# titus-leistner/mmlf

Measured on AMD Instinct MI355X. Metric: 96x96 EPI patches/sec fwd+bwd, bs=512, higher is better.
Workload: dtype f32 via 2 x f16 operand split (22 significant bits per operand, locally scaled; 3 MFMA passes, f32 accumulate)

## Files before the change

### include/mmlf_hip.h

```cpp
#ifndef MMLF_HIP_H
#define MMLF_HIP_H

#include <stddef.h>
#include <stdint.h>

#ifdef __cplusplus
extern "C" {
#endif

#define MMLF_TILE_POSITIONS 256

const char *mmlf_last_error(void);
#define MMLF_ABI_VERSION 10
int mmlf_abi_version(void);

const char *mmlf_build_info(void);
int mmlf_build_is_ablation(void);
int mmlf_conv_cus(void);

enum { MMLF_AUDIT_IN = 0, MMLF_AUDIT_PACKED = 1, MMLF_AUDIT_BIAS = 2, MMLF_AUDIT_OUT = 3, MMLF_AUDIT_REF = 4,
       MMLF_AUDIT_IN_AMAX = 5, MMLF_AUDIT_OUT_AMAX = 6, MMLF_AUDIT_BN_PARTIAL = 7, MMLF_AUDIT_MASK = 8, MMLF_AUDIT_CONV_N = 9 };
int mmlf_audit_conv_h2(int cs_in, int K, int N, int cs_out, int N_store, int out_shift, int cs_ref, int B, int H, int W,
                       int64_t *ends);
enum { MMLF_AUDIT_WG_IN = 0, MMLF_AUDIT_WG_G = 1, MMLF_AUDIT_WG_GW = 2, MMLF_AUDIT_WG_GB = 3, MMLF_AUDIT_WG_WORKSPACE = 4,
       MMLF_AUDIT_WG_IN_AMAX = 5, MMLF_AUDIT_WG_G_AMAX = 6, MMLF_AUDIT_WGRAD_N = 7 };
int mmlf_audit_wgrad_h2(int cs_in, int Cin, int cs_g, int Cout, int g_shift, int B, int H, int W, int64_t *ends);

int64_t mmlf_grid_alloc_positions(int B, int H, int W);
int64_t mmlf_packed_filter_floats(int K, int N);
int64_t mmlf_wgrad_workspace_floats(int Cin, int Cout, int B, int H, int W);

enum { MMLF_VAR_IDENTITY = 0, MMLF_VAR_TRANSPOSE = 1, MMLF_VAR_TRANSPOSE_FLIPH = 2 };

int mmlf_pack_filter(const float *w_oihw, float *packed, int Cout, int Cin, int variant, int dgrad,
                     void *stream);

int mmlf_conv2x2(const float *in, int cs_in, int K, const float *packed, const float *bias, int N,
                 float *out, int cs_out, int N_store, int out_shift, int vh, int vw,
                 int B, int H, int W, int relu, const float *relu_ref, int cs_ref, void *stream);

int64_t mmlf_packed_filter_split_bytes(int K, int N);
int mmlf_pack_filter_split(const float *w_oihw, void *packed, int Cout, int Cin, int variant, int dgrad,
                           void *stream);
int mmlf_conv2x2_split(const float *in, int cs_in, int K, const void *packed, const float *bias, int N,
                       float *out, int cs_out, int N_store, int out_shift, int vh, int vw,
                       int B, int H, int W, int relu, const float *relu_ref, int cs_ref, void *stream);

int64_t mmlf_amax_entries(int B, int H, int W);
int mmlf_grid_pad_w(void);
int mmlf_grid_pad_h(void);
int mmlf_amax_head(void);
int mmlf_amax_shard_stride(void);
int64_t mmlf_packed_filter_h2_bytes(int K, int N);
int mmlf_pack_filter_h2(const float *w_oihw, void *packed, int Cout, int Cin, int variant, int dgrad, void *stream);
typedef struct mmlf_pack_desc {
    const float *w_oihw;
    void *packed;
    int32_t Cout, Cin, variant, dgrad;
    int32_t col0;
    int32_t np;
} mmlf_pack_desc;
int mmlf_packed_filter_h2_columns(int N);
int mmlf_pack_filters_h2(const mmlf_pack_desc *table, int n, int total_columns, void *stream);
int mmlf_conv2x2_h2(const float *in, int cs_in, int K, const void *packed, const float *bias, int N,
                    float *out, int cs_out, int N_store, int out_shift, int vh, int vw,
                    int B, int H, int W, int relu, const float *relu_ref, int cs_ref,
                    const float *in_amax , float *out_amax ,
                    double *bn_partial ,
                    uint32_t *relu_mask_out , const uint32_t *relu_mask_in , void *stream);
int64_t mmlf_relu_mask_words(int B, int H, int W);
int mmlf_conv2x2_blocks(int K, int N, int B, int H, int W);

int64_t mmlf_conv2x2_thin_workspace_floats(int B, int H, int W);
int mmlf_conv2x2_thin(const float *in, int cs_in, int K, const float *w_oihw, const float *bias, int N,
                      float *out, int cs_out, int out_shift, int vh, int vw, int B, int H, int W, int relu,
                      int variant, float *workspace, float *out_amax, void *stream);
int64_t mmlf_conv2x2_wgrad_thin_workspace_floats(int Cin);
int mmlf_conv2x2_wgrad_thin(const float *in, int cs_in, int Cin, const float *g, int cs_g, int Cout, int g_shift,
                            float *gw_oihw, float *gb, int variant, int accumulate, float *workspace,
                            int B, int H, int W, void *stream);

int mmlf_conv2x2_wgrad(const float *in, int cs_in, int Cin, const float *g, int cs_g, int Cout,
                       int g_shift, float *gw_oihw, float *gb, int variant, int accumulate,
                       float *workspace, int B, int H, int W, void *stream);

int mmlf_conv2x2_wgrad_split(const float *in, int cs_in, int Cin, const float *g, int cs_g, int Cout,
                             int g_shift, float *gw_oihw, float *gb, int variant, int accumulate,
                             float *workspace, int B, int H, int W, void *stream);

int mmlf_conv2x2_wgrad_h2(const float *in, int cs_in, int Cin, const float *g, int cs_g, int Cout,
                          int g_shift, float *gw_oihw, float *gb, int variant, int accumulate,
                          float *workspace, int B, int H, int W, const float *in_amax, const float *g_amax,
                          void *stream);

int mmlf_bn_stats_train(const float *z, int cs, int C, const float *gamma, const float *beta,
                        float *running_mean, float *running_var, double momentum, double eps,
                        float *save_mean, float *save_invstd, float *scale, float *shift,
                        double *partial, int nblocks, int B, int H, int W, void *stream);
int mmlf_bn_coeffs_eval(const float *gamma, const float *beta, const float *running_mean,
                        const float *running_var, double eps, float *scale, float *shift, int C,
                        void *stream);
int mmlf_fold_bn_eval(const float *w_oihw, const float *bias, const float *scale, const float *shift,
                      float *w_out, float *bias_out, int Cout, int Cin, void *stream);
int mmlf_bn_stats_finalize(const double *partial, int nblocks, int C, const float *gamma, const float *beta,
                           float *running_mean, float *running_var, double momentum, double eps,
                           float *save_mean, float *save_invstd, float *scale, float *shift,
                           int B, int H, int W, void *stream);
int mmlf_bn_apply_relu(const float *z, int cs_z, int C, const float *scale, const float *shift,
                       float *y, int cs_y, int c_off, int C_store, int B, int H, int W,
                       float *amax_out , void *stream);
int mmlf_bn_apply_relu4(const float *const z[4], int cs_z, int C, const float *const scale[4],
                        const float *const shift[4], float *y, int cs_y, int B, int H, int W,
                        float *amax_out , void *stream);
int mmlf_bn_bwd_reduce(const float *gy, int cs_gy, int c_off, const float *z, int cs_z, int C,
                       const float *scale, const float *shift, const float *gamma,
                       const float *save_mean, const float *save_invstd,
                       float *dgamma, float *dbeta, int accumulate, float *coef,
                       double *partial, int nblocks, int B, int H, int W, void *stream);
int mmlf_bn_bwd_apply(const float *gy, int cs_gy, int c_off, const float *z, int cs_z, int C,
                      const float *scale, const float *shift, const float *save_mean,
                      const float *coef, float *dz, int cs_dz, int B, int H, int W,
                      float *amax_out , void *stream);
int mmlf_relu_bwd_slice(const float *src, int cs_src, int c_off, const float *ref, int cs_ref, int ref_off, int C,
                        float *dst, int cs_dst, int B, int H, int W,
                        float *amax_out , void *stream);
enum { MMLF_AUDIT_SLICE_SRC = 0, MMLF_AUDIT_SLICE_REF = 1, MMLF_AUDIT_SLICE_DST = 2, MMLF_AUDIT_SLICE_AMAX = 3,
       MMLF_AUDIT_SLICE_N = 4 };
int mmlf_audit_relu_bwd_slice(int cs_src, int c_off, int cs_ref, int ref_off, int C, int cs_dst, int B, int H, int W,
                              int64_t *ends);

int mmlf_pack_nchw(const float *nchw, int C, float *grid, int cs, int B, int H, int W,
                   float *amax_out , void *stream);
int mmlf_unpack_nchw(const float *grid, int cs, float *nchw, int C, int B, int H, int W, void *stream);
int mmlf_zero_slack(float *grid, int cs, int B, int H, int W, float *amax, void *stream);
int mmlf_zero_slack4(float *const grid[4], const int cs[4], float *const amax[4], int B, int H, int W, void *stream);

int64_t mmlf_grid_alloc_positions_k3(int B, int H, int W);
int mmlf_zero_slack_k3(float *grid, int cs, int B, int H, int W, float *amax, void *stream);
int mmlf_zero_slack4_k3(float *const grid[4], const int cs[4], float *const amax[4], int B, int H, int W, void *stream);
int64_t mmlf_packed_filter3x3_floats(int K, int N);
int mmlf_pack_filter3x3(const float *w_oihw, float *packed, int Cout, int Cin, int variant, int dgrad, void *stream);
int mmlf_conv3x3(const float *in, int cs_in, int K, const float *packed, const float *bias, int N,
                 float *out, int cs_out, int N_store, int B, int H, int W, int relu, const float *relu_ref, int cs_ref,
                 void *stream);
int64_t mmlf_wgrad3x3_workspace_floats(int Cin, int Cout, int B, int H, int W);
int mmlf_conv3x3_wgrad(const float *in, int cs_in, int Cin, const float *g, int cs_g, int Cout, float *gw_oihw, float *gb,
                       int variant, int accumulate, float *workspace, int B, int H, int W, void *stream);
int mmlf_fold_bn_eval3x3(const float *w_oihw, const float *bias, const float *scale, const float *shift,
                         float *w_out, float *bias_out, int Cout, int Cin, void *stream);
int mmlf_audit_conv3x3(int cs_in, int K, int N, int cs_out, int N_store, int cs_ref, int B, int H, int W, int64_t *ends);
int mmlf_audit_wgrad3x3(int cs_in, int Cin, int cs_g, int Cout, int B, int H, int W, int64_t *ends);

int mmlf_head_upr(const float *output_nchw, const float *grid108, float *posterior, int steps,
                  int B, int H, int W, void *stream);
int mmlf_head_dpp(const float *scores_nchw, const float *grid_torch, const float *grid_np,
                  float *one_hot, float *posterior, float *mean, float *logvar, int steps,
                  int B, int H, int W, void *stream);
int mmlf_head_upr_bwd(const float *output_nchw, const float *grid108, const float *grad_posterior, float *grad_output,
                      int steps, int B, int H, int W, void *stream);
int mmlf_head_dpp_bwd(const float *scores_nchw, const float *grid_np, const float *mean, const float *grad_posterior,
                      const float *grad_logvar, float *grad_scores, int steps, int B, int H, int W, void *stream);

int mmlf_loss_fwd_bwd(int kind, const float *output_nchw, int oc, const float *gt, const int32_t *mask,
                      const float *grid_torch, double half_step, float *loss_out, float *grad_nchw,
                      double *scratch, int nblocks, const double *den_override, int B, int H, int W,
                      void *stream);

int64_t mmlf_loss_multi_scratch_doubles(int nblocks);
int mmlf_loss_multi_fwd_bwd(int kind, const float *output_nchw, int oc, const float *target, int P,
                            const int32_t *mask, const int32_t *mask_padding, const float *grid_torch,
                            double half_step, float *loss_out, float *grad_nchw, double *scratch, int nblocks,
                            const double *den_override, const double *aux_override, int B, int H, int W,
                            void *stream);

int mmlf_adam_step(float *p, const float *g, float *m, float *v, int64_t n, double lr, double beta1,
                   double beta2, double eps, int64_t step, double grad_scale, void *stream);

int mmlf_shift_views(const float *h, const float *v, const float *i, const float *d,
                     float *oh, float *ov, float *oi, float *od, const int32_t *tab_s, const float *tab_w,
                     int S, int views, int H, int W, void *stream);
int mmlf_shift_pack(const float *in, int kind, float *grid, int cs, const int32_t *tab_s, const float *tab_w,
                    int S, int views, int H, int W, float *amax_out, void *stream);
int mmlf_ensamble_reduce(const float *means, const float *logvars, const float *grid, float *mean,
                         float *logvar, float *posterior, int S, int B, int H, int W, void *stream);

int mmlf_lmm_to_discrete(const float *means, const float *logvars, const double *edges, double *out,
                         int S, int B, int n_bins, long long HW, void *stream);

int mmlf_patch_gather(const float *stacks, const float *center, const float *gt, const float *mpi,
                      const int32_t *mask, int S, int V, int P, int Hf, int Wf, const int32_t *iparam,
                      const float *fparam, const int32_t *tab_s, const float *tab_w, const double *mat,
                      const int32_t *rot_src, float *o_stacks, float *o_center, float *o_gt, float *o_mpi,
                      int32_t *o_mask, double *mean_sum, int B, int ps, void *stream);
int mmlf_patch_contrast(float *o_stacks, float *o_center, const double *mean_sum, const float *alpha,
                        int B, int V, int ps, void *stream);

#ifdef __cplusplus
}
#endif
#endif
```

### mmlf_amd/csrc/conv.hip

```cpp
#include "conv_device.h"


#ifdef MMLF_BOUNDS_DEBUG
extern "C" int mmlf_debug_oob_counts(unsigned long long *host8, int reset)
{
    unsigned long long other[8];
    if (hipMemcpyFromSymbol(host8, HIP_SYMBOL(g_mmlf_oob), sizeof(unsigned long long) * 8) != hipSuccess) return 1;
    if (reset) {
        const unsigned long long z[8] = {};
        if (hipMemcpyToSymbol(HIP_SYMBOL(g_mmlf_oob), z, sizeof(z)) != hipSuccess) return 1;
    }
    if (mmlf_oob_counts_wgrad(other, reset)) return 1;
    for (int k = 0; k < 8; ++k) host8[k] += other[k];
    return 0;
}
#endif

template <int KS>
__global__ void pack_filter_f32_kernel(const float *__restrict__ w, float *__restrict__ out, int Cout, int Cin,
                                       int variant, int dgrad, int nchunk, int NP)
{
    constexpr int TAPS = KS * KS;
    const long long total = (long long)nchunk * TAPS * 2 * NP * 4;
    for (long long idx = blockIdx.x * (long long)blockDim.x + threadIdx.x; idx < total;
         idx += (long long)gridDim.x * blockDim.x) {
        int s = idx & 3;
        long long r = idx >> 2;
        int n = r % NP; r /= NP;
        int kh = r & 1; r >>= 1;
        int t = r % TAPS; r /= TAPS;
        int c = (int)r;
        int k = 8 * c + 4 * kh + s;
        int ci, co, tsrc;
        if (!dgrad) { ci = k; co = n; tsrc = t; }
        else { co = k; ci = n; tsrc = TAPS - 1 - t; }
        float v = 0.f;
        if (ci < Cin && co < Cout) v = w[((size_t)co * Cin + ci) * TAPS + master_tap<KS>(tsrc, variant)];
        out[idx] = v;
    }
}

struct ConvArgs {
    const float *in;
    const float *wp;
    const float *bias;
    float *out;
    const float *ref;
    long long NQ;
    int cs_in, nchunk, cs_out, n_store, n_true, out_shift, vh, vw, P, G, relu, cs_ref;
    int a_pieces, seg_slot, seg_delta;
    int a_per_seg, a_tail;
    int nw;
    const float *in_amax;
    const float *w_unscale;
    float *out_amax;
    Magic divP, divR;
    int R;
    double *bn_partial;
    unsigned *relu_mask_out;
    const unsigned *relu_mask_in;
    long long out_bytes, ref_bytes;
    long long in_bytes, amax_n, mask_words;
};


__device__ __forceinline__ unsigned wave_row_mask(const ConvArgs &a, long long Q0, int w, int lane)
{
    const unsigned qrow = (unsigned)Q0 + 32 * w + (lane & 31);
    const unsigned row = fastdiv(qrow, a.divP);
    const int x = (int)(qrow - row * a.P), y = (int)(row - fastdiv(row, a.divR) * a.R);
    return (unsigned)__ballot((long long)qrow < a.NQ && y < a.vh && x < a.vw);
}

template <int NT>
__device__ __forceinline__ void conv_epilogue(const ConvArgs &a, const f32x16 (&acc)[NT], long long Q0, int w, int i,
                                              int kh)
{
    const unsigned m = wave_row_mask(a, Q0, w, i) >> (4 * kh);
    const long long qb = Q0 + 32 * w + a.out_shift;
    const __amdgpu_buffer_rsrc_t ob = __builtin_amdgcn_make_buffer_rsrc(
        a.out + (size_t)qb * a.cs_out, 0, mmlf_records_left(a.out_bytes, qb * a.cs_out * 4ll), MMLF_BUF_FLAGS);
    const bool has_ref = a.ref != nullptr;
    const __amdgpu_buffer_rsrc_t rb = __builtin_amdgcn_make_buffer_rsrc(
        const_cast<float *>(has_ref ? a.ref + (size_t)qb * a.cs_ref : a.out), 0,
        has_ref ? mmlf_records_left(a.ref_bytes, qb * a.cs_ref * 4ll) : 0, MMLF_BUF_FLAGS);
    unsigned lo = ((unsigned)(4 * kh) * a.cs_out + i) * 4u;
    unsigned lr = ((unsigned)(4 * kh) * a.cs_ref + i) * 4u;
    asm volatile("" : "+v"(lo), "+v"(lr));
    float bv[NT];
#pragma unroll
    for (int nt = 0; nt < NT; ++nt) {
        const int ch = 32 * nt + i;
        bv[nt] = (a.bias && ch < a.n_true) ? a.bias[ch] : 0.f;
    }
#pragma unroll
    for (int nt = 0; nt < NT; ++nt) {
        if (32 * nt + i >= a.n_store) continue;
        unsigned keep = m;
        if (has_ref) {
            float rv[16];
#pragma unroll
            for (int r = 0; r < 16; ++r)
                rv[r] = __uint_as_float(__builtin_amdgcn_raw_buffer_load_b32(
                    rb, lr + (unsigned)((r & 3) + 8 * (r >> 2)) * a.cs_ref * 4u + 128 * nt, 0, 0));
#pragma unroll
            for (int r = 0; r < 16; ++r)
                if (!(rv[r] > 0.f)) keep &= ~(1u << ((r & 3) + 8 * (r >> 2)));
        }
#pragma unroll
        for (int r = 0; r < 16; ++r) {
            const int rc = (r & 3) + 8 * (r >> 2);
            float v = acc[nt][r] + bv[nt];
            if (a.relu) v = fmaxf(v, 0.f);
            __builtin_amdgcn_raw_buffer_store_b32(__float_as_uint((keep >> rc & 1) ? v : 0.f), ob,
                                                  lo + (unsigned)rc * a.cs_out * 4u + 128 * nt, 0, 0);
        }
    }
}

__device__ __forceinline__ void pack_filter_h2_column(const float *__restrict__ w, unsigned short *__restrict__ out,
                                                      int Cout, int Cin, int variant, int dgrad, int nchunk, int NP,
                                                      float *__restrict__ unscale, int n, float *red)
{
    const int tid = threadIdx.x;
    const int K = dgrad ? Cout : Cin, N = dgrad ? Cin : Cout;
    auto at = [&](int k, int tap) -> size_t {
        return dgrad ? ((size_t)k * Cin + n) * 4 + tap : ((size_t)n * Cin + k) * 4 + tap;
    };
    float m = 0.f;
    if (n < N)
        for (int e = tid; e < 4 * K; e += 256) m = fmaxf(m, fabsf(w[at(e >> 2, e & 3)]));
    m = mmlf_wave_max(m);
    if ((tid & 63) == 0) red[tid >> 6] = m;
    __syncthreads();
    const float sc = pow2_scale_for(fmaxf(fmaxf(red[0], red[1]), fmaxf(red[2], red[3])));
    if (tid == 0) unscale[n] = 1.f / sc;
    for (int e = tid; e < 4 * nchunk; e += 256) {
        const int c = e >> 2, t = e & 3;
        const int tap = master_tap<2>(dgrad ? 3 - t : t, variant);
        unsigned short h[8], l[8];
#pragma unroll
        for (int j = 0; j < 8; ++j) {
            const int k = 8 * c + j;
            const float v = (k < K && n < N) ? w[at(k, tap)] * sc : 0.f;
            const _Float16 hh = (_Float16)v, ll = (_Float16)(v - (float)hh);
            h[j] = __builtin_bit_cast(unsigned short, hh);
            l[j] = __builtin_bit_cast(unsigned short, ll);
        }
        uint4 vh, vl;
        vh.x = h[0] | (unsigned)h[1] << 16; vh.y = h[2] | (unsigned)h[3] << 16;
        vh.z = h[4] | (unsigned)h[5] << 16; vh.w = h[6] | (unsigned)h[7] << 16;
        vl.x = l[0] | (unsigned)l[1] << 16; vl.y = l[2] | (unsigned)l[3] << 16;
        vl.z = l[4] | (unsigned)l[5] << 16; vl.w = l[6] | (unsigned)l[7] << 16;
        *reinterpret_cast<uint4 *>(out + ((((size_t)c * 2 + 0) * 4 + t) * NP + n) * 8) = vh;
        *reinterpret_cast<uint4 *>(out + ((((size_t)c * 2 + 1) * 4 + t) * NP + n) * 8) = vl;
    }
}

__global__ __launch_bounds__(256) void pack_filter_h2_kernel(const float *__restrict__ w, unsigned short *__restrict__ out,
                                                             int Cout, int Cin, int variant, int dgrad, int nchunk,
                                                             int NP, float *__restrict__ unscale)
{
    __shared__ float red[4];
    pack_filter_h2_column(w, out, Cout, Cin, variant, dgrad, nchunk, NP, unscale, blockIdx.x, red);
}

__global__ __launch_bounds__(256) void pack_filters_h2_kernel(const mmlf_pack_desc *__restrict__ table, int n)
{
    __shared__ float red[4];
    int lo = 0, hi = n - 1;
    while (lo < hi) {
        const int mid = (lo + hi + 1) >> 1;
        if (table[mid].col0 <= (int)blockIdx.x) lo = mid; else hi = mid - 1;
    }
    const mmlf_pack_desc d = table[lo];
    const int K = d.dgrad ? d.Cout : d.Cin;
    const int nchunk = (K + 7) / 8;
    unsigned short *out = reinterpret_cast<unsigned short *>(d.packed);
    float *tail = reinterpret_cast<float *>(reinterpret_cast<char *>(d.packed) + (size_t)nchunk * 8 * d.np * 16);
    pack_filter_h2_column(d.w_oihw, out, d.Cout, d.Cin, d.variant, d.dgrad, nchunk, d.np, tail, (int)blockIdx.x - d.col0, red);
}

__global__ void pack_filter_split_kernel(const float *__restrict__ w, unsigned short *__restrict__ out, int Cout,
                                         int Cin, int variant, int dgrad, int nchunk, int NP)
{
    const long long total = (long long)nchunk * 2 * 2 * NP * 8;
    for (long long idx = blockIdx.x * (long long)blockDim.x + threadIdx.x; idx < total;
         idx += (long long)gridDim.x * blockDim.x) {
        const int j = idx & 7;
        long long r = idx >> 3;
        const int n = r % NP; r /= NP;
        const int kh = r & 1; r >>= 1;
        const int u = r & 1; r >>= 1;
        const int c = (int)r;
        const int k = 8 * c + j, t = 2 * u + kh;
        int ci, co, tsrc;
        if (!dgrad) { ci = k; co = n; tsrc = t; }
        else { co = k; ci = n; tsrc = 3 - t; }
        float v = 0.f;
        if (ci < Cin && co < Cout) v = w[((size_t)co * Cin + ci) * 4 + master_tap<2>(tsrc, variant)];
        unsigned p[3];
        split3(v, p[0], p[1], p[2]);
        for (int pl = 0; pl < 3; ++pl) {
            out[((((size_t)c * 3 + pl) * 4 + t) * NP + n) * 8 + j] = (unsigned short)p[pl];
        }
    }
}



enum { EPI_GENERIC = -1, EPI_PLAIN = 0, EPI_RELU = 1, EPI_STATS = 2, EPI_BITS_IN = 4, EPI_REF_IN = 8, EPI_MASK_OUT = 16 };
template <int G, int EPI>
__device__ __forceinline__ void conv_epilogue16(const ConvArgs &a, const f32x4 (&acc)[2][G], long long Q0, int w,
                                                int r16, int q4, float unscale_a, float &run_max,
                                                double *stats_in )
{
    constexpr bool GEN = EPI == EPI_GENERIC;
    const bool do_relu = GEN ? a.relu != 0 : (EPI & EPI_RELU) != 0;
    double *const stats = (GEN || (EPI & EPI_STATS)) ? stats_in : nullptr;
    const bool mask_out = GEN ? a.relu_mask_out != nullptr : (EPI & EPI_MASK_OUT) != 0;
    const unsigned m = wave_row_mask(a, Q0, w, r16 + 16 * q4) >> (4 * q4);
    const long long qb = Q0 + 32 * w + a.out_shift;
    const int ob_left = mmlf_records_left(a.out_bytes, qb * a.cs_out * 4ll);
    const __amdgpu_buffer_rsrc_t ob =
        __builtin_amdgcn_make_buffer_rsrc(a.out + (size_t)qb * a.cs_out, 0, ob_left, MMLF_BUF_FLAGS);
    const bool has_ref = GEN ? a.ref != nullptr : (EPI & EPI_REF_IN) != 0;
    const __amdgpu_buffer_rsrc_t rb = __builtin_amdgcn_make_buffer_rsrc(
        const_cast<float *>(has_ref ? a.ref + (size_t)qb * a.cs_ref : a.out), 0,
        has_ref ? mmlf_records_left(a.ref_bytes, qb * a.cs_ref * 4ll) : 0, MMLF_BUF_FLAGS);
    unsigned lo = ((unsigned)(4 * q4) * a.cs_out + r16) * 4u;
    unsigned lr = ((unsigned)(4 * q4) * a.cs_ref + r16) * 4u;
    asm volatile("" : "+v"(lo), "+v"(lr));
    float mk[8];
#pragma unroll
    for (int k = 0; k < 8; ++k) mk[k] = 0.f;
    const bool use_bits = GEN ? a.relu_mask_in != nullptr : (EPI & EPI_BITS_IN) != 0;
    const size_t mbase = ((size_t)(Q0 / MMLF_TILE) * 8 + w) * 512 + (r16 + 16 * q4);
    unsigned mw[8];
#pragma unroll
    for (int k = 0; k < 8; ++k) mw[k] = use_bits ? a.relu_mask_in[mbase + 64 * k] : 0u;
    MMLF_OOB(OOB_MASK, (use_bits || mask_out) && (long long)mbase + 64 * 7 >= a.mask_words);
    float bv[G], uwv[G];
#pragma unroll
    for (int nb = 0; nb < G; ++nb) {
        const int ch = 16 * nb + r16;
        bv[nb] = (a.bias && ch < a.n_true) ? a.bias[ch] : 0.f;
        uwv[nb] = (a.w_unscale && ch < 16 * G) ? a.w_unscale[ch] : 1.f;
    }
#pragma unroll
    for (int nb = 0; nb < G; ++nb) asm volatile("" : "+v"(bv[nb]), "+v"(uwv[nb]));
#pragma unroll
    for (int nb = 0; nb < G; ++nb) {
        const int ch = 16 * nb + r16;
        if (ch >= a.n_store) continue;
        const float bvn = bv[nb];
        const float uw = uwv[nb];
        unsigned keep = m;
        float s1 = 0.f, s2 = 0.f;
        if (use_bits) {
#pragma unroll
            for (int k = 0; k < 8; ++k)
                if (!(mw[k] >> nb & 1)) keep &= ~(1u << (16 * (k >> 2) + (k & 3)));
        } else if (has_ref) {
            float rv[8];
#pragma unroll
            for (int k = 0; k < 8; ++k)
            {
                MMLF_OOB(OOB_REF, (qb * a.cs_ref * 4ll) + lr + (long long)(16 * (k >> 2) + (k & 3)) * a.cs_ref * 4 + 64 * nb >= a.ref_bytes);
                rv[k] = __uint_as_float(__builtin_amdgcn_raw_buffer_load_b32(
                    rb, lr + (unsigned)(16 * (k >> 2) + (k & 3)) * a.cs_ref * 4u + 64 * nb, 0, 0));
            }
#pragma unroll
            for (int k = 0; k < 8; ++k)
                if (!(rv[k] > 0.f)) keep &= ~(1u << (16 * (k >> 2) + (k & 3)));
        }
#pragma unroll
        for (int k = 0; k < 8; ++k) {
            const int rc = 16 * (k >> 2) + (k & 3);
            float v = fmaf(acc[k >> 2][nb][k & 3] * unscale_a, uw, bvn);
            if (do_relu) v = fmaxf(v, 0.f);
            v = (keep >> rc & 1) ? v : 0.f;
            if (mask_out) mw[k] |= (v > 0.f ? 1u : 0u) << nb;
            asm("v_max_f32 %0, %1, |%2|" : "=v"(mk[k]) : "v"(mk[k]), "v"(v));
            s1 += v;
            s2 = fmaf(v, v, s2);
            MMLF_OOB(OOB_OUT, (long long)lo + 64 * nb + (long long)rc * a.cs_out * 4 >= ob_left);
            __builtin_amdgcn_raw_buffer_store_b32(__float_as_uint(v), ob, lo + 64 * nb, (unsigned)rc * a.cs_out * 4u, 0);
        }
        if (stats) {
            s1 += __shfl_xor(s1, 16); s1 += __shfl_xor(s1, 32);
            s2 += __shfl_xor(s2, 16); s2 += __shfl_xor(s2, 32);
            if (q4 == 0) {
                stats[2 * (16 * nb + r16)] += (double)s1;
                stats[2 * (16 * nb + r16) + 1] += (double)s2;
            }
        }
    }
    if (mask_out) {
#pragma unroll
        for (int k = 0; k < 8; ++k) a.relu_mask_out[mbase + 64 * k] = mw[k];
    }
    if (a.out_amax) {
        const unsigned d0 = (unsigned)qb;
        const unsigned rd0 = fastdiv(d0, a.divP);
        const int nfirst = (int)((rd0 + 1) * (unsigned)a.P - d0);
        float m_lo = 0.f, m_hi = 0.f;
#pragma unroll
        for (int k = 0; k < 8; ++k) {
            const int pos = 16 * (k >> 2) + 4 * q4 + (k & 3);
            if (pos < nfirst) m_lo = fmaxf(m_lo, mk[k]);
            else m_hi = fmaxf(m_hi, mk[k]);
        }
        m_lo = mmlf_wave_max(m_lo);
        m_hi = mmlf_wave_max(m_hi);
        if (r16 + 16 * q4 == 0) {
            MMLF_OOB(OOB_AMAX, MMLF_AMAX_HEAD + (long long)fastdiv(d0 + 31, a.divP) >= a.amax_n);
            if (m_lo > 0.f) mmlf_amax_raise_nowait(a.out_amax + MMLF_AMAX_HEAD + rd0, m_lo);
            if (m_hi > 0.f) {
                const unsigned rdl = fastdiv(d0 + 31, a.divP);
                for (unsigned r = rd0 + 1; r <= rdl; ++r) mmlf_amax_raise_nowait(a.out_amax + MMLF_AMAX_HEAD + r, m_hi);
            }
            run_max = fmaxf(run_max, fmaxf(m_lo, m_hi));
        }
    }
}

template <int G> constexpr int tr_mask_words() { return (G + 7) / 8; }
template <int G, int EPI>
__device__ __forceinline__ void conv_epilogue16_tr(const ConvArgs &a, const f32x4 (&acc)[2][G], long long Q0, int w,
                                                   int r16, int q4, float unscale_a, float &run_max,
                                                   const float *coef )
{
    static_assert(EPI >= 0 && !(EPI & (EPI_STATS | EPI_REF_IN)), "kinds of the transposed epilogue");
    constexpr int NP = 16 * G, MW = tr_mask_words<G>();
    constexpr bool do_relu = (EPI & EPI_RELU) != 0, mask_out = (EPI & EPI_MASK_OUT) != 0, use_bits = (EPI & EPI_BITS_IN) != 0;
    const unsigned m = wave_row_mask(a, Q0, w, r16 + 16 * q4);
    const long long qb = Q0 + 32 * w + a.out_shift;
    const int ob_left = mmlf_records_left(a.out_bytes, qb * a.cs_out * 4ll);
    const __amdgpu_buffer_rsrc_t ob =
        __builtin_amdgcn_make_buffer_rsrc(a.out + (size_t)qb * a.cs_out, 0, ob_left, MMLF_BUF_FLAGS);
    unsigned lo = ((unsigned)r16 * a.cs_out + 4u * q4) * 4u;
    asm volatile("" : "+v"(lo));
    const size_t mbase = ((size_t)(Q0 / MMLF_TILE) * 8 + w) * 512 + (r16 + 16 * q4);
    unsigned mw[2][MW];
    bool ok[2];
#pragma unroll
    for (int mb = 0; mb < 2; ++mb) {
        ok[mb] = (m >> (16 * mb + r16) & 1u) != 0;
#pragma unroll
        for (int j = 0; j < MW; ++j) {
            mw[mb][j] = use_bits ? a.relu_mask_in[mbase + 64 * (MW * mb + j)] : 0u;
            if (use_bits && !ok[mb]) mw[mb][j] = 0u;
        }
    }
    MMLF_OOB(OOB_MASK, (use_bits || mask_out) && (long long)mbase + 64 * (2 * MW - 1) >= a.mask_words);
    float mk[2] = {0.f, 0.f};
    const float *cl = coef + 4 * q4;
    f32x4 uw_n = *reinterpret_cast<const f32x4 *>(cl), b_n = *reinterpret_cast<const f32x4 *>(cl + NP);
#pragma unroll
    for (int nb = 0; nb < G; ++nb) {
        const int c0 = 16 * nb + 4 * q4;
        const f32x4 uw4 = uw_n, b4 = b_n;
        if (nb + 1 < G) {
            uw_n = *reinterpret_cast<const f32x4 *>(cl + 16 * (nb + 1));
            b_n = *reinterpret_cast<const f32x4 *>(cl + NP + 16 * (nb + 1));
        }
        __builtin_amdgcn_sched_barrier(0);
#pragma unroll
        for (int mb = 0; mb < 2; ++mb) {
            u32x4 st;
#pragma unroll
            for (int r = 0; r < 4; ++r) {
                float v = fmaf(acc[mb][nb][r] * unscale_a, uw4[r], b4[r]);
                if (do_relu) v = fmaxf(v, 0.f);
                if (use_bits) {
                    const int keep = ((int)(mw[mb][nb >> 3] << (31 - (4 * (nb & 7) + r)))) >> 31;
                    v = __uint_as_float(__float_as_uint(v) & (unsigned)keep);
                } else {
                    v = ok[mb] ? v : 0.f;
                }
                if (mask_out) mw[mb][nb >> 3] |= (v > 0.f ? 1u : 0u) << (4 * (nb & 7) + r);
                asm("v_max_f32 %0, %1, |%2|" : "=v"(mk[mb]) : "v"(mk[mb]), "v"(v));
                st[r] = __float_as_uint(v);
            }
            if (c0 < a.n_store) {
                MMLF_OOB(OOB_OUT, (long long)lo + 64 * nb + (long long)(16 * mb) * a.cs_out * 4 + 12 >= ob_left);
                __builtin_amdgcn_raw_buffer_store_b128(st, ob, lo + 64 * nb, (unsigned)(16 * mb) * a.cs_out * 4u, 0);
            }
        }
        __builtin_amdgcn_sched_barrier(0);
    }
    if (mask_out) {
#pragma unroll
        for (int mb = 0; mb < 2; ++mb)
#pragma unroll
            for (int j = 0; j < MW; ++j) a.relu_mask_out[mbase + 64 * (MW * mb + j)] = mw[mb][j];
    }
    if (a.out_amax) {
        const unsigned d0 = (unsigned)qb;
        const unsigned rd0 = fastdiv(d0, a.divP);
        const int nfirst = (int)((rd0 + 1) * (unsigned)a.P - d0);
        float m_lo = 0.f, m_hi = 0.f;
#pragma unroll
        for (int mb = 0; mb < 2; ++mb) {
            if (16 * mb + r16 < nfirst) m_lo = fmaxf(m_lo, mk[mb]);
            else m_hi = fmaxf(m_hi, mk[mb]);
        }
        m_lo = mmlf_wave_max(m_lo);
        m_hi = mmlf_wave_max(m_hi);
        if (r16 + 16 * q4 == 0) {
            MMLF_OOB(OOB_AMAX, MMLF_AMAX_HEAD + (long long)fastdiv(d0 + 31, a.divP) >= a.amax_n);
            if (m_lo > 0.f) mmlf_amax_raise_nowait(a.out_amax + MMLF_AMAX_HEAD + rd0, m_lo);
            if (m_hi > 0.f) {
                const unsigned rdl = fastdiv(d0 + 31, a.divP);
                for (unsigned r = rd0 + 1; r <= rdl; ++r) mmlf_amax_raise_nowait(a.out_amax + MMLF_AMAX_HEAD + r, m_hi);
            }
            run_max = fmaxf(run_max, fmaxf(m_lo, m_hi));
        }
    }
}
template <int NP>
__device__ __forceinline__ void conv_fill_coef(const ConvArgs &a, float *coef, int tid, int nthreads)
{
    for (int k = tid; k < NP; k += nthreads) {
        coef[k] = a.w_unscale ? a.w_unscale[k] : 1.f;
        coef[NP + k] = (a.bias && k < a.n_true) ? a.bias[k] : 0.f;
    }
}

__device__ __forceinline__ float wave_operand_amax_gather(const ConvArgs &a, long long Q0, int w, int lane)
{
    const long long q0 = Q0 + 32 * w;
    float m = 0.f;
    if (q0 < a.NQ) {
        const long long ql = q0 + 31 < a.NQ ? q0 + 31 : a.NQ - 1;
        const unsigned r0 = fastdiv((unsigned)q0, a.divP);
        unsigned r1 = fastdiv((unsigned)ql, a.divP);
        r1 += (r1 - fastdiv(r1, a.divR) * (unsigned)a.R != (unsigned)(a.R - 1)) ? 1u : 0u;
        MMLF_OOB(OOB_AMAX, lane == 0 && MMLF_AMAX_HEAD + (long long)r1 >= a.amax_n);
        for (unsigned r = r0 + lane; r <= r1; r += 64) m = fmaxf(m, a.in_amax[MMLF_AMAX_HEAD + r]);
    }
    return m;
}
__device__ __forceinline__ float wave_operand_scale(float gathered)
{
    return __uint_as_float(__builtin_amdgcn_readfirstlane(__float_as_uint(pow2_scale_for(mmlf_wave_max(gathered)))));
}

typedef const __attribute__((address_space(4))) ConvArgs *ConvKernArgs;
__device__ __forceinline__ ConvArgs late_args()
{
#if defined(__HIP_DEVICE_COMPILE__)
    ConvKernArgs p = (ConvKernArgs)__builtin_amdgcn_kernarg_segment_ptr();
    asm volatile("" : "+s"(p));
    return *p;
#else
    return ConvArgs();
#endif
}

constexpr int RING16 = 3;
template <int G, int PL, int EPI = EPI_GENERIC, int NW = 8, bool TR = false>
__global__ __launch_bounds__(64 * NW, (NW == 16 || G <= 6 ? 4 : 2)) void conv4tap_x6s_kernel(ConvArgs a, int ntiles)
{
    constexpr int NP = G * 16;
    constexpr int TILE = 32 * NW;
    constexpr int D = NW == 16 ? RING16 : 2;
    constexpr bool EARLY = PL == 2 && G % 3 == 0 && G >= 9;
    constexpr int A_F4 = 2 * 640;
    constexpr int B_F4 = 4 * PL * NP;
    constexpr int BUF_F4 = A_F4 + B_F4;
    constexpr int N_B = B_F4 / 64;
    constexpr int PER_WAVE = (20 + N_B + NW - 1) / NW;
    constexpr int PER_SLOT = (PER_WAVE + 1) / 2;
    extern __shared__ __attribute__((aligned(16))) char smem[];
    float4 *lds = reinterpret_cast<float4 *>(smem);

    const int tid = threadIdx.x;
    const int lane = tid & 63;
    const int w = __builtin_amdgcn_readfirstlane(tid >> 6);
    const int r16 = lane & 15, q4 = lane >> 4;

    f32x4 acc[2][G];
#pragma unroll
    for (int mb = 0; mb < 2; ++mb)
#pragma unroll
        for (int nb = 0; nb < G; ++nb)
#pragma unroll
            for (int r = 0; r < 4; ++r) acc[mb][nb][r] = 0.f;

    const unsigned voff_a = ((unsigned)(lane >> 1) * (unsigned)a.cs_in + 4u * (lane & 1)) * 4u;
    const unsigned voff_b = (unsigned)lane * 16u;
    const unsigned lds_base = (unsigned)(size_t)(lds_void_t *)smem;
    const char *in0 = reinterpret_cast<const char *>(a.in);
    const char *wp_base = reinterpret_cast<const char *>(a.wp);
    const size_t tile_bytes = (size_t)TILE * a.cs_in * 4;
    const int n_a = a.a_pieces;
    const int nA = (n_a - w + NW - 1) / NW;
    const int jb0 = w + NW * nA - n_a;
    const int nB = (N_B - jb0 + NW - 1) / NW;
    int n_mine = nA + nB;
    unsigned a_src[3], a_dst[3];
#pragma unroll
    for (int k = 0; k < 3; ++k) {
        const int j = w + NW * k;
        const int seg = j >= a.a_per_seg, idx = j - seg * a.a_per_seg;
        const int slot = 320 * seg + 32 * idx;
        a_src[k] = (unsigned)(slot + seg * a.seg_delta) * (unsigned)a.cs_in * 4u;
        a_dst[k] = (unsigned)slot * 32u + (idx == a.a_per_seg - 1 ? 1u : 0u);
    }
    const unsigned tail_lim = ((unsigned)(a.a_tail - 1) * (unsigned)a.cs_in + 4u) * 4u;
    const unsigned b_src0 = 1024u * jb0, b_dst0 = (unsigned)(A_F4 + 64 * jb0) * 16u;

#ifdef MMLF_BOUNDS_DEBUG
#define MMLF_DMA_SRC_CHECK()                                                                             \
    do {                                                                                                 \
        MMLF_OOB(OOB_IN, (long long)(sb_ - in0) + vo_ + 16 > a.in_bytes);                                \
        const unsigned long long u_ = (unsigned long long)sb_;                                           \
        sb_ = reinterpret_cast<const char *>(                                                            \
            ((unsigned long long)__builtin_amdgcn_readfirstlane((unsigned)(u_ >> 32)) << 32) |           \
            (unsigned)__builtin_amdgcn_readfirstlane((unsigned)u_));                                     \
    } while (0)
#else
#define MMLF_DMA_SRC_CHECK() do { } while (0)
#endif
#define X6_DMA_PIECE(tl, c, buf, k)                                                                      \
    do {                                                                                                 \
        if ((k) < PER_WAVE && (k) < n_mine) {                                                            \
            const char *sb_;                                                                             \
            unsigned vo_, d_;                                                                            \
            if ((k) < nA) {                                                                              \
                sb_ = in0 + (size_t)(tl) * tile_bytes + 32u * (c) + a_src[(k) < 3 ? (k) : 0];            \
                d_ = a_dst[(k) < 3 ? (k) : 0];                                                           \
                vo_ = min(voff_a, (d_ & 1u) ? tail_lim : 0xffffffffu);                                   \
                d_ &= ~1u;                                                                               \
                MMLF_DMA_SRC_CHECK();                                                                    \
            } else {                                                                                     \
                const unsigned kb_ = (1024u * NW) * (unsigned)((k) - nA);                                \
                sb_ = wp_base + (size_t)(c) * (B_F4 * 16) + b_src0 + kb_;                                \
                vo_ = voff_b;                                                                            \
                d_ = b_dst0 + kb_;                                                                       \
            }                                                                                            \
            d_ = __builtin_amdgcn_readfirstlane(d_ + lds_base + (buf) * (BUF_F4 * 16));                  \
            unsigned keep_;                                                                              \
            asm volatile("s_mov_b32 %0, m0\n\ts_mov_b32 m0, %3\n\ts_nop 0\n\t"                       \
                         "global_load_lds_dwordx4 %1, %2\n\ts_mov_b32 m0, %0"                           \
                         : "=&s"(keep_) : "v"(vo_), "s"(sb_), "s"(d_) : "memory");                      \
        }                                                                                                \
    } while (0)
#define X6_DMA_SLOT(tl, c, buf, slot)                                                                    \
    do {                                                                                                 \
        _Pragma("unroll") for (int k_ = 0; k_ < PER_SLOT; ++k_)                                          \
            X6_DMA_PIECE(tl, c, buf, (slot) * PER_SLOT + k_);                                            \
    } while (0)
#define X6_DMA_WAIT() asm volatile("s_waitcnt vmcnt(0)" ::: "memory")
#define X6_CHUNK_WAIT()                                                                                  \
    do {                                                                                                 \
        if (D > 2 && more) {       \
            static_assert(PER_WAVE <= 3 || D == 2, "counted waits are written for up to three pieces per wave");             \
            if (n_mine == 1) asm volatile("s_waitcnt vmcnt(%0)" ::"n"(1 * (D - 2)) : "memory");            \
            else if (n_mine == 2) asm volatile("s_waitcnt vmcnt(%0)" ::"n"(2 * (D - 2)) : "memory");       \
            else if (n_mine == 3) asm volatile("s_waitcnt vmcnt(%0)" ::"n"(3 * (D - 2)) : "memory");       \
            else X6_DMA_WAIT();                                                                          \
        } else {                                                                                         \
            X6_DMA_WAIT();                                                                               \
        }                                                                                                \
    } while (0)

    const int per_xcd = (int)gridDim.x >> 3;
    const int first_tile = (gridDim.x & 7) == 0 ? (int)(blockIdx.x & 7) * per_xcd + (int)(blockIdx.x >> 3)
                                                : (int)blockIdx.x;
    int tile = first_tile, c = 0;
    int ntile = tile, nc = 0;
    if (tile >= ntiles) return;
    float *coef = reinterpret_cast<float *>(lds + D * BUF_F4);
    double *stats_all = reinterpret_cast<double *>(lds + D * BUF_F4);
    if constexpr (TR) conv_fill_coef<NP>(late_args(), coef, tid, 64 * NW);
    else if (late_args().bn_partial)
        for (int k = tid; k < NW * NP * 2; k += 64 * NW) stats_all[k] = 0.0;
    float scale_a = 1.f, unscale_a = 1.f, run_max = 0.f;
    if constexpr (PL == 2) {
        scale_a = wave_operand_scale(wave_operand_amax_gather(late_args(), (long long)tile * TILE, w, lane));
        unscale_a = 1.f / scale_a;
    }
#pragma unroll
    for (int d = 0; d < D - 1; ++d) {
        if (ntile < ntiles) {
            X6_DMA_SLOT(ntile, nc, d, 0);
            X6_DMA_SLOT(ntile, nc, d, 1);
        }
        if (++nc == a.nchunk) { nc = 0; ntile += gridDim.x; }
    }
    X6_DMA_WAIT();
    __syncthreads();
    int buf = 0;
    float4 ra[2][2];
    bf16x8 bq[3][PL];
    const int a_lane = 2 * (32 * w + r16 + (q4 & 1) + (q4 >> 1) * a.seg_slot);
    const int b_lane = q4 * NP + r16;
    if constexpr (EARLY) {
#pragma unroll
        for (int mb = 0; mb < 2; ++mb)
#pragma unroll
            for (int hf = 0; hf < 2; ++hf) ra[mb][hf] = lds[a_lane + 32 * mb + hf];
#pragma unroll
        for (int g0 = 0; g0 < 2; ++g0)
#pragma unroll
            for (int pl = 0; pl < PL; ++pl)
                bq[g0][pl] = (reinterpret_cast<const bf16x8 *>(lds + A_F4) + b_lane)[pl * 4 * NP + 16 * g0];
    }

    while (tile < ntiles) {
        asm volatile("" : "+s"(n_mine));
        const bool more = ntile < ntiles;
        const int fb = buf == 0 ? D - 1 : buf - 1;
        const float4 *base = lds + buf * BUF_F4;
        const float4 *nbase = lds + (buf + 1 == D ? 0 : buf + 1) * BUF_F4;
        const float4 *ap = base + a_lane;
        const bf16x8 *bp = reinterpret_cast<const bf16x8 *>(base + A_F4) + b_lane;
        const bf16x8 *bpn = reinterpret_cast<const bf16x8 *>(nbase + A_F4) + b_lane;
        const bool tile_end = c + 1 == a.nchunk;

        if constexpr (!EARLY) {
#pragma unroll
            for (int mb = 0; mb < 2; ++mb)
#pragma unroll
                for (int hf = 0; hf < 2; ++hf) ra[mb][hf] = ap[32 * mb + hf];
#pragma unroll
            for (int g0 = 0; g0 < 2; ++g0)
#pragma unroll
                for (int pl = 0; pl < PL; ++pl) bq[g0][pl] = bp[pl * 4 * NP + 16 * g0];
        }
        bf16x8 asp[2][PL];
#pragma unroll
        for (int mb = 0; mb < 2; ++mb) {
            unsigned hh[4], mm[4], ll[4];
            if constexpr (PL == 3) {
                split3_pair(ra[mb][0].x, ra[mb][0].y, hh[0], mm[0], ll[0]);
                split3_pair(ra[mb][0].z, ra[mb][0].w, hh[1], mm[1], ll[1]);
                split3_pair(ra[mb][1].x, ra[mb][1].y, hh[2], mm[2], ll[2]);
                split3_pair(ra[mb][1].z, ra[mb][1].w, hh[3], mm[3], ll[3]);
                const u32x4_t vm = {mm[0], mm[1], mm[2], mm[3]};
                asp[mb][1] = __builtin_bit_cast(bf16x8, vm);
            } else {
                split2_pair_f16(ra[mb][0].x, ra[mb][0].y, scale_a, hh[0], ll[0]);
                split2_pair_f16(ra[mb][0].z, ra[mb][0].w, scale_a, hh[1], ll[1]);
                split2_pair_f16(ra[mb][1].x, ra[mb][1].y, scale_a, hh[2], ll[2]);
                split2_pair_f16(ra[mb][1].z, ra[mb][1].w, scale_a, hh[3], ll[3]);
            }
            const u32x4_t vh = {hh[0], hh[1], hh[2], hh[3]}, vl = {ll[0], ll[1], ll[2], ll[3]};
            asp[mb][0] = __builtin_bit_cast(bf16x8, vh);
            asp[mb][PL - 1] = __builtin_bit_cast(bf16x8, vl);
        }
#pragma unroll
        for (int g = 0; g < G; ++g) {
            if (EARLY && g == G - 2) {
                X6_CHUNK_WAIT();
                asm volatile("s_waitcnt lgkmcnt(0)" ::: "memory");
                __syncthreads();
                if (!tile_end) {
#pragma unroll
                    for (int mb = 0; mb < 2; ++mb)
#pragma unroll
                        for (int hf = 0; hf < 2; ++hf) ra[mb][hf] = (nbase + a_lane)[32 * mb + hf];
                }
            }
            if (g + 2 < G) {
#pragma unroll
                for (int pl = 0; pl < PL; ++pl) bq[(g + 2) % 3][pl] = bp[pl * 4 * NP + 16 * (g + 2)];
            } else if (EARLY && !tile_end) {
#pragma unroll
                for (int pl = 0; pl < PL; ++pl) bq[(g + 2) % 3][pl] = bpn[pl * 4 * NP + 16 * (g + 2 - G)];
            }
            __builtin_amdgcn_sched_barrier(0);
            if (more) {
                if (w < NW / 2) {
                    if (g == 0) { X6_DMA_SLOT(ntile, nc, fb, 0); X6_DMA_SLOT(ntile, nc, fb, 1); }
                } else {
                    if (g == (PL == 2 && G >= 8 ? G / 8 : G / 4)) { X6_DMA_SLOT(ntile, nc, fb, 0); X6_DMA_SLOT(ntile, nc, fb, 1); }
                }
            }
            __builtin_amdgcn_sched_barrier(0);
#define X6_TERM(pa, pb)                                                                                      \
    _Pragma("unroll") for (int mb = 0; mb < 2; ++mb)                                                         \
        acc[mb][g] = __builtin_amdgcn_mfma_f32_16x16x32_bf16(asp[mb][pa], bq[g % 3][pb], acc[mb][g], 0, 0, 0)
#define H2_TERM(pa, pb)                                                                                      \
    _Pragma("unroll") for (int mb = 0; mb < 2; ++mb)                                                         \
        acc[mb][g] = TR ? __builtin_amdgcn_mfma_f32_16x16x32_f16(__builtin_bit_cast(f16x8, bq[g % 3][pb]),   \
                                                                 __builtin_bit_cast(f16x8, asp[mb][pa]), acc[mb][g], 0, 0, 0) \
                        : __builtin_amdgcn_mfma_f32_16x16x32_f16(__builtin_bit_cast(f16x8, asp[mb][pa]),     \
                                                                 __builtin_bit_cast(f16x8, bq[g % 3][pb]), acc[mb][g], 0, 0, 0)
            if constexpr (PL == 3) {
                X6_TERM(2, 0);
                X6_TERM(0, 2);
                X6_TERM(1, 1);
                X6_TERM(1, 0);
                X6_TERM(0, 1);
                X6_TERM(0, 0);
            } else {
                H2_TERM(1, 0);
                H2_TERM(0, 1);
                H2_TERM(0, 0);
            }
#undef X6_TERM
#undef H2_TERM
            __builtin_amdgcn_sched_barrier(0);
        }
        if (more && ++nc == a.nchunk) { nc = 0; ntile += gridDim.x; }
        if constexpr (!EARLY) X6_CHUNK_WAIT();
        if (++c == a.nchunk) {
            const ConvArgs e = late_args();
            float next_amax = 0.f;
            if constexpr (PL == 2)
                if (tile + (int)gridDim.x < ntiles)
                    next_amax = wave_operand_amax_gather(e, (long long)(tile + gridDim.x) * TILE, w, lane);
            if constexpr (TR)
                conv_epilogue16_tr<G, EPI>(e, acc, (long long)tile * TILE, w, r16, q4, unscale_a, run_max, coef);
            else
                conv_epilogue16<G, EPI>(e, acc, (long long)tile * TILE, w, r16, q4, unscale_a, run_max,
                                        e.bn_partial ? stats_all + (size_t)w * NP * 2 : nullptr);
#pragma unroll
            for (int mb = 0; mb < 2; ++mb)
#pragma unroll
                for (int nb = 0; nb < G; ++nb)
#pragma unroll
                    for (int r = 0; r < 4; ++r) acc[mb][nb][r] = 0.f;
            c = 0;
            tile += gridDim.x;
            if constexpr (PL == 2) {
                if (tile < ntiles) {
                    scale_a = wave_operand_scale(next_amax);
                    unscale_a = 1.f / scale_a;
                }
            }
            if constexpr (EARLY) {
#pragma unroll
                for (int mb = 0; mb < 2; ++mb)
#pragma unroll
                    for (int hf = 0; hf < 2; ++hf) ra[mb][hf] = (nbase + a_lane)[32 * mb + hf];
#pragma unroll
                for (int g0 = 0; g0 < 2; ++g0)
#pragma unroll
                    for (int pl = 0; pl < PL; ++pl) bq[g0][pl] = bpn[pl * 4 * NP + 16 * g0];
            }
        }
        if constexpr (!EARLY) __syncthreads();
        buf = buf + 1 == D ? 0 : buf + 1;
    }
    if constexpr (EARLY) __syncthreads();
    const ConvArgs e = late_args();
    if (e.out_amax) mmlf_amax_update(run_max, e.out_amax, blockIdx.x * NW + w);
    if (e.bn_partial) {
        for (int k = tid; k < 2 * e.n_true; k += 64 * NW) {
            const int ch = k % e.n_true, which = k / e.n_true;
            double t = 0.0;
#pragma unroll
            for (int ww = 0; ww < NW; ++ww) t += stats_all[((size_t)ww * NP + ch) * 2 + which];
            e.bn_partial[((size_t)blockIdx.x * 2 + which) * e.n_true + ch] = t;
        }
    }
#undef X6_DMA_PIECE
#undef MMLF_DMA_SRC_CHECK
#undef X6_DMA_SLOT
#undef X6_DMA_WAIT
#undef X6_CHUNK_WAIT
}



template <int G, int NCH, int EPI, bool TR = false>
__global__ __launch_bounds__(512, 2) void conv4tap_rs_kernel(ConvArgs a, int ngroups)
{
    constexpr int NP = G * 16;
    constexpr int WBYTES = NCH * 2 * 4 * NP * 16;
    constexpr int NS = NCH / 4, REM = NCH % 4;
    static_assert(REM == 0 || REM == 1, "input channels: a multiple of 32, or one octet more");
    constexpr int NSTEP = 4 * NS + REM, NLOAD = 4 * NSTEP;
    extern __shared__ __attribute__((aligned(16))) char smem[];
    const int tid = threadIdx.x;
    const int lane = tid & 63;
    const int w = __builtin_amdgcn_readfirstlane(tid >> 6);
    const int r16 = lane & 15, q4 = lane >> 4;

    for (int o = tid * 16; o < WBYTES; o += 512 * 16)
        *reinterpret_cast<uint4 *>(smem + o) = *reinterpret_cast<const uint4 *>(reinterpret_cast<const char *>(a.wp) + o);
    float *coef = reinterpret_cast<float *>(smem + WBYTES);
    double *stats_all = reinterpret_cast<double *>(smem + WBYTES);
    if constexpr (TR) conv_fill_coef<NP>(a, coef, tid, 512);
    else if (a.bn_partial)
        for (int k = tid; k < 8 * NP * 2; k += 512) stats_all[k] = 0.0;
    __syncthreads();

    int gi, gstep, gend;
    if ((gridDim.x & 7) == 0) {
        const int per = (ngroups + 7) >> 3, nbx = (int)gridDim.x >> 3;
        const int x = (int)blockIdx.x & 7;
        gi = x * per + ((int)blockIdx.x >> 3) * 8 + w;
        gstep = nbx * 8;
        gend = min(ngroups, (x + 1) * per);
    } else {
        gi = (int)blockIdx.x * 8 + w;
        gstep = (int)gridDim.x * 8;
        gend = ngroups;
    }

    f32x4 acc[2][G];
#pragma unroll
    for (int mb = 0; mb < 2; ++mb)
#pragma unroll
        for (int nb = 0; nb < G; ++nb)
#pragma unroll
            for (int r = 0; r < 4; ++r) acc[mb][nb][r] = 0.f;
    float run_max = 0.f;
    const bf16x8 *bpF = reinterpret_cast<const bf16x8 *>(smem) + q4 * 8 * NP + r16;
    const bf16x8 *bpR = reinterpret_cast<const bf16x8 *>(smem) + q4 * NP + r16;
    auto bfrag = [&](int k, int nb, int pl) -> bf16x8 {
        return k < 4 * NS ? bpF[(8 * (k % NS) + pl) * 4 * NP + (k / NS) * NP + 16 * nb] : bpR[(8 * NS + pl) * 4 * NP + 16 * nb];
    };
    const size_t row_off = (size_t)r16 * a.cs_in;
    const size_t rem_off = (size_t)((q4 & 1) + (q4 >> 1) * a.P) * a.cs_in + 32 * NS;

    for (; gi < gend; gi += gstep) {
        const long long Q0 = (long long)(gi >> 3) * MMLF_TILE;
        const int wv = gi & 7;
        const float gathered = wave_operand_amax_gather(a, Q0, wv, lane);
        const float *p0 = a.in + (size_t)(Q0 + 32 * wv) * a.cs_in + row_off;
        float4 raw[NSTEP][2][2];
#pragma unroll
        for (int k = 0; k < NSTEP; ++k) {
            const int t = k / NS, s_ = k % NS;
            const float *pk = k < 4 * NS ? p0 + (size_t)((t & 1) + (t >> 1) * a.P) * a.cs_in + 32 * s_ + 8 * q4 : p0 + rem_off;
#pragma unroll
            for (int mb = 0; mb < 2; ++mb)
#pragma unroll
                for (int hf = 0; hf < 2; ++hf)
                {
                    MMLF_OOB(OOB_IN, (long long)((pk + (size_t)(16 * mb) * a.cs_in + 4 * hf + 4) - a.in) * 4 > a.in_bytes);
                    raw[k][mb][hf] = reinterpret_cast<const float4 *>(pk + (size_t)(16 * mb) * a.cs_in)[hf];
                }
            __builtin_amdgcn_sched_barrier(0);
        }
        asm volatile("s_waitcnt vmcnt(%0)" ::"n"(NLOAD > 63 ? 63 : NLOAD) : "memory");
        const float scale_a = wave_operand_scale(gathered);
        const float unscale_a = 1.f / scale_a;
        bf16x8 bq[3][2];
#pragma unroll
        for (int g0 = 0; g0 < 2; ++g0)
#pragma unroll
            for (int pl = 0; pl < 2; ++pl) bq[g0][pl] = bfrag(0, g0, pl);
#pragma unroll
        for (int k = 0; k < NSTEP; ++k) {
            asm volatile("s_waitcnt vmcnt(%0)" ::"n"(4 * (NSTEP - 1 - k) > 63 ? 63 : 4 * (NSTEP - 1 - k)) : "memory");
            bf16x8 asp[2][2];
#pragma unroll
            for (int mb = 0; mb < 2; ++mb) {
                unsigned hh[4], ll[4];
                float4 &r0 = raw[k][mb][0], &r1 = raw[k][mb][1];
                asm volatile("" : "+v"(r0.x), "+v"(r0.y), "+v"(r0.z), "+v"(r0.w), "+v"(r1.x), "+v"(r1.y), "+v"(r1.z), "+v"(r1.w));
                split2_pair_f16(r0.x, r0.y, scale_a, hh[0], ll[0]);
                split2_pair_f16(r0.z, r0.w, scale_a, hh[1], ll[1]);
                split2_pair_f16(r1.x, r1.y, scale_a, hh[2], ll[2]);
                split2_pair_f16(r1.z, r1.w, scale_a, hh[3], ll[3]);
                const u32x4_t vh = {hh[0], hh[1], hh[2], hh[3]}, vl = {ll[0], ll[1], ll[2], ll[3]};
                asp[mb][0] = __builtin_bit_cast(bf16x8, vh);
                asp[mb][1] = __builtin_bit_cast(bf16x8, vl);
            }
            __builtin_amdgcn_sched_barrier(0);
            asm volatile("s_nop 4" ::: "memory");
            __builtin_amdgcn_sched_barrier(0);
#pragma unroll
            for (int g = 0; g < G; ++g) {
                constexpr int NB = NSTEP * G;
                const int idx = k * G + g;
                if (idx + 2 < NB) {
#pragma unroll
                    for (int pl = 0; pl < 2; ++pl) bq[(idx + 2) % 3][pl] = bfrag((idx + 2) / G, (idx + 2) % G, pl);
                }
#define RS_TERM(pa, pb)                                                                                      \
    _Pragma("unroll") for (int mb = 0; mb < 2; ++mb)                                                         \
        acc[mb][g] = TR ? __builtin_amdgcn_mfma_f32_16x16x32_f16(__builtin_bit_cast(f16x8, bq[idx % 3][pb]), \
                                                                 __builtin_bit_cast(f16x8, asp[mb][pa]), acc[mb][g], 0, 0, 0) \
                        : __builtin_amdgcn_mfma_f32_16x16x32_f16(__builtin_bit_cast(f16x8, asp[mb][pa]),     \
                                                                 __builtin_bit_cast(f16x8, bq[idx % 3][pb]), acc[mb][g], 0, 0, 0)
                RS_TERM(1, 0);
                RS_TERM(0, 1);
                RS_TERM(0, 0);
#undef RS_TERM
            }
        }
        if constexpr (TR)
            conv_epilogue16_tr<G, EPI>(a, acc, Q0, wv, r16, q4, unscale_a, run_max, coef);
        else
            conv_epilogue16<G, EPI>(a, acc, Q0, wv, r16, q4, unscale_a, run_max,
                                    a.bn_partial ? stats_all + (size_t)w * NP * 2 : nullptr);
#pragma unroll
        for (int mb = 0; mb < 2; ++mb)
#pragma unroll
            for (int nb = 0; nb < G; ++nb)
#pragma unroll
                for (int r = 0; r < 4; ++r) acc[mb][nb][r] = 0.f;
    }
    if (a.out_amax) mmlf_amax_update(run_max, a.out_amax, blockIdx.x * 8 + w);
    if (a.bn_partial) {
        __syncthreads();
        for (int k = tid; k < 2 * a.n_true; k += 512) {
// ... 168 lines not shown
                           int dgrad, void *stream)
{
    MMLF_CHECK_ARG(w && packed, "%s: null pointer", who);
    MMLF_CHECK_ARG(variant >= 0 && variant <= 2, "%s: bad variant %d", who, variant);
    MMLF_CHECK_ARG(Cout > 0 && Cin > 0, "%s: bad channels %d x %d", who, Cout, Cin);
    const int K = dgrad ? Cout : Cin, N = dgrad ? Cin : Cout;
    const int nt = pick_nt(N);
    MMLF_CHECK_ARG(nt > 0, "%s: N=%d not supported (max 288)", who, N);
    const int nchunk = (K + 7) / 8, NP = nt * 32;
    const long long total = (long long)nchunk * ks * ks * 2 * NP * 4;
    int blocks = (int)((total + 255) / 256);
    if (blocks > 4096) blocks = 4096;
    hipLaunchKernelGGL(ks == 2 ? pack_filter_f32_kernel<2> : pack_filter_f32_kernel<3>, dim3(blocks), dim3(256), 0,
                       (hipStream_t)stream, w, packed, Cout, Cin, variant, dgrad, nchunk, NP);
    return mmlf_launch_status(who);
}

extern "C" int64_t mmlf_packed_filter_floats(int K, int N) { return packed_filter_f32_floats(2, K, N); }

extern "C" int mmlf_pack_filter(const float *w, float *packed, int Cout, int Cin, int variant, int dgrad,
                                void *stream)
{
    return pack_filter_f32("mmlf_pack_filter", 2, w, packed, Cout, Cin, variant, dgrad, stream);
}

static void conv_buffer_bytes(ConvArgs &a, const Grid &g, long long alloc)
{
    a.out_bytes = (alloc * a.cs_out - (a.cs_out - a.n_store)) * 4;
    a.ref_bytes = a.ref ? alloc * a.cs_ref * 4 : 0;
    a.in_bytes = alloc * a.cs_in * 4;
    a.amax_n = amax_entries(g);
    a.mask_words = g.NQpad / MMLF_TILE * 4096;
}

static int conv_common_args(const char *who, int ks, int np, ConvArgs &a, Grid &g, const float *in, int cs_in, int K,
                            const void *packed, const float *bias, int N, float *out, int cs_out, int N_store,
                            int out_shift, int vh, int vw, int B, int H, int W, int relu, const float *relu_ref, int cs_ref)
{
    MMLF_CHECK_ARG(in && packed && out, "%s: null pointer", who);
    MMLF_CHECK_ARG(B > 0 && H > 0 && W > 0, "%s: bad shape B=%d H=%d W=%d", who, B, H, W);
    MMLF_CHECK_ARG(cs_in > 0 && cs_in % 8 == 0, "%s: cs_in=%d must be a multiple of 8", who, cs_in);
    MMLF_CHECK_ARG(K > 0 && (K + 7) / 8 * 8 == cs_in, "%s: K=%d does not match cs_in=%d", who, K, cs_in);
    MMLF_CHECK_ARG(np > 0, "%s: N=%d not supported (max 288)", who, N);
    MMLF_CHECK_ARG(N_store > 0 && N_store <= cs_out && N_store <= np, "%s: N_store=%d vs cs_out=%d NP=%d", who,
                   N_store, cs_out, np);
    g = make_grid(B, H, W);
    MMLF_CHECK_ARG(out_shift >= 0 && out_shift <= g.P + 1, "%s: out_shift=%d", who, out_shift);
    MMLF_CHECK_ARG(!relu_ref || cs_ref >= N_store, "%s: cs_ref=%d < N_store", who, cs_ref);
    MMLF_CHECK_ARG(g.NQpad + (ks - 1) * g.P + 64 < (1ll << 31), "%s: batch x image too large for 32-bit grid positions", who);
    a = {};
    a.in = in; a.wp = reinterpret_cast<const float *>(packed); a.bias = bias; a.out = out; a.ref = relu_ref;
    a.NQ = g.NQ; a.cs_in = cs_in; a.nchunk = cs_in / 8; a.cs_out = cs_out; a.n_store = N_store; a.n_true = N;
    a.out_shift = out_shift; a.vh = vh; a.vw = vw; a.P = g.P; a.G = g.G; a.R = g.R; a.relu = relu; a.cs_ref = cs_ref;
    a.divP = make_magic((unsigned)g.P); a.divR = make_magic((unsigned)g.R);
    conv_buffer_bytes(a, g, ks == 3 ? grid_alloc_positions_k3(g) : grid_alloc_positions(g));
    return 0;
}

template <int KS, int NT>
static int launch_conv_f32(const ConvArgs &a, long long ntiles, int ncb, hipStream_t st)
{
    constexpr const char *who = KS == 2 ? "mmlf_conv2x2" : "mmlf_conv3x3";
    constexpr size_t lds = ConvF32Lds<KS, NT>::BYTES;
    static PerDeviceOnce attr_once;
    if constexpr (KS == 2) {
        if (attr_once.run([] { return mmlf_allow_lds(reinterpret_cast<const void *>(conv4tap_kernel<NT>), lds, who); })) return 1;
        hipLaunchKernelGGL(conv4tap_kernel<NT>, dim3((unsigned)ntiles), dim3(512), lds, st, a);
    } else {
        if (attr_once.run([] { return mmlf_allow_lds(reinterpret_cast<const void *>(conv9tap_kernel<NT>), lds, who); })) return 1;
        hipLaunchKernelGGL(conv9tap_kernel<NT>, dim3((unsigned)(ntiles * ncb)), dim3(512), lds, st, a, ncb, ncb * NT * 32);
    }
    return mmlf_launch_status(who);
}

extern "C" int mmlf_conv2x2(const float *in, int cs_in, int K, const float *packed, const float *bias, int N,
                            float *out, int cs_out, int N_store, int out_shift, int vh, int vw, int B, int H,
                            int W, int relu, const float *relu_ref, int cs_ref, void *stream)
{
    const int nt = pick_nt(N);
    ConvArgs a;
    Grid g;
    if (conv_common_args("mmlf_conv2x2", 2, nt * 32, a, g, in, cs_in, K, packed, bias, N, out, cs_out, N_store, out_shift, vh,
                         vw, B, H, W, relu, relu_ref, cs_ref))
        return 1;
    const long long ntiles = g.NQpad / MMLF_TILE;
    hipStream_t st = (hipStream_t)stream;
    switch (nt) {
    case 1: return launch_conv_f32<2, 1>(a, ntiles, 1, st);
    case 3: return launch_conv_f32<2, 3>(a, ntiles, 1, st);
    case 4: return launch_conv_f32<2, 4>(a, ntiles, 1, st);
    default: return launch_conv_f32<2, 9>(a, ntiles, 1, st);
    }
}

static inline int x6_np(int N)
{
    if (N <= 0 || N > 288) return -1;
    if (N <= 32) return 32;
    if (N <= 80) return 80;
    if (N <= 128) return (N + 15) / 16 * 16;
    return 288;
}

extern "C" int64_t mmlf_packed_filter_split_bytes(int K, int N)
{
    const int np = x6_np(N);
    if (np < 0 || K <= 0) return -1;
    return (int64_t)((K + 7) / 8) * 12 * np * 16;
}

extern "C" int mmlf_pack_filter_split(const float *w, void *packed, int Cout, int Cin, int variant, int dgrad,
                                      void *stream)
{
    MMLF_CHECK_ARG(w && packed, "mmlf_pack_filter_split: null pointer");
    MMLF_CHECK_ARG(variant >= 0 && variant <= 2, "mmlf_pack_filter_split: bad variant %d", variant);
    const int K = dgrad ? Cout : Cin, N = dgrad ? Cin : Cout;
    const int NP = x6_np(N);
    MMLF_CHECK_ARG(NP > 0, "mmlf_pack_filter_split: N=%d not supported (max 288)", N);
    const int nchunk = (K + 7) / 8;
    const long long total = (long long)nchunk * 32 * NP;
    int blocks = (int)((total + 255) / 256);
    if (blocks > 4096) blocks = 4096;
    hipLaunchKernelGGL(pack_filter_split_kernel, dim3(blocks), dim3(256), 0, (hipStream_t)stream, w,
                       (unsigned short *)packed, Cout, Cin, variant, dgrad, nchunk, NP);
    return mmlf_launch_status("mmlf_pack_filter_split");
}

static long long conv_split_blocks(int G, long long ntiles, int nw = 8)
{
    const long long grid = (G <= 6 && nw == 8 ? 2ll : 1ll) * device_cus();
    return grid > ntiles ? ntiles : grid;
}
static bool conv_sixteen_waves(int planes, int np, const Grid &g)
{
    static const int on = [] { const char *e = getenv("MMLF_CONV_NW16"); return e ? atoi(e) : 1; }();
    return on && planes == 2 && np == 80 && g.P + 513 <= 640;
}

static bool conv_tr_enabled()
{
    static const int on = [] { const char *e = getenv("MMLF_CONV_TR"); return e ? atoi(e) : 1; }();
    return on != 0;
}
static bool conv_tr_fits(const ConvArgs &a)
{
    return a.n_store % 4 == 0 && a.cs_out % 4 == 0 && (reinterpret_cast<uintptr_t>(a.out) & 15) == 0;
}

template <int G, int PL, int EPI, bool TR = false>
static int launch_conv_x6s_epi(const ConvArgs &a, long long ntiles, hipStream_t st)
{
    constexpr size_t lds_pipe = 2 * (2 * 640 + 4 * PL * G * 16) * sizeof(float4);
    constexpr size_t lds_stats = 8 * (G * 16) * 2 * sizeof(double);
    constexpr size_t lds_coef = 2 * (G * 16) * sizeof(float);
    static PerDeviceOnce attr_once;
    if (attr_once.run([] { return mmlf_allow_lds(reinterpret_cast<const void *>(conv4tap_x6s_kernel<G, PL, EPI, 8, TR>),
                                                 lds_pipe + (TR ? lds_coef : PL == 2 ? lds_stats : 0), "mmlf_conv2x2_h2"); }))
        return 1;
    if constexpr (PL == 2 && G == 5) {
        if (a.nw == 16) {
            constexpr size_t lds_stats16 = 16 * (G * 16) * 2 * sizeof(double);
            constexpr size_t lds_pipe16 = RING16 * (2 * 640 + 4 * PL * G * 16) * sizeof(float4);
            static PerDeviceOnce attr_once16;
            if (attr_once16.run([] { return mmlf_allow_lds(reinterpret_cast<const void *>(conv4tap_x6s_kernel<G, PL, EPI, 16, TR>),
                                                           lds_pipe16 + (TR ? lds_coef : lds_stats16), "mmlf_conv2x2_h2(16 waves)"); }))
                return 1;
            const size_t lds16 = lds_pipe16 + (TR ? lds_coef : a.bn_partial ? lds_stats16 : 0);
            const long long grid16 = conv_split_blocks(G, ntiles, 16);
            hipLaunchKernelGGL((conv4tap_x6s_kernel<G, PL, EPI, 16, TR>), dim3((unsigned)grid16), dim3(1024), lds16, st, a, (int)ntiles);
            return mmlf_launch_status("mmlf_conv2x2_h2(16 waves)");
        }
    }
    const size_t lds = lds_pipe + (TR ? lds_coef : a.bn_partial ? lds_stats : 0);
    const long long grid = conv_split_blocks(G, ntiles);
    hipLaunchKernelGGL((conv4tap_x6s_kernel<G, PL, EPI, 8, TR>), dim3((unsigned)grid), dim3(512), lds, st, a, (int)ntiles);
    return mmlf_launch_status(PL == 3 ? "mmlf_conv2x2_split" : "mmlf_conv2x2_h2");
}

static int conv_rs_mode()
{
    static const int mode = [] { const char *e = getenv("MMLF_CONV_RS"); return e ? atoi(e) : -1; }();
    return mode;
}
static bool conv_rs_shape(int planes, int np, int nchunk, int nw)
{
    if (!(planes == 2 && np == 80 && (nchunk == 9 || nchunk == 4))) return false;
    const int mode = conv_rs_mode();
    return mode < 0 ? nw == 8 : mode != 0;
}
static long long conv_rs_blocks(long long ngroups)
{
    const long long grid = device_cus(), need = (ngroups + 7) / 8;
    return grid > need ? need : grid;
}
template <int G, int NCH, int EPI, bool TR = false>
static int launch_conv_rs_epi(const ConvArgs &a, long long ngroups, hipStream_t st)
{
    constexpr size_t lds = (size_t)NCH * 2 * 4 * (G * 16) * 16 + (TR ? 2 * (G * 16) * sizeof(float) : 8 * (G * 16) * 2 * sizeof(double));
    static PerDeviceOnce attr_once;
    if (attr_once.run([] { return mmlf_allow_lds(reinterpret_cast<const void *>(conv4tap_rs_kernel<G, NCH, EPI, TR>), lds, "mmlf_conv2x2_h2(register-streamed)"); }))
        return 1;
    hipLaunchKernelGGL((conv4tap_rs_kernel<G, NCH, EPI, TR>), dim3((unsigned)conv_rs_blocks(ngroups)), dim3(512), lds, st, a, (int)ngroups);
    return mmlf_launch_status("mmlf_conv2x2_h2(register-streamed)");
}
#define MMLF_CONV_KIND_SWITCH(LAUNCH, TR_PLAIN, TR_SHAPE, ...)                                                                              \
    do {                                                                                                                \
        const int kind = (a.relu ? EPI_RELU : 0) | (a.bn_partial ? EPI_STATS : 0) | (a.relu_mask_in ? EPI_BITS_IN : 0) | \
                         (a.ref ? EPI_REF_IN : 0) | (a.relu_mask_out ? EPI_MASK_OUT : 0);                               \
        const bool tr = conv_tr_enabled() && (TR_SHAPE) && conv_tr_fits(a);                                             \
        if ((a.relu_mask_in || a.relu_mask_out) && conv_tr_enabled() && (TR_SHAPE) && !tr)                              \
            return mmlf_fail("mmlf_conv2x2_h2: ReLU mask words need n_store %% 4 == 0 and a 16-byte aligned output");   \
        switch (kind) {                                                                                                 \
        case EPI_PLAIN: return tr && TR_PLAIN ? LAUNCH<__VA_ARGS__, EPI_PLAIN, true>(a, n, st) : LAUNCH<__VA_ARGS__, EPI_PLAIN>(a, n, st); \
        case EPI_RELU: return tr ? LAUNCH<__VA_ARGS__, EPI_RELU, true>(a, n, st) : LAUNCH<__VA_ARGS__, EPI_RELU>(a, n, st); \
        case EPI_RELU | EPI_MASK_OUT:                                                                                   \
            return tr ? LAUNCH<__VA_ARGS__, EPI_RELU | EPI_MASK_OUT, true>(a, n, st) : LAUNCH<__VA_ARGS__, EPI_RELU | EPI_MASK_OUT>(a, n, st); \
        case EPI_BITS_IN: return tr ? LAUNCH<__VA_ARGS__, EPI_BITS_IN, true>(a, n, st) : LAUNCH<__VA_ARGS__, EPI_BITS_IN>(a, n, st); \
        case EPI_STATS: return LAUNCH<__VA_ARGS__, EPI_STATS>(a, n, st);                                                \
        default: break;                                                                                                 \
        }                                                                                                               \
    } while (0)
template <int G, int NCH>
static int launch_conv_rs(const ConvArgs &a, long long n, hipStream_t st)
{
    MMLF_CONV_KIND_SWITCH(launch_conv_rs_epi, false, true, G, NCH);
    return launch_conv_rs_epi<G, NCH, EPI_GENERIC>(a, n, st);
}

template <int G, int PL>
static int launch_conv_x6s(const ConvArgs &a, long long ntiles, hipStream_t st)
{
    if constexpr (PL == 2 && G == 5) {
        if (conv_rs_shape(PL, G * 16, a.nchunk, a.nw)) {
            const long long ngroups = ntiles * a.nw;
            return a.nchunk == 9 ? launch_conv_rs<G, 9>(a, ngroups, st) : launch_conv_rs<G, 4>(a, ngroups, st);
        }
    }
    if constexpr (PL == 2 && (G == 5 || G == 18)) {
        const long long n = ntiles;
        if (a.ref && !a.relu && !a.bn_partial && !a.relu_mask_in && !a.relu_mask_out)
            return launch_conv_x6s_epi<G, PL, EPI_REF_IN>(a, n, st);
        MMLF_CONV_KIND_SWITCH(launch_conv_x6s_epi, G == 18, G != 18 || a.seg_delta == 0, G, PL);
    }
    return launch_conv_x6s_epi<G, PL, EPI_GENERIC>(a, ntiles, st);
}

template <int PL>
static int launch_conv_split(int np, const ConvArgs &a, long long ntiles, hipStream_t st)
{
    switch (np) {
    case 32: return launch_conv_x6s<2, PL>(a, ntiles, st);
    case 80: return launch_conv_x6s<5, PL>(a, ntiles, st);
    case 96: return launch_conv_x6s<6, PL>(a, ntiles, st);
    case 112: return launch_conv_x6s<7, PL>(a, ntiles, st);
    case 128: return launch_conv_x6s<8, PL>(a, ntiles, st);
    default: return launch_conv_x6s<18, PL>(a, ntiles, st);
    }
}

static int conv_split_impl(const char *who, int planes, const float *in, int cs_in, int K, const void *packed,
                           const float *bias, int N, float *out, int cs_out, int N_store, int out_shift, int vh,
                           int vw, int B, int H, int W, int relu, const float *relu_ref, int cs_ref,
                           const float *in_amax, float *out_amax, double *bn_partial, void *stream,
                           unsigned *relu_mask_out = nullptr, const unsigned *relu_mask_in = nullptr)
{
    const int np = x6_np(N);
    ConvArgs a;
    Grid g;
    if (conv_common_args(who, 2, np, a, g, in, cs_in, K, packed, bias, N, out, cs_out, N_store, out_shift, vh, vw, B, H, W, relu,
                         relu_ref, cs_ref))
        return 1;
    MMLF_CHECK_ARG(!(relu_ref && relu_mask_in), "%s: relu_ref and relu_mask_in are alternatives", who);
    MMLF_CHECK_ARG((long long)cs_in * 4 * 64 < (1ll << 31), "%s: cs_in too large", who);
    MMLF_CHECK_ARG(planes == 3 || in_amax, "%s: the f16 split needs the input's max |x|", who);
    MMLF_CHECK_ARG(!bn_partial || (planes == 2 && N_store >= N), "%s: BatchNorm statistics need the f16 split path", who);
    a.in_amax = in_amax; a.out_amax = out_amax; a.bn_partial = bn_partial;
    a.relu_mask_out = relu_mask_out; a.relu_mask_in = relu_mask_in;
    a.w_unscale = planes == 2 ? reinterpret_cast<const float *>(reinterpret_cast<const char *>(packed) +
                                                                  (size_t)(cs_in / 8) * 8 * np * 16)
                              : nullptr;
    a.nw = conv_sixteen_waves(planes, np, g) ? 16 : 8;
    const int tile = 32 * a.nw;
    if (g.P + tile + 1 <= 640) {
        a.a_pieces = a.a_per_seg = (g.P + tile + 1 + 31) / 32; a.seg_slot = g.P; a.seg_delta = 0;
    } else {
        a.a_per_seg = 9; a.a_pieces = 18; a.seg_slot = 320; a.seg_delta = g.P - 320;
    }
    a.a_tail = (a.seg_delta ? 257 : g.P + tile + 1) - 32 * (a.a_per_seg - 1);
    const long long ntiles = g.NQpad / tile;
    hipStream_t st = (hipStream_t)stream;
    return planes == 3 ? launch_conv_split<3>(np, a, ntiles, st) : launch_conv_split<2>(np, a, ntiles, st);
}

extern "C" int mmlf_conv2x2_split(const float *in, int cs_in, int K, const void *packed, const float *bias, int N,
                                  float *out, int cs_out, int N_store, int out_shift, int vh, int vw, int B, int H,
                                  int W, int relu, const float *relu_ref, int cs_ref, void *stream)
{
    return conv_split_impl("mmlf_conv2x2_split", 3, in, cs_in, K, packed, bias, N, out, cs_out, N_store, out_shift,
                           vh, vw, B, H, W, relu, relu_ref, cs_ref, nullptr, nullptr, nullptr, stream);
}

extern "C" int64_t mmlf_packed_filter_h2_bytes(int K, int N)
{
    const int np = x6_np(N);
    if (np < 0 || K <= 0) return -1;
    return (int64_t)((K + 7) / 8) * 8 * np * 16 + (int64_t)np * 4;
}

extern "C" int mmlf_pack_filter_h2(const float *w, void *packed, int Cout, int Cin, int variant, int dgrad,
                                   void *stream)
{
    MMLF_CHECK_ARG(w && packed, "mmlf_pack_filter_h2: null pointer");
    MMLF_CHECK_ARG(variant >= 0 && variant <= 2, "mmlf_pack_filter_h2: bad variant %d", variant);
    const int K = dgrad ? Cout : Cin, N = dgrad ? Cin : Cout;
    const int NP = x6_np(N);
    MMLF_CHECK_ARG(NP > 0, "mmlf_pack_filter_h2: N=%d not supported (max 288)", N);
    const int nchunk = (K + 7) / 8;
    float *tail = reinterpret_cast<float *>(reinterpret_cast<char *>(packed) + (size_t)nchunk * 8 * NP * 16);
    hipLaunchKernelGGL(pack_filter_h2_kernel, dim3(NP), dim3(256), 0, (hipStream_t)stream, w, (unsigned short *)packed,
                       Cout, Cin, variant, dgrad, nchunk, NP, tail);
    return mmlf_launch_status("mmlf_pack_filter_h2");
}

extern "C" int mmlf_packed_filter_h2_columns(int N) { return x6_np(N); }

extern "C" int mmlf_pack_filters_h2(const mmlf_pack_desc *table, int n, int total_columns, void *stream)
{
    MMLF_CHECK_ARG(table && n > 0 && total_columns > 0, "mmlf_pack_filters_h2: empty table");
    hipLaunchKernelGGL(pack_filters_h2_kernel, dim3((unsigned)total_columns), dim3(256), 0, (hipStream_t)stream, table, n);
    return mmlf_launch_status("mmlf_pack_filters_h2");
}

extern "C" int mmlf_conv2x2_h2(const float *in, int cs_in, int K, const void *packed, const float *bias, int N,
                               float *out, int cs_out, int N_store, int out_shift, int vh, int vw, int B, int H,
                               int W, int relu, const float *relu_ref, int cs_ref, const float *in_amax,
                               float *out_amax, double *bn_partial, uint32_t *relu_mask_out,
                               const uint32_t *relu_mask_in, void *stream)
{
    return conv_split_impl("mmlf_conv2x2_h2", 2, in, cs_in, K, packed, bias, N, out, cs_out, N_store, out_shift, vh,
                           vw, B, H, W, relu, relu_ref, cs_ref, in_amax, out_amax, bn_partial, stream, relu_mask_out,
                           relu_mask_in);
}

extern "C" int64_t mmlf_relu_mask_words(int B, int H, int W)
{
    if (B <= 0 || H <= 0 || W <= 0) return -1;
    return make_grid(B, H, W).NQpad / MMLF_TILE * 4096;
}

extern "C" int mmlf_conv2x2_blocks(int K, int N, int B, int H, int W)
{
    const int np = x6_np(N);
    if (np < 0 || K <= 0 || B <= 0 || H <= 0 || W <= 0) return -1;
    const Grid g = make_grid(B, H, W);
    const int nw = conv_sixteen_waves(2, np, g) ? 16 : 8;
    if (conv_rs_shape(2, np, (K + 7) / 8, nw)) return (int)conv_rs_blocks(g.NQpad / 32);
    return (int)conv_split_blocks(np / 16, g.NQpad / (32 * nw), nw);
}


__global__ __launch_bounds__(256) void thin_rowdot_kernel(ThinArgs a)
{
    __shared__ float tile[4][64][33];
    __shared__ float4 wt[4][32][2];
    const int lane = threadIdx.x & 63, wv = threadIdx.x >> 6;
    const long long wave = __builtin_amdgcn_readfirstlane((int)(blockIdx.x * 4 + wv));
    const long long nwaves = gridDim.x * 4ll;
    const int nslice = (a.C + 31) / 32;
    for (long long p0 = 64 * wave; p0 < a.npos; p0 += 64 * nwaves) {
        float acc[4][THIN_MAXN];
#pragma unroll
        for (int t = 0; t < 4; ++t)
#pragma unroll
            for (int o = 0; o < THIN_MAXN; ++o) acc[t][o] = 0.f;
        for (int sl = 0; sl < nslice; ++sl) {
            float4 v[8];
#pragma unroll
            for (int j = 0; j < 8; ++j) {
                const int r = (lane >> 3) + 8 * j, f = lane & 7;
                const long long p = p0 + r < a.npos ? p0 + r : a.npos - 1;
                const int c = 32 * sl + 4 * f;
                v[j] = *reinterpret_cast<const float4 *>(a.in + (size_t)p * a.cs_in + (c < a.cs_in ? c : 0));
                if (c >= a.cs_in) v[j] = make_float4(0.f, 0.f, 0.f, 0.f);
            }
            {
                const int c = 32 * sl + (lane & 31), o = lane >> 5;
                float4 w4 = make_float4(0.f, 0.f, 0.f, 0.f);
                if (c < a.C && o < a.N) {
                    const float *wp = a.w + ((size_t)o * a.C + c) * 4;
                    w4 = make_float4(wp[master_tap<2>(0, a.variant)], wp[master_tap<2>(1, a.variant)], wp[master_tap<2>(2, a.variant)],
                                     wp[master_tap<2>(3, a.variant)]);
                }
                wt[wv][lane & 31][o] = w4;
            }
#pragma unroll
            for (int j = 0; j < 8; ++j) {
                const int r = (lane >> 3) + 8 * j, f = lane & 7;
                tile[wv][r][4 * f + 0] = v[j].x; tile[wv][r][4 * f + 1] = v[j].y;
                tile[wv][r][4 * f + 2] = v[j].z; tile[wv][r][4 * f + 3] = v[j].w;
            }
#pragma unroll 8
            for (int k = 0; k < 32; ++k) {
                const float x = tile[wv][lane][k];
                const float4 w0 = wt[wv][k][0], w1 = wt[wv][k][1];
                acc[0][0] = fmaf(x, w0.x, acc[0][0]); acc[1][0] = fmaf(x, w0.y, acc[1][0]);
                acc[2][0] = fmaf(x, w0.z, acc[2][0]); acc[3][0] = fmaf(x, w0.w, acc[3][0]);
                acc[0][1] = fmaf(x, w1.x, acc[0][1]); acc[1][1] = fmaf(x, w1.y, acc[1][1]);
                acc[2][1] = fmaf(x, w1.z, acc[2][1]); acc[3][1] = fmaf(x, w1.w, acc[3][1]);
            }
        }
        const long long p = p0 + lane;
        if (p < a.npos) {
            float4 *dst = reinterpret_cast<float4 *>(a.part + (size_t)p * 4 * THIN_MAXN);
            dst[0] = make_float4(acc[0][0], acc[0][1], acc[1][0], acc[1][1]);
            dst[1] = make_float4(acc[2][0], acc[2][1], acc[3][0], acc[3][1]);
        }
    }
}

__global__ __launch_bounds__(128) void thin_combine_kernel(ThinArgs a)
{
    const int drow = blockIdx.x;
    float mx = 0.f;
    for (int x = threadIdx.x; x < a.P; x += blockDim.x) {
        const long long d = (long long)drow * a.P + x, q = d - a.out_shift;
        float v[THIN_MAXN] = {0.f, 0.f};
        bool valid = false;
        if (q >= 0 && q < a.NQ) {
            const unsigned row = fastdiv((unsigned)q, a.divP);
            const int qx = (int)(q - (long long)row * a.P), qy = (int)(row - fastdiv(row, a.divR) * a.R);
            valid = qy < a.vh && qx < a.vw;
        }
        if (valid) {
            const int offs[4] = {0, 1, a.P, a.P + 1};
#pragma unroll
            for (int o = 0; o < THIN_MAXN; ++o) {
                float s = (a.bias && o < a.N) ? a.bias[o] : 0.f;
#pragma unroll
                for (int t = 0; t < 4; ++t) s += a.part[((size_t)(q + offs[t]) * 4 + t) * THIN_MAXN + o];
                if (a.relu) s = fmaxf(s, 0.f);
                v[o] = o < a.N ? s : 0.f;
            }
        }
        float *dst = a.out + (size_t)d * a.cs_out;
        for (int o = 0; o < a.cs_out; ++o) dst[o] = o < THIN_MAXN ? v[o] : 0.f;
        mx = fmaxf(mx, fmaxf(fabsf(v[0]), fabsf(v[1])));
    }
    if (a.out_amax) mmlf_amax_update_row(mx, a.out_amax, drow);
}

extern "C" int64_t mmlf_conv2x2_thin_workspace_floats(int B, int H, int W)
{
    if (B <= 0 || H <= 0 || W <= 0) return -1;
    const Grid g = make_grid(B, H, W);
    return (g.NQ + g.P + 2) * 4 * THIN_MAXN;
}

extern "C" int mmlf_conv2x2_thin(const float *in, int cs_in, int K, const float *w_oihw, const float *bias, int N,
                                 float *out, int cs_out, int out_shift, int vh, int vw, int B, int H, int W, int relu,
                                 int variant, float *workspace, float *out_amax, void *stream)
{
    MMLF_CHECK_ARG(in && w_oihw && out && workspace, "mmlf_conv2x2_thin: null pointer");
    MMLF_CHECK_ARG(N >= 1 && N <= THIN_MAXN && K >= 1 && K <= cs_in && cs_in % 4 == 0 && cs_in <= 512,
                   "mmlf_conv2x2_thin: N=%d K=%d cs_in=%d (N <= 2, cs_in <= 512)", N, K, cs_in);
    MMLF_CHECK_ARG(B > 0 && H > 0 && W > 0 && cs_out >= THIN_MAXN && variant >= 0 && variant <= 2, "mmlf_conv2x2_thin: bad shape");
    const Grid g = make_grid(B, H, W);
    MMLF_CHECK_ARG(out_shift >= 0 && out_shift <= g.P + 1 && g.NQpad + 2 * g.P + 64 < (1ll << 31), "mmlf_conv2x2_thin: out_shift / size");
    ThinArgs a = {};
    a.in = in; a.w = w_oihw; a.bias = bias; a.part = workspace; a.out = out; a.out_amax = out_amax;
    a.NQ = g.NQ; a.npos = g.NQ + g.P + 2; a.cs_in = cs_in; a.C = K; a.N = N; a.cs_out = cs_out; a.out_shift = out_shift;
    a.vh = vh; a.vw = vw; a.P = g.P; a.R = g.R; a.relu = relu; a.variant = variant;
    a.divP = make_magic((unsigned)g.P); a.divR = make_magic((unsigned)g.R);
    hipStream_t st = (hipStream_t)stream;
    hipLaunchKernelGGL(thin_rowdot_kernel, dim3(4 * device_cus()), dim3(256), 0, st, a);
    hipLaunchKernelGGL(thin_combine_kernel, dim3((unsigned)(B * g.R)), dim3(128), 0, st, a);
    return mmlf_launch_status("mmlf_conv2x2_thin");
}

#ifndef MMLF_GIT_HASH
#define MMLF_GIT_HASH "unknown"
#endif
#ifdef MMLF_BOUNDS_DEBUG
#define MMLF_BOUNDS_DEBUG_VALUE 1
#else
#define MMLF_BOUNDS_DEBUG_VALUE 0
#endif
extern "C" int mmlf_build_is_ablation(void) { return 0; }
extern "C" const char *mmlf_build_info(void)
{
    static char text[448];
    static std::once_flag once;
// ... 92 lines not shown
```

### mmlf_amd/csrc/elementwise.hip

```cpp
#include "common.h"
#include "../../include/mmlf_hip.h"

thread_local char g_mmlf_err[512] = "";

extern "C" const char *mmlf_last_error(void) { return g_mmlf_err; }
extern "C" int mmlf_abi_version(void) { return MMLF_ABI_VERSION; }
extern "C" int64_t mmlf_amax_entries(int B, int H, int W)
{
    if (B <= 0 || H <= 0 || W <= 0) return -1;
    return amax_entries(make_grid(B, H, W));
}
extern "C" int mmlf_grid_pad_w(void) { return GRID_PAD; }
extern "C" int mmlf_grid_pad_h(void) { return GRID_PAD; }
extern "C" int mmlf_amax_head(void) { return MMLF_AMAX_HEAD; }
extern "C" int mmlf_amax_shard_stride(void) { return MMLF_AMAX_SHARD_STRIDE; }
extern "C" int64_t mmlf_grid_alloc_positions(int B, int H, int W)
{
    if (B <= 0 || H <= 0 || W <= 0) return -1;
    return grid_alloc_positions(make_grid(B, H, W));
}
extern "C" int64_t mmlf_grid_alloc_positions_k3(int B, int H, int W)
{
    if (B <= 0 || H <= 0 || W <= 0) return -1;
    return grid_alloc_positions_k3(make_grid(B, H, W));
// ... 63 lines not shown
                                                        const float *__restrict__ invstd, int C,
                                                        double *__restrict__ partial, int B, int H, int W)
{
    const int P = W + GRID_PAD, R = H + GRID_PAD;
    const int cvn = (C + V - 1) / V;
    const int ppi = 256 / cvn;
    const int tid = threadIdx.x;
    const int pl = tid / cvn, cg = tid - pl * cvn;
    const bool active = pl < ppi;
    double s0[V], s1[V];
#pragma unroll
    for (int e = 0; e < V; ++e) { s0[e] = 0; s1[e] = 0; }
    __shared__ double red[2][256][V];
    float *cf = reinterpret_cast<float *>(&red[0][0][0]);
    if (BWD) {
        for (int c = tid; c < cvn * V; c += 256) {
            const bool in = c < C;
            cf[0 * 256 * V + c] = in ? scale[c] : 0.f;
            cf[1 * 256 * V + c] = in ? shift[c] : 0.f;
            cf[2 * 256 * V + c] = in ? mean[c] : 0.f;
            cf[3 * 256 * V + c] = in ? invstd[c] : 0.f;
        }
        __syncthreads();
    }
    const int nrows = B * H;
    const bool z_aligned = V == 4 && (reinterpret_cast<uintptr_t>(z) & 15) == 0 && (cs_z & 3) == 0;
    const bool g_aligned = V == 4 && BWD && (reinterpret_cast<uintptr_t>(gy + c_off) & 15) == 0 && (cs_gy & 3) == 0;
    for (int row = blockIdx.x; row < nrows; row += gridDim.x) {
        const int b = row / H, y = row - b * H + 1;
        const size_t base = ((size_t)(b * R + y) * P + 1);
        for (int x = pl; active && x < W; x += ppi) {
            float zz[V];
            VecIO<V>::load_nt(z + (base + x) * cs_z + V * cg, zz, z_aligned);
            if (!BWD) {
#pragma unroll
                for (int e = 0; e < V; ++e) { s0[e] += zz[e]; s1[e] += (double)zz[e] * zz[e]; }
            } else {
                float gg[V];
                VecIO<V>::load_nt(gy + (base + x) * cs_gy + c_off + V * cg, gg, g_aligned);
#pragma unroll
                for (int h = 0; h < V; h += 2) {
                    asm volatile("" ::: "memory");
#pragma unroll
                    for (int e = h; e < h + 2 && e < V; ++e) {
                        const float sc = cf[0 * 256 * V + V * cg + e], sh = cf[1 * 256 * V + V * cg + e];
                        const float u = fmaf(zz[e], sc, sh);
                        gg[e] = u > 0.f ? gg[e] : 0.f;
                    }
                }
#pragma unroll
                for (int h = 0; h < V; h += 2) {
                    asm volatile("" ::: "memory");
#pragma unroll
                    for (int e = h; e < h + 2 && e < V; ++e) {
                        const float mu = cf[2 * 256 * V + V * cg + e], iv = cf[3 * 256 * V + V * cg + e];
                        s0[e] += gg[e];
                        s1[e] += (double)gg[e] * (double)((zz[e] - mu) * iv);
                    }
                }
            }
        }
    }
    __syncthreads();
#pragma unroll
    for (int e = 0; e < V; ++e) { red[0][tid][e] = s0[e]; red[1][tid][e] = s1[e]; }
    __syncthreads();
    if (tid < cvn) {
#pragma unroll
        for (int e = 0; e < V; ++e) {
            double a0 = 0, a1 = 0;
            for (int p = 0; p < ppi; ++p) { a0 += red[0][p * cvn + tid][e]; a1 += red[1][p * cvn + tid][e]; }
            const int c = V * tid + e;
            if (c < C) {
                partial[((size_t)blockIdx.x * 2 + 0) * C + c] = a0;
                partial[((size_t)blockIdx.x * 2 + 1) * C + c] = a1;
            }
        }
    }
}

template <int V>
__global__ __launch_bounds__(256) void bn_reduce_kernel(const float *__restrict__ z, int cs_z, const float *__restrict__ gy, int cs_gy,
                                                        int c_off, const float *__restrict__ scale, const float *__restrict__ shift,
                                                        const float *__restrict__ mean, const float *__restrict__ invstd, int C,
                                                        double *__restrict__ partial, int B, int H, int W)
{
    bn_reduce_body<false, V>(z, cs_z, gy, cs_gy, c_off, scale, shift, mean, invstd, C, partial, B, H, W);
}

__global__ __launch_bounds__(256)
void bn_reduce_bwd_kernel(const float *__restrict__ z, int cs_z, const float *__restrict__ gy, int cs_gy, int c_off,
                          const float *__restrict__ scale, const float *__restrict__ shift, const float *__restrict__ mean,
                          const float *__restrict__ invstd, int C, double *__restrict__ partial, int B, int H, int W)
{
    bn_reduce_body<true, 4>(z, cs_z, gy, cs_gy, c_off, scale, shift, mean, invstd, C, partial, B, H, W);
}

__device__ __forceinline__ void reduce_partials(const double *__restrict__ partial, int nblocks, int C, int c,
                                                double &s0, double &s1)
{
    double a = 0, b = 0;
    for (int blk = threadIdx.x; blk < nblocks; blk += 64) {
        a += partial[((size_t)blk * 2 + 0) * C + c];
        b += partial[((size_t)blk * 2 + 1) * C + c];
    }
    for (int off = 32; off > 0; off >>= 1) {
        a += __shfl_down(a, off, 64);
        b += __shfl_down(b, off, 64);
    }
    s0 = a; s1 = b;
}

__global__ __launch_bounds__(64) void bn_stats_finalize_kernel(const double *__restrict__ partial, int nblocks, int C,
                                                               double n, const float *__restrict__ gamma,
                                                               const float *__restrict__ beta, float *running_mean,
                                                               float *running_var, double momentum, double eps,
                                                               float *save_mean, float *save_invstd, float *scale,
                                                               float *shift)
{
    const int c = blockIdx.x;
    double s, ss;
    reduce_partials(partial, nblocks, C, c, s, ss);
    if (threadIdx.x != 0) return;
    const double mean = s / n;
    double var = ss / n - mean * mean;
    if (var < 0) var = 0;
    const double invstd = 1.0 / sqrt(var + eps);
    const float meanf = (float)mean, invf = (float)invstd;
    save_mean[c] = meanf;
    save_invstd[c] = invf;
    if (running_mean) {
        const double unb = n > 1 ? var * n / (n - 1) : var;
        running_mean[c] = (float)((1.0 - momentum) * running_mean[c] + momentum * mean);
        running_var[c] = (float)((1.0 - momentum) * running_var[c] + momentum * unb);
    }
    const float sc = (gamma ? gamma[c] : 1.f) * invf;
    scale[c] = sc;
    shift[c] = (beta ? beta[c] : 0.f) - meanf * sc;
}

__global__ void bn_coeffs_eval_kernel(const float *gamma, const float *beta, const float *rm, const float *rv,
                                      double eps, float *scale, float *shift, int C)
{
    const int c = blockIdx.x * blockDim.x + threadIdx.x;
    if (c >= C) return;
    const float sc = (float)((double)(gamma ? gamma[c] : 1.f) * (1.0 / sqrt((double)rv[c] + eps)));
    scale[c] = sc;
    shift[c] = fmaf(-rm[c], sc, beta ? beta[c] : 0.f);
}

__global__ __launch_bounds__(64) void bn_bwd_finalize_kernel(const double *__restrict__ partial, int nblocks, int C,
                                                             double n, const float *__restrict__ gamma,
                                                             const float *__restrict__ invstd, float *dgamma,
                                                             float *dbeta, int accumulate, float *coef)
{
    const int c = blockIdx.x;
    double sg, sgx;
    reduce_partials(partial, nblocks, C, c, sg, sgx);
    if (threadIdx.x != 0) return;
    if (dgamma) dgamma[c] = accumulate ? dgamma[c] + (float)sgx : (float)sgx;
    if (dbeta) dbeta[c] = accumulate ? dbeta[c] + (float)sg : (float)sg;
    const double k1 = (double)(gamma ? gamma[c] : 1.f) * invstd[c];
    coef[c] = (float)k1;
    coef[C + c] = (float)(k1 * sg / n);
    coef[2 * C + c] = (float)(k1 * (double)invstd[c] * sgx / n);
}

__global__ void fold_bn_kernel(const float *__restrict__ w, const float *__restrict__ b,
                               const float *__restrict__ scale, const float *__restrict__ shift,
                               float *__restrict__ w_out, float *__restrict__ b_out, int Cout, int per_co)
{
    const long long total = (long long)Cout * per_co;
    for (long long i = blockIdx.x * (long long)blockDim.x + threadIdx.x; i < total;
         i += (long long)gridDim.x * blockDim.x) {
        const int co = (int)(i / per_co);
        w_out[i] = w[i] * scale[co];
        if (i % per_co == 0) b_out[co] = fmaf(b ? b[co] : 0.f, scale[co], shift[co]);
    }
}

template <int MODE, int V>
__global__ __launch_bounds__(256) void bn_rows_kernel(const float *__restrict__ z, int cs_z,
                                                      const float *__restrict__ gy, int cs_gy, int c_off_gy,
                                                      const float *__restrict__ scale,
                                                      const float *__restrict__ shift,
                                                      const float *__restrict__ mean,
                                                      const float *__restrict__ coef, int C,
                                                      float *__restrict__ out, int cs_out, int c_off_out,
                                                      int C_store, int H, int W, float *__restrict__ amax, int nrows)
{
    extern __shared__ float coefs[];
    const int P = W + GRID_PAD, R = H + GRID_PAD;
    const int cvn = (C_store + V - 1) / V;
    const int Cpad = cvn * V;
    for (int c = threadIdx.x; c < Cpad; c += blockDim.x) {
        const bool ok = c < C;
        coefs[c] = ok ? scale[c] : 0.f;
        coefs[Cpad + c] = ok ? shift[c] : 0.f;
        if (MODE == 1) {
            coefs[2 * Cpad + c] = ok ? mean[c] : 0.f;
            coefs[3 * Cpad + c] = ok ? coef[c] : 0.f;
            coefs[4 * Cpad + c] = ok ? coef[C + c] : 0.f;
            coefs[5 * Cpad + c] = ok ? coef[2 * C + c] : 0.f;
        }
    }
    __syncthreads();
    const int dx = 256 / cvn, dc = 256 - dx * cvn;
    for (int row = blockIdx.x; row < nrows; row += gridDim.x) {
    const int y = row % R;
    const size_t base = (size_t)row * P;
    const bool row_in = (y >= 1 && y <= H);
    int x = threadIdx.x / cvn, cg = threadIdx.x - x * cvn;
    float mx = 0.f;
    for (; x < P; x += dx, cg += dc) {
        if (cg >= cvn) { cg -= cvn; ++x; if (x >= P) break; }
        float o[V];
#pragma unroll
        for (int k = 0; k < V; ++k) o[k] = 0.f;
        if (row_in && x >= 1 && x <= W && V * cg < C) {
            float zz[V], gg[V];
            VecIO<V>::load_nt(z + (base + x) * cs_z + V * cg, zz);
            if (MODE == 1) VecIO<V>::load_nt(gy + (base + x) * cs_gy + c_off_gy + V * cg, gg);
#pragma unroll
            for (int k = 0; k < V; ++k) {
                const int c = V * cg + k;
                const float u = fmaf(zz[k], coefs[c], coefs[Cpad + c]);
                if (MODE == 0) {
                    o[k] = fmaxf(u, 0.f);
                } else {
                    const float g = u > 0.f ? gg[k] : 0.f;
                    o[k] = coefs[3 * Cpad + c] * g - coefs[4 * Cpad + c] - coefs[5 * Cpad + c] * (zz[k] - coefs[2 * Cpad + c]);
                }
            }
        }
#pragma unroll
        for (int k = 0; k < V; ++k) mx = fmaxf(mx, fabsf(o[k]));
        float *op = out + (base + x) * cs_out + c_off_out + V * cg;
        if (V * cg + V - 1 < C_store) {
            VecIO<V>::store_nt(op, o);
        } else {
#pragma unroll
            for (int k = 0; k < V; ++k)
                if (V * cg + k < C_store) op[k] = o[k];
        }
    }
    if (amax) mmlf_amax_update_row(mx, amax, row);
    }
}

template <int V>
__global__ __launch_bounds__(256) void relu_slice_rows_kernel(const float *__restrict__ src, int cs_src, int c_off,
                                                              const float *__restrict__ ref, int cs_ref, int ref_off, int C,
                                                              float *__restrict__ dst, int cs_dst, int H, int W,
                                                              float *__restrict__ amax, int nrows)
{
    const int P = W + GRID_PAD, R = H + GRID_PAD;
    const int cvn = cs_dst / V;
    const int dx = 256 / cvn, dc = 256 - dx * cvn;
    for (int row = blockIdx.x; row < nrows; row += gridDim.x) {
        const int y = row % R;
        const size_t base = (size_t)row * P;
        const bool row_in = (y >= 1 && y <= H);
        int x = threadIdx.x / cvn, cg = threadIdx.x - x * cvn;
        float mx = 0.f;
        for (; x < P; x += dx, cg += dc) {
            if (cg >= cvn) { cg -= cvn; ++x; if (x >= P) break; }
            float o[V];
#pragma unroll
            for (int k = 0; k < V; ++k) o[k] = 0.f;
            if (row_in && x >= 1 && x <= W && V * cg < C) {
                const float *sp = src + (base + x) * cs_src + c_off + V * cg;
                const float *rp = ref + (base + x) * cs_ref + ref_off + V * cg;
                float rr[V];
                if (V * cg + V - 1 < C) {
                    VecIO<V>::load_nt(sp, o);
                    VecIO<V>::load_nt(rp, rr);
                } else {
#pragma unroll
                    for (int k = 0; k < V; ++k) {
                        const bool in = V * cg + k < C;
                        o[k] = in ? sp[k] : 0.f;
                        rr[k] = in ? rp[k] : 0.f;
                    }
                }
#pragma unroll
                for (int k = 0; k < V; ++k) o[k] = rr[k] > 0.f ? o[k] : 0.f;
            }
#pragma unroll
            for (int k = 0; k < V; ++k) mx = fmaxf(mx, fabsf(o[k]));
            VecIO<V>::store_nt(dst + (base + x) * cs_dst + V * cg, o);
        }
        if (amax) mmlf_amax_update_row(mx, amax, row);
    }
}

struct BnApply4 { const float *z[4]; const float *scale[4]; const float *shift[4]; };
__global__ __launch_bounds__(256) void bn_apply4_kernel(BnApply4 s, int cs_z, int C, float *__restrict__ out,
                                                        int H, int W, float *__restrict__ amax, int nrows)
{
    extern __shared__ float coefs[];
    const int P = W + GRID_PAD, R = H + GRID_PAD;
    const int C4 = 4 * C, half = C / 2, cvn = 2 * C;
    for (int c = threadIdx.x; c < C4; c += blockDim.x) {
        const int k = c / C, cl = c - k * C;
        const float *sc = k == 0 ? s.scale[0] : k == 1 ? s.scale[1] : k == 2 ? s.scale[2] : s.scale[3];
        const float *sh = k == 0 ? s.shift[0] : k == 1 ? s.shift[1] : k == 2 ? s.shift[2] : s.shift[3];
        coefs[c] = sc[cl];
        coefs[C4 + c] = sh[cl];
    }
    __syncthreads();
    const int dx = 256 / cvn, dc = 256 - dx * cvn;
    for (int row = blockIdx.x; row < nrows; row += gridDim.x) {
// ... 793 lines not shown
        }
        mean[idx] = means[(size_t)bi * total + idx];
        logvar[idx] = best;
        for (int k = 0; k < S; ++k) {
            const float gk = grid[k];
            float acc = 0.f;
            for (int j = 0; j < S; ++j)
                acc = __fadd_rn(acc, laplace_pdf(gk, means[(size_t)j * total + idx],
                                                 expf(logvars[(size_t)j * total + idx])));
            post[(b * S + k) * HW + p] = __fdiv_rn(acc, (float)S);
        }
    }
}

__device__ __forceinline__ double cdf_laplace_f64(double x, double m, double v)
{
    const double z = (x - m) / v;
    return x < m ? exp(z) / 2.0 : 1.0 - exp(-z) / 2.0;
}

__global__ void lmm_to_discrete_kernel(const float *__restrict__ means, const float *__restrict__ logvars,
                                       const double *__restrict__ edges, double *__restrict__ out, int S, int B,
                                       int n_bins, long long HW)
{
    const long long total = (long long)B * n_bins * HW;
    for (long long idx = blockIdx.x * (long long)blockDim.x + threadIdx.x; idx < total;
         idx += (long long)gridDim.x * blockDim.x) {
        const long long p = idx % HW;
        const long long r = idx / HW;
        const int k = (int)(r % n_bins);
        const long long b = r / n_bins;
        const double e0 = edges[k], e1 = edges[k + 1];
        double acc = 0.0;
        for (int s = 0; s < S; ++s) {
            const size_t o = ((size_t)s * B + b) * HW + p;
            const double m = (double)means[o];
            const double v = (double)expf(logvars[o]);
            acc += cdf_laplace_f64(e1, m, v) - cdf_laplace_f64(e0, m, v);
        }
        out[idx] = acc / (double)S;
    }
}

static int ew_blocks(long long total, int per = 256)
{
    long long b = (total + per - 1) / per;
    if (b > 8192) b = 8192;
    if (b < 1) b = 1;
    return (int)b;
}

extern "C" int mmlf_bn_stats_train(const float *z, int cs, int C, const float *gamma, const float *beta,
                                   float *running_mean, float *running_var, double momentum, double eps,
                                   float *save_mean, float *save_invstd, float *scale, float *shift,
                                   double *partial, int nblocks, int B, int H, int W, void *stream)
{
    MMLF_CHECK_ARG(z && save_mean && save_invstd && scale && shift && partial, "mmlf_bn_stats_train: null pointer");
    MMLF_CHECK_ARG(cs % 4 == 0 && C > 0 && C <= cs && (C + 3) / 4 <= 256, "mmlf_bn_stats_train: C=%d cs=%d", C, cs);
    MMLF_CHECK_ARG(nblocks > 0 && nblocks <= 4096, "mmlf_bn_stats_train: nblocks=%d", nblocks);
    MMLF_CHECK_ARG(B > 0 && H > 0 && W > 0, "mmlf_bn_stats_train: bad shape B=%d H=%d W=%d", B, H, W);
    hipStream_t st = (hipStream_t)stream;
    hipLaunchKernelGGL((bn_reduce_kernel<4>), dim3(nblocks), dim3(256), 0, st, z, cs, nullptr, 0, 0, nullptr,
                       nullptr, nullptr, nullptr, C, partial, B, H, W);
    const double n = (double)B * H * W;
    hipLaunchKernelGGL(bn_stats_finalize_kernel, dim3(C), dim3(64), 0, st, partial, nblocks, C, n, gamma,
                       beta, running_mean, running_var, momentum, eps, save_mean, save_invstd, scale, shift);
    return mmlf_launch_status("mmlf_bn_stats_train");
}

extern "C" int mmlf_bn_stats_finalize(const double *partial, int nblocks, int C, const float *gamma,
                                      const float *beta, float *running_mean, float *running_var, double momentum,
                                      double eps, float *save_mean, float *save_invstd, float *scale, float *shift,
                                      int B, int H, int W, void *stream)
{
    MMLF_CHECK_ARG(partial && save_mean && save_invstd && scale && shift && C > 0 && nblocks > 0,
                   "mmlf_bn_stats_finalize: bad argument");
    MMLF_CHECK_ARG(B > 0 && H > 0 && W > 0, "mmlf_bn_stats_finalize: bad shape B=%d H=%d W=%d", B, H, W);
    hipLaunchKernelGGL(bn_stats_finalize_kernel, dim3(C), dim3(64), 0, (hipStream_t)stream, partial, nblocks, C,
                       (double)B * H * W, gamma, beta, running_mean, running_var, momentum, eps, save_mean,
                       save_invstd, scale, shift);
    return mmlf_launch_status("mmlf_bn_stats_finalize");
}

extern "C" int mmlf_bn_coeffs_eval(const float *gamma, const float *beta, const float *rm, const float *rv,
                                   double eps, float *scale, float *shift, int C, void *stream)
{
    MMLF_CHECK_ARG(rm && rv && scale && shift && C > 0, "mmlf_bn_coeffs_eval: bad argument");
    hipLaunchKernelGGL(bn_coeffs_eval_kernel, dim3((C + 63) / 64), dim3(64), 0, (hipStream_t)stream, gamma, beta, rm,
                       rv, eps, scale, shift, C);
    return mmlf_launch_status("mmlf_bn_coeffs_eval");
}

static int fold_bn_eval(const char *who, int taps, const float *w_oihw, const float *bias, const float *scale,
                        const float *shift, float *w_out, float *bias_out, int Cout, int Cin, void *stream)
{
    MMLF_CHECK_ARG(w_oihw && scale && shift && w_out && bias_out && Cout > 0 && Cin > 0, "%s: bad argument", who);
    const long long total = (long long)Cout * Cin * taps;
    hipLaunchKernelGGL(fold_bn_kernel, dim3(ew_blocks(total)), dim3(256), 0, (hipStream_t)stream, w_oihw, bias, scale,
                       shift, w_out, bias_out, Cout, Cin * taps);
    return mmlf_launch_status(who);
}

extern "C" int mmlf_fold_bn_eval(const float *w_oihw, const float *bias, const float *scale, const float *shift,
                                 float *w_out, float *bias_out, int Cout, int Cin, void *stream)
{
    return fold_bn_eval("mmlf_fold_bn_eval", 4, w_oihw, bias, scale, shift, w_out, bias_out, Cout, Cin, stream);
}

extern "C" int mmlf_fold_bn_eval3x3(const float *w_oihw, const float *bias, const float *scale, const float *shift,
                                    float *w_out, float *bias_out, int Cout, int Cin, void *stream)
{
    return fold_bn_eval("mmlf_fold_bn_eval3x3", 9, w_oihw, bias, scale, shift, w_out, bias_out, Cout, Cin, stream);
}

extern "C" int mmlf_bn_apply_relu(const float *z, int cs_z, int C, const float *scale, const float *shift, float *y,
                                  int cs_y, int c_off, int C_store, int B, int H, int W, float *amax_out,
                                  void *stream)
{
    MMLF_CHECK_ARG(z && scale && shift && y, "mmlf_bn_apply_relu: null pointer");
    MMLF_CHECK_ARG(cs_z % 4 == 0 && cs_y % 2 == 0 && c_off % 2 == 0 && c_off >= 0 && C > 0 && C <= cs_z && C_store >= C &&
                       c_off + C_store <= cs_y,
                   "mmlf_bn_apply_relu: C=%d cs_z=%d cs_y=%d c_off=%d C_store=%d", C, cs_z, cs_y, c_off, C_store);
    MMLF_CHECK_ARG(B > 0 && H > 0 && W > 0, "mmlf_bn_apply_relu: bad shape B=%d H=%d W=%d", B, H, W);
    const int nrows = B * (H + GRID_PAD);
    hipLaunchKernelGGL((bn_rows_kernel<0, 4>), dim3(nrows), dim3(256), 6 * (C_store + 4) * sizeof(float), (hipStream_t)stream, z, cs_z,
                       nullptr, 0, 0, scale, shift, nullptr, nullptr, C, y, cs_y, c_off, C_store, H, W, amax_out, nrows);
    return mmlf_launch_status("mmlf_bn_apply_relu");
}

extern "C" int mmlf_bn_apply_relu4(const float *const z[4], int cs_z, int C, const float *const scale[4],
                                   const float *const shift[4], float *y, int cs_y, int B, int H, int W,
                                   float *amax_out, void *stream)
{
    MMLF_CHECK_ARG(z && scale && shift && y && B > 0 && H > 0 && W > 0, "mmlf_bn_apply_relu4: bad argument");
    MMLF_CHECK_ARG(C > 0 && C % 2 == 0 && C <= cs_z && cs_z % 2 == 0 && cs_y == 4 * C && 8 * C * sizeof(float) <= 48 * 1024,
                   "mmlf_bn_apply_relu4: C=%d cs_z=%d cs_y=%d (needs even C, cs_y == 4 * C)", C, cs_z, cs_y);
    BnApply4 s;
    for (int k = 0; k < 4; ++k) {
        MMLF_CHECK_ARG(z[k] && scale[k] && shift[k], "mmlf_bn_apply_relu4: null pointer in source %d", k);
        s.z[k] = z[k]; s.scale[k] = scale[k]; s.shift[k] = shift[k];
    }
    const int nrows = B * (H + GRID_PAD);
    hipLaunchKernelGGL(bn_apply4_kernel, dim3(nrows), dim3(256), 8 * C * sizeof(float), (hipStream_t)stream, s, cs_z, C,
                       y, H, W, amax_out, nrows);
    return mmlf_launch_status("mmlf_bn_apply_relu4");
}

extern "C" int mmlf_bn_bwd_reduce(const float *gy, int cs_gy, int c_off, const float *z, int cs_z, int C,
                                  const float *scale, const float *shift, const float *gamma,
                                  const float *save_mean, const float *save_invstd, float *dgamma, float *dbeta,
                                  int accumulate, float *coef, double *partial, int nblocks, int B, int H, int W,
                                  void *stream)
{
    MMLF_CHECK_ARG(gy && z && scale && shift && save_mean && save_invstd && coef && partial,
                   "mmlf_bn_bwd_reduce: null pointer");
    MMLF_CHECK_ARG(cs_gy % 2 == 0 && c_off % 2 == 0 && c_off >= 0 && cs_z % 4 == 0 && C > 0 && C <= cs_z &&
                       c_off + C <= cs_gy && (C + 3) / 4 <= 128,
                   "mmlf_bn_bwd_reduce: layout C=%d cs_z=%d cs_gy=%d c_off=%d", C, cs_z, cs_gy, c_off);
    MMLF_CHECK_ARG(nblocks > 0 && nblocks <= 4096, "mmlf_bn_bwd_reduce: nblocks=%d", nblocks);
    MMLF_CHECK_ARG(B > 0 && H > 0 && W > 0, "mmlf_bn_bwd_reduce: bad shape B=%d H=%d W=%d", B, H, W);
    hipStream_t st = (hipStream_t)stream;
    hipLaunchKernelGGL(bn_reduce_bwd_kernel, dim3(nblocks), dim3(256), 0, st, z, cs_z, gy, cs_gy, c_off,
                       scale, shift, save_mean, save_invstd, C, partial, B, H, W);
    hipLaunchKernelGGL(bn_bwd_finalize_kernel, dim3(C), dim3(64), 0, st, partial, nblocks, C,
                       (double)B * H * W, gamma, save_invstd, dgamma, dbeta, accumulate, coef);
    return mmlf_launch_status("mmlf_bn_bwd_reduce");
}

extern "C" int mmlf_bn_bwd_apply(const float *gy, int cs_gy, int c_off, const float *z, int cs_z, int C,
                                 const float *scale, const float *shift, const float *save_mean, const float *coef,
                                 float *dz, int cs_dz, int B, int H, int W, float *amax_out, void *stream)
{
    MMLF_CHECK_ARG(gy && z && scale && shift && save_mean && coef && dz, "mmlf_bn_bwd_apply: null pointer");
    MMLF_CHECK_ARG(cs_gy % 2 == 0 && c_off % 2 == 0 && c_off >= 0 && cs_z % 4 == 0 && cs_dz % 4 == 0 && C > 0 && C <= cs_z &&
                       C <= cs_dz && c_off + C <= cs_gy,
                   "mmlf_bn_bwd_apply: layout C=%d cs_z=%d cs_dz=%d cs_gy=%d c_off=%d", C, cs_z, cs_dz, cs_gy, c_off);
    MMLF_CHECK_ARG(B > 0 && H > 0 && W > 0, "mmlf_bn_bwd_apply: bad shape B=%d H=%d W=%d", B, H, W);
    const int nrows = B * (H + GRID_PAD);
    hipLaunchKernelGGL((bn_rows_kernel<1, 4>), dim3(nrows), dim3(256), 6 * (cs_dz + 4) * sizeof(float), (hipStream_t)stream, z, cs_z, gy,
                       cs_gy, c_off, scale, shift, save_mean, coef, C, dz, cs_dz, 0, cs_dz, H, W, amax_out, nrows);
    return mmlf_launch_status("mmlf_bn_bwd_apply");
}

static int relu_bwd_slice_args(const char *who, int cs_src, int c_off, int cs_ref, int ref_off, int C, int cs_dst, int B, int H,
                               int W)
{
    MMLF_CHECK_ARG(cs_src > 0 && cs_src % 2 == 0 && c_off % 2 == 0 && c_off >= 0 && cs_dst > 0 && cs_dst % 4 == 0 && C > 0 &&
                       C <= cs_dst && c_off + C <= cs_src && (C + 3) / 4 <= 128 && cs_dst / 4 <= 256,
                   "%s: layout C=%d cs_src=%d c_off=%d cs_dst=%d", who, C, cs_src, c_off, cs_dst);
    MMLF_CHECK_ARG(cs_ref > 0 && cs_ref % 2 == 0 && ref_off % 2 == 0 && ref_off >= 0 && ref_off + C <= cs_ref,
                   "%s: layout C=%d cs_ref=%d ref_off=%d", who, C, cs_ref, ref_off);
    MMLF_CHECK_ARG(B > 0 && H > 0 && W > 0, "%s: bad shape B=%d H=%d W=%d", who, B, H, W);
    return 0;
}

extern "C" int mmlf_relu_bwd_slice(const float *src, int cs_src, int c_off, const float *ref, int cs_ref, int ref_off, int C,
                                   float *dst, int cs_dst, int B, int H, int W, float *amax_out, void *stream)
{
    MMLF_CHECK_ARG(src && ref && dst, "mmlf_relu_bwd_slice: null pointer");
    if (relu_bwd_slice_args("mmlf_relu_bwd_slice", cs_src, c_off, cs_ref, ref_off, C, cs_dst, B, H, W)) return 1;
    const int nrows = B * (H + GRID_PAD);
    hipLaunchKernelGGL((relu_slice_rows_kernel<4>), dim3(nrows), dim3(256), 0, (hipStream_t)stream, src, cs_src, c_off, ref,
                       cs_ref, ref_off, C, dst, cs_dst, H, W, amax_out, nrows);
    return mmlf_launch_status("mmlf_relu_bwd_slice");
}

extern "C" int mmlf_audit_relu_bwd_slice(int cs_src, int c_off, int cs_ref, int ref_off, int C, int cs_dst, int B, int H, int W,
                                         int64_t *ends )
{
    MMLF_CHECK_ARG(ends, "mmlf_audit_relu_bwd_slice: null pointer");
    if (relu_bwd_slice_args("mmlf_audit_relu_bwd_slice", cs_src, c_off, cs_ref, ref_off, C, cs_dst, B, H, W)) return 1;
    const Grid g = make_grid(B, H, W);
    const long long q_last = ((long long)(B - 1) * g.R + H) * g.P + W;
    ends[MMLF_AUDIT_SLICE_SRC] = (q_last * cs_src + c_off + C) * 4;
    ends[MMLF_AUDIT_SLICE_REF] = (q_last * cs_ref + ref_off + C) * 4;
    ends[MMLF_AUDIT_SLICE_DST] = g.NQ * cs_dst * 4;
    ends[MMLF_AUDIT_SLICE_AMAX] = (MMLF_AMAX_HEAD + (long long)B * g.R) * 4;
    return 0;
}

extern "C" int mmlf_pack_nchw(const float *nchw, int C, float *grid, int cs, int B, int H, int W, float *amax_out,
                              void *stream)
{
    MMLF_CHECK_ARG(nchw && grid && C > 0 && cs % 4 == 0 && C <= cs, "mmlf_pack_nchw: C=%d cs=%d", C, cs);
    MMLF_CHECK_ARG(B > 0 && H > 0 && W > 0, "mmlf_pack_nchw: bad shape B=%d H=%d W=%d", B, H, W);
    int xt = PACK_XT;
    constexpr size_t tile_limit = 32 * 1024;
    while (xt > 4 && (size_t)cs * (xt | 1) * sizeof(float) > tile_limit) xt >>= 1;
    const size_t lds = (size_t)cs * (xt | 1) * sizeof(float);
    MMLF_CHECK_ARG(lds <= 64 * 1024, "mmlf_pack_nchw: cs=%d does not fit the transpose tile", cs);
    hipLaunchKernelGGL(pack_nchw_kernel, dim3(B * (H + GRID_PAD)), dim3(256), lds, (hipStream_t)stream, nchw, C, grid, cs, H, W,
                       amax_out, xt);
    return mmlf_launch_status("mmlf_pack_nchw");
}

__global__ void zero_slack_kernel(float *__restrict__ buf, long long head, long long tail_off, long long tail,
                                  float *__restrict__ amax, long long n_amax)
{
    for (long long i = blockIdx.x * (long long)blockDim.x + threadIdx.x; i < head + tail + n_amax;
         i += (long long)gridDim.x * blockDim.x) {
        if (i < head + tail) buf[i < head ? i : tail_off + (i - head)] = 0.f;
        else amax[i - head - tail] = 0.f;
    }
}

static int zero_slack_impl(float *grid, int cs, int B, int H, int W, float *amax, int ksize, void *stream)
{
    MMLF_CHECK_ARG(grid && cs > 0 && B > 0 && H > 0 && W > 0, "mmlf_zero_slack: bad argument");
    const Grid g = make_grid(B, H, W);
    const long long head = (long long)(g.P + 1) * cs, tail_off = g.NQ * cs;
    const long long tail = ((ksize == 3 ? grid_alloc_positions_k3(g) : grid_alloc_positions(g)) - g.NQ) * cs;
    const long long n_amax = amax ? amax_entries(g) : 0;
    hipLaunchKernelGGL(zero_slack_kernel, dim3(ew_blocks(head + tail + n_amax)), dim3(256), 0, (hipStream_t)stream, grid,
                       head, tail_off, tail, amax, n_amax);
    return mmlf_launch_status("mmlf_zero_slack");
}

extern "C" int mmlf_zero_slack(float *grid, int cs, int B, int H, int W, float *amax, void *stream)
{
    return zero_slack_impl(grid, cs, B, H, W, amax, 2, stream);
}

extern "C" int mmlf_zero_slack_k3(float *grid, int cs, int B, int H, int W, float *amax, void *stream)
{
    return zero_slack_impl(grid, cs, B, H, W, amax, 3, stream);
}

struct ZeroSlack4 { float *buf[4]; float *amax[4]; long long head[4], tail_off[4], tail[4], end[4]; long long n_amax; };
__global__ void zero_slack4_kernel(ZeroSlack4 z)
{
    for (long long i = blockIdx.x * (long long)blockDim.x + threadIdx.x; i < z.end[3]; i += (long long)gridDim.x * blockDim.x) {
        const int k = i < z.end[0] ? 0 : i < z.end[1] ? 1 : i < z.end[2] ? 2 : 3;
        const long long j = i - (k ? z.end[k - 1] : 0);
        if (j < z.head[k] + z.tail[k]) z.buf[k][j < z.head[k] ? j : z.tail_off[k] + (j - z.head[k])] = 0.f;
        else z.amax[k][j - z.head[k] - z.tail[k]] = 0.f;
    }
}

static int zero_slack4_impl(float *const grid[4], const int cs[4], float *const amax[4], int B, int H, int W, int ksize,
                            void *stream)
{
    MMLF_CHECK_ARG(grid && cs && amax && B > 0 && H > 0 && W > 0, "mmlf_zero_slack4: bad argument");
    const Grid g = make_grid(B, H, W);
    ZeroSlack4 z;
    long long run = 0;
    for (int k = 0; k < 4; ++k) {
        z.buf[k] = grid[k]; z.amax[k] = amax[k];
        z.head[k] = z.tail_off[k] = z.tail[k] = 0;
        if (grid[k]) {
            MMLF_CHECK_ARG(cs[k] > 0, "mmlf_zero_slack4: cs[%d]=%d", k, cs[k]);
            z.head[k] = (long long)(g.P + 1) * cs[k];
            z.tail_off[k] = g.NQ * cs[k];
            z.tail[k] = ((ksize == 3 ? grid_alloc_positions_k3(g) : grid_alloc_positions(g)) - g.NQ) * cs[k];
            run += z.head[k] + z.tail[k] + (amax[k] ? amax_entries(g) : 0);
        }
        z.end[k] = run;
    }
    z.n_amax = amax_entries(g);
    if (run == 0) return 0;
    hipLaunchKernelGGL(zero_slack4_kernel, dim3(ew_blocks(run)), dim3(256), 0, (hipStream_t)stream, z);
    return mmlf_launch_status("mmlf_zero_slack4");
}

extern "C" int mmlf_zero_slack4(float *const grid[4], const int cs[4], float *const amax[4], int B, int H, int W, void *stream)
{
    return zero_slack4_impl(grid, cs, amax, B, H, W, 2, stream);
}

extern "C" int mmlf_zero_slack4_k3(float *const grid[4], const int cs[4], float *const amax[4], int B, int H, int W,
                                   void *stream)
{
    return zero_slack4_impl(grid, cs, amax, B, H, W, 3, stream);
}

extern "C" int mmlf_unpack_nchw(const float *grid, int cs, float *nchw, int C, int B, int H, int W, void *stream)
{
    MMLF_CHECK_ARG(nchw && grid && C > 0 && C <= cs && cs % 4 == 0, "mmlf_unpack_nchw: C=%d cs=%d", C, cs);
    MMLF_CHECK_ARG(B > 0 && H > 0 && W > 0, "mmlf_unpack_nchw: bad shape B=%d H=%d W=%d", B, H, W);
// ... 206 lines not shown
```

### mmlf_amd/engine.py

```python
import ctypes
import os
import threading

import torch

from . import _lib
from ._lib import call, ptr

VAR_IDENTITY, VAR_TRANSPOSE, VAR_TRANSPOSE_FLIPH = 0, 1, 2
BN_BLOCKS = 1024
LOSS_BLOCKS = 1024


def cs_of(c):
    return (c + 7) // 8 * 8


class Geometry:

    def __init__(self, B, H, W, ksize=2):
        self.B, self.H, self.W = B, H, W
        self.ksize = ksize
        self.P, self.R = W + int(_lib.load().mmlf_grid_pad_w()), H + int(_lib.load().mmlf_grid_pad_h())
        self.G = self.P * self.R
        self.NQ = B * self.G
        self.alloc = int(_lib.load().mmlf_grid_alloc_positions_k3(B, H, W) if ksize == 3
                         else _lib.load().mmlf_grid_alloc_positions(B, H, W))
        self.amax_n = int(_lib.load().mmlf_amax_entries(B, H, W))
        self.amax_head = int(_lib.load().mmlf_amax_head())
        self.amax_stride = int(_lib.load().mmlf_amax_shard_stride())
        if self.alloc * 288 * 4 >= 2 ** 63 or self.NQ + 2 * self.P + 600 >= 2 ** 31:
            raise ValueError('batch x image too large for 32-bit grid positions')

    def buf(self, cs, device):
        t = torch.empty(self.alloc * cs, dtype=torch.float32, device=device)
        t.absmax = torch.empty(self.amax_n, dtype=torch.float32, device=device)
        call('mmlf_zero_slack_k3' if self.ksize == 3 else 'mmlf_zero_slack', ptr(t), cs, self.B, self.H, self.W, ptr(t.absmax),
             _lib.stream_ptr())
        return t

    def bufs(self, css, device):
        assert 1 <= len(css) <= 4
        ts = []
        for cs in css:
            t = torch.empty(self.alloc * cs, dtype=torch.float32, device=device)
            t.absmax = torch.empty(self.amax_n, dtype=torch.float32, device=device)
            ts.append(t)
        n = len(ts)
        grid = (ctypes.c_void_p * 4)(*([ptr(t) for t in ts] + [None] * (4 - n)))
        amax = (ctypes.c_void_p * 4)(*([ptr(t.absmax) for t in ts] + [None] * (4 - n)))
        csa = (ctypes.c_int * 4)(*(list(css) + [0] * (4 - n)))
        call('mmlf_zero_slack4_k3' if self.ksize == 3 else 'mmlf_zero_slack4', grid, csa, amax, self.B, self.H, self.W,
             _lib.stream_ptr())
        return ts

    def relu_mask(self, device):
        n = int(_lib.load().mmlf_relu_mask_words(self.B, self.H, self.W))
        return torch.empty(n, dtype=torch.int32, device=device)

    def amax_of(self, t, cs):
        rows = t[:self.NQ * cs].view(self.B * self.R, self.P * cs).abs().amax(1)
        out = torch.zeros(self.amax_n, dtype=torch.float32, device=t.device)
        out[0] = rows.max()
        out[self.amax_head:self.amax_head + rows.numel()] = rows
        return out

    def amax_canonical(self, a):
        out = a.clone()
        out[:self.amax_head] = 0
        out[0] = a[:self.amax_head].max()
        return out


class _Workspace:
    _tls = threading.local()

    @classmethod
    def get(cls, device):
        table = cls._tls.__dict__.setdefault('table', {})
        key = (device.type, device.index)
        ws = table.get(key)
        if ws is None:
            ws = table[key] = cls(device)
        return ws

    def __init__(self, device):
        self.device = device
        self.wgrad = None
        self.wgrad_side = None
        self.side = torch.cuda.Stream(device=device) if device.type == 'cuda' else None
        self.partial = torch.empty(2 * 512 * max(BN_BLOCKS, LOSS_BLOCKS) + 8, dtype=torch.float64, device=device)

    def packed_filters(self, items):
        import numpy as np
        lib = _lib.load()
        sig = tuple((w.data_ptr(), w.shape[0], w.shape[1], int(var), int(dg)) for _, w, var, dg in items)
        self.enter_stream()
        caches = self.__dict__.setdefault('_packs', {})
        cache = caches.get(sig)
        if cache is None:
            if len(caches) >= 4:
                caches.clear()
            desc = np.zeros(len(items), dtype=np.dtype([('w', '<u8'), ('packed', '<u8'), ('Cout', '<i4'), ('Cin', '<i4'),
                                                         ('variant', '<i4'), ('dgrad', '<i4'), ('col0', '<i4'), ('np', '<i4')]))
            offs, total, col = [], 0, 0
            for i, (_, w, var, dg) in enumerate(items):
                cout, cin = w.shape[0], w.shape[1]
                K, N = (cout, cin) if dg else (cin, cout)
                nbytes = int(lib.mmlf_packed_filter_h2_bytes(cs_of(K), N))
                npk = int(lib.mmlf_packed_filter_h2_columns(N))
                if nbytes < 0 or npk < 0:
                    raise RuntimeError(f'pack_filters: unsupported channels K={K} N={N}')
                offs.append((total, nbytes))
                desc[i] = (w.data_ptr(), 0, cout, cin, int(var), int(dg), col, npk)
                total += (nbytes + 255) // 256 * 256
                col += npk
            store = torch.empty(total, dtype=torch.uint8, device=self.device)
            for i, (o, _) in enumerate(offs):
                desc['packed'][i] = store.data_ptr() + o
            table = torch.from_numpy(desc.view(np.uint8).copy()).to(self.device)
            views = [store[o:o + n].view(torch.float32) for o, n in offs]
            cache = caches[sig] = (sig, table, store, views, col)
        _, table, _, views, col = cache
        call('mmlf_pack_filters_h2', ptr(table), len(items), col, _lib.stream_ptr())
        return {key: v for (key, _, _, _), v in zip(items, views)}

    def enter_stream(self):
        if self.device.type != 'cuda':
            return
        cur = torch.cuda.current_stream(self.device)
        last = self.__dict__.get('_last_stream')
        if last is not None and last != cur:
            cur.wait_event(last.record_event())
        self._last_stream = cur

    def scratch(self, name, n):
        if not name.endswith('_side'):
            self.enter_stream()
        t = getattr(self, name, None)
        if t is None or t.numel() < n:
            t = torch.empty(n, dtype=torch.float32, device=self.device)
            setattr(self, name, t)
        return t

    def wgrad_ws(self, geo, cin, cout, side=False):
        query = _lib.load().mmlf_wgrad3x3_workspace_floats if geo.ksize == 3 else _lib.load().mmlf_wgrad_workspace_floats
        n = int(query(cin, cout, geo.B, geo.H, geo.W))
        if n < 0:
            raise RuntimeError(f'wgrad: unsupported channels {cin}->{cout}')
        name = 'wgrad_side' if side else 'wgrad'
        if not side:
            self.enter_stream()
        if getattr(self, name) is None or getattr(self, name).numel() < n:
            setattr(self, name, torch.empty(n, dtype=torch.float32, device=self.device))
        return getattr(self, name)


CONV_MODE = os.environ.get('MMLF_CONV_MODE', 'f16x3')
_PACK = {'f16x3': ('mmlf_packed_filter_h2_bytes', 1, 'mmlf_pack_filter_h2'),
         'bf16x6': ('mmlf_packed_filter_split_bytes', 1, 'mmlf_pack_filter_split'),
         'f32': ('mmlf_packed_filter_floats', 4, 'mmlf_pack_filter')}
_PACK3 = ('mmlf_packed_filter3x3_floats', 4, 'mmlf_pack_filter3x3')


def _pack(who, query, unit, entry, w, variant, dgrad):
    cout, cin = w.shape[0], w.shape[1]
    K, N = (cout, cin) if dgrad else (cin, cout)
    n = int(getattr(_lib.load(), query)(cs_of(K), N))
    if n < 0:
        raise RuntimeError(f'{who}: unsupported channels K={K} N={N}')
    out = torch.empty(n * unit // 4, dtype=torch.float32, device=w.device)
    call(entry, ptr(w), ptr(out), cout, cin, variant, int(dgrad), _lib.stream_ptr())
    return out


def pack_filter(w, variant, dgrad):
    return _pack('pack_filter', *_PACK.get(CONV_MODE, _PACK['f32']), w, variant, dgrad)


PROFILE = None


def _tic():
    e0, e1 = torch.cuda.Event(enable_timing=True), torch.cuda.Event(enable_timing=True)
    e0.record()
    return e0, e1


def _toc(events, tag, flops, nbytes):
    events[1].record()
    PROFILE.append((tag, flops, events[0], events[1], nbytes))


def _amax_of(geo, t, cs):
    a = getattr(t, 'absmax', None)
    if a is None:
        return geo.amax_of(t, cs)
    if CHECK_ABSMAX:
        true = geo.amax_of(t, cs)
        c = geo.amax_canonical(a)
        exact = geo.P >= 32
        bad = (c != true) if exact else (c < true)
        bad[0] = c[0] != true[0]
        if bool(bad.any()):
            k = int(bad.nonzero()[0])
            raise AssertionError(f'amax entry {k} holds {float(c[k])!r}, true max |x| is {float(true[k])!r}')
    return a


CHECK_ABSMAX = bool(os.environ.get('MMLF_CHECK_ABSMAX'))
OVERLAP_WGRAD = os.environ.get('MMLF_OVERLAP_WGRAD', '1') not in ('', '0')


CHECK_EXTENTS = bool(os.environ.get('MMLF_CHECK_EXTENTS'))
EXTENT_CHECKS = 0


def _audit(entry, scalars, n_ends, kind, have):
    global EXTENT_CHECKS
    ends = (ctypes.c_int64 * n_ends)()
    call(entry, *scalars, ends)
    for name, (k, t, off) in have.items():
        if t is None:
            continue
        got = t.untyped_storage().nbytes() - t.storage_offset() * t.element_size() - 4 * off
        if ends[k] > got:
            raise RuntimeError(f'MMLF_CHECK_EXTENTS: {kind}: the launch may touch {ends[k]} bytes behind `{name}`, '
                               f'the tensor has {got}')
    EXTENT_CHECKS += 1


def relu_bwd_slice(geo, src, cs_src, c_off, ref, cs_ref, ref_off, C, dst, cs_dst):
    amax = getattr(dst, 'absmax', None)
    if CHECK_EXTENTS:
        _audit('mmlf_audit_relu_bwd_slice', (cs_src, c_off, cs_ref, ref_off, C, cs_dst, geo.B, geo.H, geo.W), 4,
               f'relu_bwd_slice C={C} {cs_src}+{c_off} B={geo.B} {geo.H}x{geo.W}',
               {'src': (0, src, 0), 'ref': (1, ref, 0), 'dst': (2, dst, 0), 'amax': (3, amax, 0)})
    call('mmlf_relu_bwd_slice', ptr(src), cs_src, c_off, ptr(ref), cs_ref, ref_off, C, ptr(dst), cs_dst, geo.B, geo.H, geo.W,
         ptr(amax), _lib.stream_ptr())


THIN_MAX_N, THIN_MIN_K = 2, 64


def wgrad(geo, x, cs_in, cin, g, cs_g, cout, g_shift, gw, gb, variant, workspace, side=False):
    if cout <= THIN_MAX_N and cin >= THIN_MIN_K and cs_in <= 512:
        ws = _Workspace.get(x.device).scratch('thin_wgrad_side' if side else 'thin_wgrad', int(_lib.load().mmlf_conv2x2_wgrad_thin_workspace_floats(cin)))
        call('mmlf_conv2x2_wgrad_thin', ptr(x), cs_in, cin, ptr(g), cs_g, cout, g_shift, ptr(gw), ptr(gb), variant, 1,
             ptr(ws), geo.B, geo.H, geo.W, _lib.stream_ptr())
        return
    args = (ptr(x), cs_in, cin, ptr(g), cs_g, cout, g_shift, ptr(gw), ptr(gb), variant, 1, ptr(workspace),
            geo.B, geo.H, geo.W)
    prof = PROFILE is not None and cin >= 256 and cout >= 256
    if prof:
        events = _tic()
    if CONV_MODE == 'f16x3':
        ax, ag = _amax_of(geo, x, cs_in), _amax_of(geo, g, cs_g)
        if CHECK_EXTENTS:
            _audit('mmlf_audit_wgrad_h2', (cs_in, cin, cs_g, cout, g_shift, geo.B, geo.H, geo.W), 7,
                   f'wgrad {cin}->{cout} B={geo.B} {geo.H}x{geo.W} g_shift={g_shift}',
                   {'in': (0, x, 0), 'g': (1, g, 0), 'gw': (2, gw, 0), 'gb': (3, gb, 0), 'workspace': (4, workspace, 0),
                    'in_amax': (5, ax, 0), 'g_amax': (6, ag, 0)})
        call('mmlf_conv2x2_wgrad_h2', *args, ptr(ax), ptr(ag), _lib.stream_ptr())
    else:
        call('mmlf_conv2x2_wgrad_split' if CONV_MODE == 'bf16x6' else 'mmlf_conv2x2_wgrad', *args, _lib.stream_ptr())
    if prof:
        vh, vw = (geo.H + 1, geo.W + 1) if g_shift == 0 else (geo.H, geo.W)
        nbytes = 4.0 * geo.B * (cin * (geo.H * geo.W if g_shift == 0 else (geo.H + 1) * (geo.W + 1)) + cout * vh * vw)
        _toc(events, 'wgrad_side' if side else 'wgrad', 2.0 * geo.B * vh * vw * cout * 4 * cin, nbytes)


def conv(geo, x, cs_in, K, packed, bias, N, out, cs_out, out_shift, vh, vw, relu, ref=None, cs_ref=0,
         n_store=None, out_off=0, bn_partial=None, mask_out=None, mask_in=None, w_master=None, variant=0):
    aout = getattr(out, 'absmax', None)
    if (w_master is not None and N <= THIN_MAX_N and K >= THIN_MIN_K and cs_in <= 512 and ref is None and mask_in is None
            and mask_out is None and bn_partial is None and out_off == 0 and n_store in (None, cs_out)):
        ws = _Workspace.get(x.device).scratch('thin_fwd', int(_lib.load().mmlf_conv2x2_thin_workspace_floats(geo.B, geo.H, geo.W)))
        call('mmlf_conv2x2_thin', ptr(x), cs_in, K, ptr(w_master), ptr(bias), N, ptr(out), cs_out, out_shift, vh, vw,
             geo.B, geo.H, geo.W, int(relu), variant, ptr(ws), ptr(aout), _lib.stream_ptr())
        return
    n_store = cs_out if n_store is None else n_store
    prof = PROFILE is not None and ((K >= 256 and N >= 256) or (K == N and 64 <= K < 128))
    if prof:
        events = _tic()
    args = (ptr(x), cs_in, K, ptr(packed), ptr(bias), N, ptr(out) + 4 * out_off, cs_out, n_store, out_shift, vh, vw,
            geo.B, geo.H, geo.W, int(relu), ptr(ref), cs_ref)
    if CONV_MODE == 'f16x3':
        ax = _amax_of(geo, x, cs_in)
        if CHECK_EXTENTS:
            _audit('mmlf_audit_conv_h2', (cs_in, K, N, cs_out, n_store, out_shift, cs_ref, geo.B, geo.H, geo.W), 9,
                   f'conv {K}->{N} B={geo.B} {geo.H}x{geo.W} shift={out_shift}',
                   {'in': (0, x, 0), 'packed': (1, packed, 0), 'bias': (2, bias, 0), 'out': (3, out, out_off),
                    'ref': (4, ref, 0), 'in_amax': (5, ax, 0), 'out_amax': (6, aout, 0), 'bn_partial': (7, bn_partial, 0),
                    'mask_out': (8, mask_out, 0), 'mask_in': (8, mask_in, 0)})
        call('mmlf_conv2x2_h2', *args, ptr(ax), ptr(aout), ptr(bn_partial), ptr(mask_out), ptr(mask_in), _lib.stream_ptr())
    else:
        call('mmlf_conv2x2_split' if CONV_MODE == 'bf16x6' else 'mmlf_conv2x2', *args, _lib.stream_ptr())
    if prof:
        nbytes = 4.0 * geo.B * (K * (geo.H * geo.W if out_shift == 0 else (geo.H + 1) * (geo.W + 1)) + N * vh * vw)
        _toc(events, 'conv' if K >= 256 else 'conv70', 2.0 * geo.B * vh * vw * N * 4 * K, nbytes)



def pack_filter3(w, variant, dgrad):
    return _pack('pack_filter3', *_PACK3, w, variant, dgrad)


def conv3(geo, x, cs_in, K, packed, bias, N, out, cs_out, relu, ref=None, cs_ref=0, n_store=None, out_off=0):
    n_store = cs_out if n_store is None else n_store
    if CHECK_EXTENTS:
        _audit('mmlf_audit_conv3x3', (cs_in, K, N, cs_out, n_store, cs_ref if ref is not None else 0, geo.B, geo.H, geo.W), 5,
               f'conv3x3 {K}->{N} B={geo.B} {geo.H}x{geo.W}',
               {'in': (0, x, 0), 'packed': (1, packed, 0), 'bias': (2, bias, 0), 'out': (3, out, out_off), 'ref': (4, ref, 0)})
    prof = PROFILE is not None and K >= 256 and N >= 256
    if prof:
        events = _tic()
    call('mmlf_conv3x3', ptr(x), cs_in, K, ptr(packed), ptr(bias), N, ptr(out) + 4 * out_off, cs_out, n_store,
         geo.B, geo.H, geo.W, int(relu), ptr(ref), cs_ref, _lib.stream_ptr())
    if prof:
        nbytes = 4.0 * geo.B * geo.H * geo.W * (K + N)
        _toc(events, 'conv3x3', 2.0 * geo.B * geo.H * geo.W * N * 9 * K, nbytes)


def wgrad3(geo, x, cs_in, cin, g, cs_g, cout, gw, gb, variant, workspace):
    if CHECK_EXTENTS:
        _audit('mmlf_audit_wgrad3x3', (cs_in, cin, cs_g, cout, geo.B, geo.H, geo.W), 5,
               f'wgrad3x3 {cin}->{cout} B={geo.B} {geo.H}x{geo.W}',
               {'in': (0, x, 0), 'g': (1, g, 0), 'gw': (2, gw, 0), 'gb': (3, gb, 0), 'workspace': (4, workspace, 0)})
    call('mmlf_conv3x3_wgrad', ptr(x), cs_in, cin, ptr(g), cs_g, cout, ptr(gw), ptr(gb), variant, 1, ptr(workspace),
         geo.B, geo.H, geo.W, _lib.stream_ptr())


class BlockSpec:

    def __init__(self, prefix, cin, cout, bn):
        self.prefix, self.cin, self.cout, self.bn = prefix, cin, cout, bn


class _Rec:
    __slots__ = ('spec', 'var', 'x', 'cs_x', 'x_relu', 'xmask', 'y', 'ymask', 'z', 'scale', 'shift', 'smean', 'sinv', 'eval')

    def __init__(self, spec, var, x, cs_x, x_relu, xmask, y, ymask, z):
        self.spec, self.var, self.x, self.cs_x, self.x_relu, self.xmask = spec, var, x, cs_x, x_relu, xmask
        self.y, self.ymask, self.z = y, ymask, z
        self.scale = self.shift = self.smean = self.sinv = None
        self.eval = False


class Trunk:

    def __init__(self, chs, in_blocks, out_blocks, views, oc, momentum, eps=1e-5, ksize=2, batchnorm=True):
        if ksize not in (2, 3):
            raise ValueError(f'native trunk: ksize {ksize} (2 or 3)')
        if not batchnorm and ksize != 2:
            raise ValueError('native trunk: blocks without BatchNorm run on the 2x2 kernels only')
        self.batchnorm = bn = bool(batchnorm)
        self.ksize = ksize
        self.chs, self.views, self.oc = chs, views, oc
        self.momentum, self.eps = float(momentum), float(eps)
        cin0 = views * 3
        self.streams = []
        for key, net, var in (('h', 'in_net_hv', VAR_TRANSPOSE), ('v', 'in_net_hv', VAR_IDENTITY),
                              ('i', 'in_net_id', VAR_TRANSPOSE_FLIPH), ('d', 'in_net_id', VAR_IDENTITY)):
            blocks = [BlockSpec(f'{net}.0', cin0, chs, bn)]
            blocks += [BlockSpec(f'{net}.{k}', chs, chs, bn) for k in range(1, in_blocks)]
            self.streams.append((key, var, blocks))
        c = 4 * chs
        self.out_blocks = [BlockSpec(f'out_net.{k}', c, c, bn) for k in range(out_blocks - 1)]
        self.out_blocks.append(BlockSpec(f'out_net.{out_blocks - 1}', c, oc, None))
        if chs % 2 or cs_of(c) != c:
            raise ValueError('native trunk needs an even model_chs with 4*model_chs a multiple of 8')

    def _prepack(self, p, dev, with_dgrad):
        if CONV_MODE != 'f16x3' or dev.type != 'cuda' or self.ksize != 2:
            return {}
        items = []

        def add(name, var, dgrad):
            items.append(((name, var, dgrad), p[name], var, dgrad))

        def block(spec, var, first):
            thin = spec.cout <= THIN_MAX_N and spec.cin >= THIN_MIN_K
            if not thin:
                add(f'{spec.prefix}.0.weight', var, False)
            add(f'{spec.prefix}.2.weight', var, False)
            if with_dgrad:
                add(f'{spec.prefix}.2.weight', var, True)
                if not first:
                    add(f'{spec.prefix}.0.weight', var, True)

        for _, var, blocks in self.streams:
            for k, spec in enumerate(blocks):
                block(spec, var, k == 0)
        for spec in self.out_blocks:
            block(spec, VAR_IDENTITY, False)
        return _Workspace.get(dev).packed_filters(items)

    def _pack(self, w, var, dgrad):
        return (pack_filter3 if self.ksize == 3 else pack_filter)(w, var, dgrad)

    def _packed(self, packs, p, name, var, dgrad):
        pk = packs.get((name, var, dgrad))
        return pk if pk is not None else self._pack(p[name], var, dgrad)

    def _conv(self, geo, second, x, cs_in, K, packed, bias, N, out, cs_out, relu, ref=None, cs_ref=0, n_store=None, out_off=0,
              **only2x2):
        if self.ksize == 3:
            assert all(v is None for v in only2x2.values()), only2x2
            conv3(geo, x, cs_in, K, packed, bias, N, out, cs_out, relu, ref=ref, cs_ref=cs_ref, n_store=n_store, out_off=out_off)
            return
        out_shift, vh, vw = (geo.P + 1, geo.H, geo.W) if second else (0, geo.H + 1, geo.W + 1)
        conv(geo, x, cs_in, K, packed, bias, N, out, cs_out, out_shift, vh, vw, relu, ref=ref, cs_ref=cs_ref, n_store=n_store,
             out_off=out_off, **only2x2)

    def _dgrad(self, geo, second, g, cs_g, K, packed, N, dx, cs_dx, **relu_of):
        self._conv(geo, not second, g, cs_g, K, packed, None, N, dx, cs_dx, False, **relu_of)

    def _wgrad(self, geo, second, x, cs_in, cin, g, cs_g, cout, gw, gb, var, side=False):
        ws = _Workspace.get(x.device).wgrad_ws(geo, cin, cout, side=side)
        if self.ksize == 3:
            wgrad3(geo, x, cs_in, cin, g, cs_g, cout, gw, gb, var, ws)
        else:
            wgrad(geo, x, cs_in, cin, g, cs_g, cout, geo.P + 1 if second else 0, gw, gb, var, ws, side=side)

    def _block_fwd(self, geo, spec, var, x, cs_x, x_relu, xmask, p, train, rec_list, out=None, cs_out=None, c_off=0, packs=None,
                   tracked=None, deferred=None):
        dev = x.device
        ws = _Workspace.get(dev)
        B, H, W = geo.B, geo.H, geo.W
        C, cs_mid = spec.cout, cs_of(spec.cout)
        pre = spec.prefix
        w1, b1, w2, b2 = p[f'{pre}.0.weight'], p[f'{pre}.0.bias'], p[f'{pre}.2.weight'], p[f'{pre}.2.bias']
        packs = packs or {}
        save = rec_list is not None
        f16 = CONV_MODE == 'f16x3' and self.ksize == 2
        thin = C <= THIN_MAX_N and spec.cin >= THIN_MIN_K and self.ksize == 2
        bits = save and f16 and not thin
        folded = spec.bn is True and not train and not save
        relu2 = spec.bn is False or folded
        fused_stats = spec.bn is True and train and f16
        new_out = spec.bn is not None and out is None
        pk1 = None if thin else self._packed(packs, p, f'{pre}.0.weight', var, False)
        if spec.bn is False:
            pk2 = self._packed(packs, p, f'{pre}.2.weight', var, False)
        got = geo.bufs([cs_mid] * ((1 if relu2 else 2) + (1 if new_out else 0)), dev)
        y = got[0]
        z = None if relu2 else got[1]
        if new_out:
            out, cs_out, c_off = got[-1], cs_mid, 0
        ymask = geo.relu_mask(dev) if bits else None
        omask = geo.relu_mask(dev) if bits and relu2 and new_out else None
        head = {'w_master': w1, 'variant': var} if thin else {}
        self._conv(geo, False, x, cs_x, spec.cin, pk1, b1, C, y, cs_mid, True, mask_out=ymask, **head)
        if folded:
            coef = torch.empty(2 * C, dtype=torch.float32, device=dev)
            call('mmlf_bn_coeffs_eval', ptr(p[f'{pre}.3.weight']), ptr(p[f'{pre}.3.bias']), ptr(p[f'{pre}.3.running_mean']),
                 ptr(p[f'{pre}.3.running_var']), self.eps, ptr(coef), ptr(coef[C:]), C, _lib.stream_ptr())
            w2f, b2f = torch.empty_like(w2), torch.empty_like(b2)
            call('mmlf_fold_bn_eval3x3' if self.ksize == 3 else 'mmlf_fold_bn_eval', ptr(w2), ptr(b2), ptr(coef), ptr(coef[C:]),
                 ptr(w2f), ptr(b2f), C, C, _lib.stream_ptr())
            pk2, b2 = self._pack(w2f, var, False), b2f
        elif spec.bn is not False:
            pk2 = self._packed(packs, p, f'{pre}.2.weight', var, False)
        rec = None
        if save:
            rec = _Rec(spec, var, x, cs_x, x_relu, xmask, y, ymask, z)
            rec_list.append(rec)
        if relu2:
            self._conv(geo, True, y, cs_mid, C, pk2, b2, C, out, cs_out, True, n_store=cs_out if new_out else C, out_off=c_off,
                       mask_out=omask)
            return out, cs_out, omask
        self._conv(geo, True, y, cs_mid, C, pk2, b2, C, z, cs_mid, False, bn_partial=ws.partial if fused_stats else None)
        if spec.bn is None:
            return z, cs_mid, None
        coef = torch.empty(4 * C, dtype=torch.float32, device=dev)
        scale, shift, smean, sinv = coef[:C], coef[C:2 * C], coef[2 * C:3 * C], coef[3 * C:]
        g, bt = p[f'{pre}.3.weight'], p[f'{pre}.3.bias']
        rm, rv = p[f'{pre}.3.running_mean'], p[f'{pre}.3.running_var']
        if train:
            if fused_stats:
                nblk = int(_lib.load().mmlf_conv2x2_blocks(C, C, B, H, W))
                call('mmlf_bn_stats_finalize', ptr(ws.partial), nblk, C, ptr(g), ptr(bt), ptr(rm), ptr(rv),
                     self.momentum, self.eps, ptr(smean), ptr(sinv), ptr(scale), ptr(shift), B, H, W,
                     _lib.stream_ptr())
            else:
                call('mmlf_bn_stats_train', ptr(z), cs_mid, C, ptr(g), ptr(bt), ptr(rm), ptr(rv), self.momentum,
                     self.eps, ptr(smean), ptr(sinv), ptr(scale), ptr(shift), ptr(ws.partial), BN_BLOCKS, B, H, W,
                     _lib.stream_ptr())
            if tracked is None:
                p[f'{pre}.3.num_batches_tracked'].add_(1)
            else:
                tracked.append(p[f'{pre}.3.num_batches_tracked'])
        else:
            call('mmlf_bn_coeffs_eval', ptr(g), ptr(bt), ptr(rm), ptr(rv), self.eps, ptr(scale), ptr(shift), C,
                 _lib.stream_ptr())
            if save:
                smean.copy_(rm)
                sinv.copy_(torch.rsqrt(rv.double() + self.eps).float())
                rec.eval = True
        if deferred is not None:
            deferred.append((z, scale, shift))
        else:
            call('mmlf_bn_apply_relu', ptr(z), cs_mid, C, ptr(scale), ptr(shift), ptr(out), cs_out, c_off,
                 cs_out if new_out else C, B, H, W, ptr(out.absmax), _lib.stream_ptr())
        if save:
            rec.scale, rec.shift, rec.smean, rec.sinv = scale, shift, smean, sinv
        return out, cs_out, None

    def forward(self, p, stacks, train, save, packed=None):
        if packed is not None:
            geo, xs_in = packed
            B, H, W = geo.B, geo.H, geo.W
            dev = xs_in[0].device
            cin0 = self.views * 3
        else:
            h = stacks[0]
            B, n, c, H, W = h.shape
            dev = h.device
            geo = Geometry(B, H, W, self.ksize)
            cin0 = n * c
        _Workspace.get(dev).enter_stream()
        packs = self._prepack(p, dev, save)
        tracked = []
        tape = {'geo': geo, 'streams': [], 'out': [], 'packs': packs}
        if packed is not None:
            concat, xs = geo.buf(4 * self.chs, dev), list(xs_in)
        else:
            concat, *xs = geo.bufs([4 * self.chs] + [cs_of(cin0)] * 3, dev)
            xs.append(geo.buf(cs_of(cin0), dev))
        fold = not train and not save
        deferred = [] if (not fold and self.chs % 2 == 0 and all(b[-1].bn for _, _, b in self.streams)) else None
        for s, (key, var, blocks) in enumerate(self.streams):
            x = xs[s]
            if packed is None:
                call('mmlf_pack_nchw', ptr(stacks[s]), cin0, ptr(x), cs_of(cin0), B, H, W, ptr(x.absmax), _lib.stream_ptr())
            cs_x = cs_of(cin0)
            recs = []
            x_relu, xmask = False, None
            for k, spec in enumerate(blocks):
                last = k == len(blocks) - 1
                x, cs_x, xmask = self._block_fwd(geo, spec, var, x, cs_x, x_relu, xmask, p, train, recs if save else None,
                                                 out=concat if last else None, cs_out=4 * self.chs, c_off=s * self.chs,
                                                 packs=packs, tracked=tracked, deferred=deferred if last else None)
                x_relu = spec.bn is False
            tape['streams'].append(recs)
        if deferred:
            arr = lambda k: (ctypes.c_void_p * 4)(*[ptr(d[k]) for d in deferred])
            call('mmlf_bn_apply_relu4', arr(0), cs_of(self.chs), self.chs, arr(1), arr(2), ptr(concat), 4 * self.chs,
                 B, H, W, ptr(concat.absmax), _lib.stream_ptr())
            del deferred[:]
        if save and not self.batchnorm:
            tape['concat'] = concat
        x, cs_x, x_relu, xmask = concat, 4 * self.chs, False, None
        for spec in self.out_blocks:
            x, cs_x, xmask = self._block_fwd(geo, spec, VAR_IDENTITY, x, cs_x, x_relu, xmask, p, train,
                                             tape['out'] if save else None, packs=packs, tracked=tracked)
            x_relu = spec.bn is False
        if tracked:
            counts = {}
            for t in tracked:
                counts.setdefault(t.data_ptr(), [t, 0])[1] += 1
            torch._foreach_add_([t for t, _ in counts.values()], [n for _, n in counts.values()])
        out = torch.empty((B, self.oc, H, W), dtype=torch.float32, device=dev)
        call('mmlf_unpack_nchw', ptr(x), cs_x, ptr(out), self.oc, B, H, W, _lib.stream_ptr())
        return out, (tape if save else None)

    def _block_bwd(self, geo, rec, p, grads, gy, cs_gy, c_off, need_dx, after_bn=None, overlap=False, packs=None):
        spec, var = rec.spec, rec.var
        dev = gy.device
        ws = _Workspace.get(dev)
        B, H, W = geo.B, geo.H, geo.W
        C, cs_mid = spec.cout, cs_of(spec.cout)
        x, cs_x, y, z = rec.x, rec.cs_x, rec.y, rec.z
        pre = spec.prefix
        sp = _lib.stream_ptr
        packs = packs or {}
        f16 = CONV_MODE == 'f16x3' and self.ksize == 2
        gw1, gb1, gw2, gb2 = (grads[f'{pre}.{k}'] for k in ('0.weight', '0.bias', '2.weight', '2.bias'))

        y_relu = {'mask_in': rec.ymask} if rec.ymask is not None and f16 else {'ref': y, 'cs_ref': cs_mid}
        x_relu = {}
        if rec.x_relu:
            x_relu = {'mask_in': rec.xmask} if rec.xmask is not None and f16 else {'ref': x, 'cs_ref': cs_x}

        got = geo.bufs(([cs_mid] if spec.bn else []) + [cs_mid] + ([cs_x] if need_dx else []), dev)
        dy = got[1 if spec.bn else 0]
        dx = got[-1] if need_dx else None
        if spec.bn:
            coef = torch.empty(3 * C, dtype=torch.float32, device=dev)
            call('mmlf_bn_bwd_reduce', ptr(gy), cs_gy, c_off, ptr(z), cs_mid, C, ptr(rec.scale), ptr(rec.shift),
                 ptr(p[f'{pre}.3.weight']), ptr(rec.smean), ptr(rec.sinv), ptr(grads[f'{pre}.3.weight']),
                 ptr(grads[f'{pre}.3.bias']), 1, ptr(coef), ptr(ws.partial), BN_BLOCKS, B, H, W, sp())
            if rec.eval:
                coef[C:].zero_()
            dz = got[0]
            call('mmlf_bn_bwd_apply', ptr(gy), cs_gy, c_off, ptr(z), cs_mid, C, ptr(rec.scale), ptr(rec.shift),
                 ptr(rec.smean), ptr(coef), ptr(dz), cs_mid, B, H, W, ptr(dz.absmax), sp())
        else:
            assert c_off == 0 and cs_gy == cs_mid
            dz = gy
        if after_bn:
            after_bn()
        self._wgrad(geo, True, y, cs_mid, C, dz, cs_mid, C, gw2, gb2, var)
        self._dgrad(geo, True, dz, cs_mid, C, self._packed(packs, p, f'{pre}.2.weight', var, True), C, dy, cs_mid, **y_relu)
        del dz, got
        if overlap and need_dx:
            self._dgrad(geo, False, dy, cs_mid, C, self._packed(packs, p, f'{pre}.0.weight', var, True), spec.cin, dx, cs_x,
                        **x_relu)
            main = torch.cuda.current_stream()
            ready = main.record_event()
            with torch.cuda.stream(ws.side):
                ws.side.wait_event(ready)
                self._wgrad(geo, False, x, cs_x, spec.cin, dy, cs_mid, C, gw1, gb1, var, side=True)
                done = ws.side.record_event()
            return dx, done, (x, dy)
        self._wgrad(geo, False, x, cs_x, spec.cin, dy, cs_mid, C, gw1, gb1, var)
        if need_dx:
            self._dgrad(geo, False, dy, cs_mid, C, self._packed(packs, p, f'{pre}.0.weight', var, True), spec.cin, dx, cs_x,
                        **x_relu)
        return dx, None, None

    def backward(self, p, tape, grad_output, grads, on_done=None):
        geo = tape['geo']
        dev = grad_output.device
        _Workspace.get(dev).enter_stream()
        B, H, W = geo.B, geo.H, geo.W
        cs = cs_of(self.oc)
        g = geo.buf(cs, dev)
        call('mmlf_pack_nchw', ptr(grad_output.contiguous()), self.oc, ptr(g), cs, B, H, W, ptr(g.absmax),
             _lib.stream_ptr())
        cs_g = cs
        recs = tape['out']
        main = torch.cuda.current_stream()
        pending = None

        def settle():
            nonlocal pending
            if pending is not None:
                main.wait_event(pending[0])
                if on_done:
                    on_done(pending[1])
                pending = None

        while recs:
            rec = recs.pop()
            wide = OVERLAP_WGRAD and rec.spec.cin >= 128 and self.ksize == 2
            g, event, keep = self._block_bwd(geo, rec, p, grads, g, cs_g, 0, True, after_bn=settle, overlap=wide,
                                             packs=tape['packs'])
            settle()
            if event is not None:
                pending = (event, rec.spec.prefix, keep)
            elif on_done:
                on_done(rec.spec.prefix)
            cs_g = rec.cs_x
        for s in reversed(range(4)):
            recs = tape['streams'][s]
            if s == 2:
                settle()
            gs, cs_s, off = g, cs_g, s * self.chs
            if not self.batchnorm:
                cs_s, off = cs_of(self.chs), 0
                gs = geo.buf(cs_s, dev)
                relu_bwd_slice(geo, g, cs_g, s * self.chs, tape['concat'], cs_g, s * self.chs, self.chs, gs, cs_s)
            while recs:
                rec = recs.pop()
                gs, _, _ = self._block_bwd(geo, rec, p, grads, gs, cs_s, off, need_dx=bool(recs), packs=tape['packs'])
                cs_s, off = rec.cs_x, 0
            if on_done and s in (2, 0):
                on_done('in_net_id' if s == 2 else 'in_net_hv')
```

Measured before the change: 1133.

## Fuse BatchNorm-backward channel sums into the preceding dgrad conv epilogue

Adds an EPI_BN_BWD epilogue kind to the transposed conv epilogue. While storing dgrad output, it loads the lower block's pre-BN activations z, rebuilds the BN+ReLU gate, and accumulates per-channel sums of g and g*z through DPP row reductions and LDS atomics, writing per-block partials. The next block's BN backward reduce then reads these partials instead of making a separate pass over gy and z. This costs extra z loads, registers and LDS in the epilogue, and it applies only to narrow channel counts under specific geometry.

```diff
diff --git a/include/mmlf_hip.h b/include/mmlf_hip.h
--- a/include/mmlf_hip.h
+++ b/include/mmlf_hip.h
@@ -70,6 +70,8 @@
                     uint32_t *relu_mask_out , const uint32_t *relu_mask_in , void *stream);
 int64_t mmlf_relu_mask_words(int B, int H, int W);
 int mmlf_conv2x2_blocks(int K, int N, int B, int H, int W);
+
+enum { MMLF_RELU_BN_BWD_SUMS = 2 };
 
 int64_t mmlf_conv2x2_thin_workspace_floats(int B, int H, int W);
 int mmlf_conv2x2_thin(const float *in, int cs_in, int K, const float *w_oihw, const float *bias, int N,
diff --git a/mmlf_amd/csrc/conv.hip b/mmlf_amd/csrc/conv.hip
--- a/mmlf_amd/csrc/conv.hip
+++ b/mmlf_amd/csrc/conv.hip
@@ -59,6 +59,10 @@
     double *bn_partial;
     unsigned *relu_mask_out;
     const unsigned *relu_mask_in;
+    const float *bn_z, *bn_scale, *bn_shift;
+    double *bn_bwd_partial;
+    int cs_z;
+    long long z_bytes;
     long long out_bytes, ref_bytes;
     long long in_bytes, amax_n, mask_words;
 };
@@ -209,7 +213,8 @@
 
 
 
-enum { EPI_GENERIC = -1, EPI_PLAIN = 0, EPI_RELU = 1, EPI_STATS = 2, EPI_BITS_IN = 4, EPI_REF_IN = 8, EPI_MASK_OUT = 16 };
+enum { EPI_GENERIC = -1, EPI_PLAIN = 0, EPI_RELU = 1, EPI_STATS = 2, EPI_BITS_IN = 4, EPI_REF_IN = 8, EPI_MASK_OUT = 16,
+       EPI_BN_BWD = 32  };
 template <int G, int EPI>
 __device__ __forceinline__ void conv_epilogue16(const ConvArgs &a, const f32x4 (&acc)[2][G], long long Q0, int w,
                                                 int r16, int q4, float unscale_a, float &run_max,
@@ -325,15 +330,24 @@
     }
 }
 
+template <int CTRL>
+__device__ __forceinline__ float row_dpp(float x)
+{
+    return __uint_as_float((unsigned)__builtin_amdgcn_update_dpp(0, (int)__float_as_uint(x), CTRL, 0xF, 0xF, true));
+}
 template <int G> constexpr int tr_mask_words() { return (G + 7) / 8; }
 template <int G, int EPI>
 __device__ __forceinline__ void conv_epilogue16_tr(const ConvArgs &a, const f32x4 (&acc)[2][G], long long Q0, int w,
                                                    int r16, int q4, float unscale_a, float &run_max,
-                                                   const float *coef )
+                                                   const float *coef ,
+                                                   float *bn_acc = nullptr )
 {
     static_assert(EPI >= 0 && !(EPI & (EPI_STATS | EPI_REF_IN)), "kinds of the transposed epilogue");
+    static_assert(!(EPI & EPI_BN_BWD) || EPI == EPI_BN_BWD, "the BatchNorm-backward sums ride on the plain kind");
     constexpr int NP = 16 * G, MW = tr_mask_words<G>();
     constexpr bool do_relu = (EPI & EPI_RELU) != 0, mask_out = (EPI & EPI_MASK_OUT) != 0, use_bits = (EPI & EPI_BITS_IN) != 0;
+    constexpr bool bn_bwd = (EPI & EPI_BN_BWD) != 0;
+    constexpr int ZD = 3;
     const unsigned m = wave_row_mask(a, Q0, w, r16 + 16 * q4);
     const long long qb = Q0 + 32 * w + a.out_shift;
     const int ob_left = mmlf_records_left(a.out_bytes, qb * a.cs_out * 4ll);
@@ -357,15 +371,39 @@
     float mk[2] = {0.f, 0.f};
     const float *cl = coef + 4 * q4;
     f32x4 uw_n = *reinterpret_cast<const f32x4 *>(cl), b_n = *reinterpret_cast<const f32x4 *>(cl + NP);
+    __amdgpu_buffer_rsrc_t zb = ob;
+    unsigned lz = 0;
+    u32x4 zq[bn_bwd ? ZD : 1][2];
+    f32x4 sc_n = {}, sh_n = {};
+    if constexpr (bn_bwd) {
+        zb = __builtin_amdgcn_make_buffer_rsrc(const_cast<float *>(a.bn_z) + (size_t)qb * a.cs_z, 0,
+                                               mmlf_records_left(a.z_bytes, qb * a.cs_z * 4ll), MMLF_BUF_FLAGS);
+        lz = ((unsigned)r16 * a.cs_z + 4u * q4) * 4u;
+        asm volatile("" : "+v"(lz));
+#pragma unroll
+        for (int d = 0; d < ZD && d < G; ++d)
+#pragma unroll
+            for (int mb = 0; mb < 2; ++mb)
+                zq[d][mb] = (16 * d + 4 * q4 < a.n_store)
+                                ? __builtin_amdgcn_raw_buffer_load_b128(zb, lz + 64 * d, (unsigned)(16 * mb) * a.cs_z * 4u, 0)
+                                : u32x4{0u, 0u, 0u, 0u};
+        sc_n = *reinterpret_cast<const f32x4 *>(cl + 2 * NP);
+        sh_n = *reinterpret_cast<const f32x4 *>(cl + 3 * NP);
+    }
 #pragma unroll
     for (int nb = 0; nb < G; ++nb) {
         const int c0 = 16 * nb + 4 * q4;
-        const f32x4 uw4 = uw_n, b4 = b_n;
+        const f32x4 uw4 = uw_n, b4 = b_n, sc4 = sc_n, sh4 = sh_n;
         if (nb + 1 < G) {
             uw_n = *reinterpret_cast<const f32x4 *>(cl + 16 * (nb + 1));
             b_n = *reinterpret_cast<const f32x4 *>(cl + NP + 16 * (nb + 1));
+            if constexpr (bn_bwd) {
+                sc_n = *reinterpret_cast<const f32x4 *>(cl + 2 * NP + 16 * (nb + 1));
+                sh_n = *reinterpret_cast<const f32x4 *>(cl + 3 * NP + 16 * (nb + 1));
+            }
         }
         __builtin_amdgcn_sched_barrier(0);
+        float bs[8];
 #pragma unroll
         for (int mb = 0; mb < 2; ++mb) {
             u32x4 st;
@@ -382,11 +420,38 @@
                 if (mask_out) mw[mb][nb >> 3] |= (v > 0.f ? 1u : 0u) << (4 * (nb & 7) + r);
                 asm("v_max_f32 %0, %1, |%2|" : "=v"(mk[mb]) : "v"(mk[mb]), "v"(v));
                 st[r] = __float_as_uint(v);
+                if constexpr (bn_bwd) {
+                    const float z = ok[mb] ? __uint_as_float(zq[nb % ZD][mb][r]) : 0.f;
+                    const float g = fmaf(z, sc4[r], sh4[r]) > 0.f ? v : 0.f;
+                    bs[r] = mb ? bs[r] + g : g;
+                    bs[4 + r] = mb ? bs[4 + r] + g * z : g * z;
+                }
+            }
+            if constexpr (bn_bwd) {
+                if (nb + ZD < G)
+                    zq[nb % ZD][mb] = (16 * (nb + ZD) + 4 * q4 < a.n_store)
+                                          ? __builtin_amdgcn_raw_buffer_load_b128(zb, lz + 64 * (nb + ZD),
+                                                                                  (unsigned)(16 * mb) * a.cs_z * 4u, 0)
+                                          : u32x4{0u, 0u, 0u, 0u};
             }
             if (c0 < a.n_store) {
                 MMLF_OOB(OOB_OUT, (long long)lo + 64 * nb + (long long)(16 * mb) * a.cs_out * 4 + 12 >= ob_left);
                 __builtin_amdgcn_raw_buffer_store_b128(st, ob, lo + 64 * nb, (unsigned)(16 * mb) * a.cs_out * 4u, 0);
             }
+        }
+        if constexpr (bn_bwd) {
+            float y[4], t[2], u;
+#pragma unroll
+            for (int j = 0; j < 4; ++j)
+                y[j] = ((r16 & 8) ? bs[4 + j] : bs[j]) + row_dpp<0x140>((r16 & 8) ? bs[j] : bs[4 + j]);
+#pragma unroll
+            for (int j = 0; j < 2; ++j)
+                t[j] = ((r16 & 4) ? y[2 + j] : y[j]) + row_dpp<0x141>((r16 & 4) ? y[j] : y[2 + j]);
+            u = ((r16 & 2) ? t[1] : t[0]) + row_dpp<0x4E>((r16 & 2) ? t[0] : t[1]);
+            u += row_dpp<0xB1>(u);
+            if (!(r16 & 1))
+                __hip_atomic_fetch_add(bn_acc + (r16 >> 3) * NP + c0 + ((r16 >> 1) & 3), u, __ATOMIC_RELAXED,
+                                       __HIP_MEMORY_SCOPE_WAVEFRONT);
         }
         __builtin_amdgcn_sched_barrier(0);
     }
@@ -419,13 +484,19 @@
         }
     }
 }
-template <int NP>
+template <int NP, bool BN_BWD = false, int NW = 8>
 __device__ __forceinline__ void conv_fill_coef(const ConvArgs &a, float *coef, int tid, int nthreads)
 {
     for (int k = tid; k < NP; k += nthreads) {
         coef[k] = a.w_unscale ? a.w_unscale[k] : 1.f;
         coef[NP + k] = (a.bias && k < a.n_true) ? a.bias[k] : 0.f;
-    }
+        if constexpr (BN_BWD) {
+            coef[2 * NP + k] = k < a.n_true ? a.bn_scale[k] : 0.f;
+            coef[3 * NP + k] = k < a.n_true ? a.bn_shift[k] : 0.f;
+        }
+    }
+    if constexpr (BN_BWD)
+        for (int k = tid; k < NW * 2 * NP; k += nthreads) coef[4 * NP + k] = 0.f;
 }
 
 __device__ __forceinline__ float wave_operand_amax_gather(const ConvArgs &a, long long Q0, int w, int lane)
@@ -575,7 +646,9 @@
     if (tile >= ntiles) return;
     float *coef = reinterpret_cast<float *>(lds + D * BUF_F4);
     double *stats_all = reinterpret_cast<double *>(lds + D * BUF_F4);
-    if constexpr (TR) conv_fill_coef<NP>(late_args(), coef, tid, 64 * NW);
+    constexpr bool BN_BWD = EPI >= 0 && (EPI & EPI_BN_BWD) != 0;
+    float *bn_acc = coef + 4 * NP;
+    if constexpr (TR) conv_fill_coef<NP, BN_BWD, NW>(late_args(), coef, tid, 64 * NW);
     else if (late_args().bn_partial)
         for (int k = tid; k < NW * NP * 2; k += 64 * NW) stats_all[k] = 0.0;
     float scale_a = 1.f, unscale_a = 1.f, run_max = 0.f;
@@ -715,7 +788,8 @@
                 if (tile + (int)gridDim.x < ntiles)
                     next_amax = wave_operand_amax_gather(e, (long long)(tile + gridDim.x) * TILE, w, lane);
             if constexpr (TR)
-                conv_epilogue16_tr<G, EPI>(e, acc, (long long)tile * TILE, w, r16, q4, unscale_a, run_max, coef);
+                conv_epilogue16_tr<G, EPI>(e, acc, (long long)tile * TILE, w, r16, q4, unscale_a, run_max, coef,
+                                           BN_BWD ? bn_acc + w * 2 * NP : nullptr);
             else
                 conv_epilogue16<G, EPI>(e, acc, (long long)tile * TILE, w, r16, q4, unscale_a, run_max,
                                         e.bn_partial ? stats_all + (size_t)w * NP * 2 : nullptr);
@@ -750,7 +824,15 @@
     if constexpr (EARLY) __syncthreads();
     const ConvArgs e = late_args();
     if (e.out_amax) mmlf_amax_update(run_max, e.out_amax, blockIdx.x * NW + w);
-    if (e.bn_partial) {
+    if constexpr (BN_BWD) {
+        for (int k = tid; k < 2 * e.n_true; k += 64 * NW) {
+            const int ch = k % e.n_true, which = k / e.n_true;
+            float t = 0.f;
+#pragma unroll
+            for (int ww = 0; ww < NW; ++ww) t += bn_acc[(ww * 2 + which) * NP + ch];
+            e.bn_bwd_partial[((size_t)blockIdx.x * 2 + which) * e.n_true + ch] = (double)t;
+        }
+    } else if (e.bn_partial) {
         for (int k = tid; k < 2 * e.n_true; k += 64 * NW) {
             const int ch = k % e.n_true, which = k / e.n_true;
             double t = 0.0;
@@ -1225,7 +1307,9 @@
 {
     constexpr size_t lds_pipe = 2 * (2 * 640 + 4 * PL * G * 16) * sizeof(float4);
     constexpr size_t lds_stats = 8 * (G * 16) * 2 * sizeof(double);
-    constexpr size_t lds_coef = 2 * (G * 16) * sizeof(float);
+    constexpr bool BN_BWD = EPI >= 0 && (EPI & EPI_BN_BWD) != 0;
+    constexpr size_t lds_coef = (BN_BWD ? 4 + 2 * 8 : 2) * (G * 16) * sizeof(float);
+    constexpr size_t lds_coef16 = (BN_BWD ? 4 + 2 * 16 : 2) * (G * 16) * sizeof(float);
     static PerDeviceOnce attr_once;
     if (attr_once.run([] { return mmlf_allow_lds(reinterpret_cast<const void *>(conv4tap_x6s_kernel<G, PL, EPI, 8, TR>),
                                                  lds_pipe + (TR ? lds_coef : PL == 2 ? lds_stats : 0), "mmlf_conv2x2_h2"); }))
@@ -1236,9 +1320,9 @@
             constexpr size_t lds_pipe16 = RING16 * (2 * 640 + 4 * PL * G * 16) * sizeof(float4);
             static PerDeviceOnce attr_once16;
             if (attr_once16.run([] { return mmlf_allow_lds(reinterpret_cast<const void *>(conv4tap_x6s_kernel<G, PL, EPI, 16, TR>),
-                                                           lds_pipe16 + (TR ? lds_coef : lds_stats16), "mmlf_conv2x2_h2(16 waves)"); }))
+                                                           lds_pipe16 + (TR ? lds_coef16 : lds_stats16), "mmlf_conv2x2_h2(16 waves)"); }))
                 return 1;
-            const size_t lds16 = lds_pipe16 + (TR ? lds_coef : a.bn_partial ? lds_stats16 : 0);
+            const size_t lds16 = lds_pipe16 + (TR ? lds_coef16 : a.bn_partial ? lds_stats16 : 0);
             const long long grid16 = conv_split_blocks(G, ntiles, 16);
             hipLaunchKernelGGL((conv4tap_x6s_kernel<G, PL, EPI, 16, TR>), dim3((unsigned)grid16), dim3(1024), lds16, st, a, (int)ntiles);
             return mmlf_launch_status("mmlf_conv2x2_h2(16 waves)");
@@ -1276,11 +1360,17 @@
     hipLaunchKernelGGL((conv4tap_rs_kernel<G, NCH, EPI, TR>), dim3((unsigned)conv_rs_blocks(ngroups)), dim3(512), lds, st, a, (int)ngroups);
     return mmlf_launch_status("mmlf_conv2x2_h2(register-streamed)");
 }
-#define MMLF_CONV_KIND_SWITCH(LAUNCH, TR_PLAIN, TR_SHAPE, ...)                                                                              \
+#define MMLF_CONV_KIND_SWITCH(LAUNCH, TR_PLAIN, TR_SHAPE, BN_BWD_OK, ...)                                                                              \
     do {                                                                                                                \
         const int kind = (a.relu ? EPI_RELU : 0) | (a.bn_partial ? EPI_STATS : 0) | (a.relu_mask_in ? EPI_BITS_IN : 0) | \
                          (a.ref ? EPI_REF_IN : 0) | (a.relu_mask_out ? EPI_MASK_OUT : 0);                               \
         const bool tr = conv_tr_enabled() && (TR_SHAPE) && conv_tr_fits(a);                                             \
+        if (a.bn_bwd_partial) {     \
+            if constexpr ((BN_BWD_OK) && G > 0) {       \
+                if (kind == EPI_PLAIN && tr) return LAUNCH<__VA_ARGS__, EPI_BN_BWD, true>(a, n, st);                    \
+            }                                                                                                           \
+            return mmlf_fail("mmlf_conv2x2_h2: this launch has no kernel that takes the BatchNorm-backward sums"); \
+        }                                                                                                               \
         if ((a.relu_mask_in || a.relu_mask_out) && conv_tr_enabled() && (TR_SHAPE) && !tr)                              \
             return mmlf_fail("mmlf_conv2x2_h2: ReLU mask words need n_store %% 4 == 0 and a 16-byte aligned output");   \
         switch (kind) {                                                                                                 \
@@ -1296,7 +1386,7 @@
 template <int G, int NCH>
 static int launch_conv_rs(const ConvArgs &a, long long n, hipStream_t st)
 {
-    MMLF_CONV_KIND_SWITCH(launch_conv_rs_epi, false, true, G, NCH);
+    MMLF_CONV_KIND_SWITCH(launch_conv_rs_epi, false, true, false, G, NCH);
     return launch_conv_rs_epi<G, NCH, EPI_GENERIC>(a, n, st);
 }
 
@@ -1313,8 +1403,9 @@
         const long long n = ntiles;
         if (a.ref && !a.relu && !a.bn_partial && !a.relu_mask_in && !a.relu_mask_out)
             return launch_conv_x6s_epi<G, PL, EPI_REF_IN>(a, n, st);
-        MMLF_CONV_KIND_SWITCH(launch_conv_x6s_epi, G == 18, G != 18 || a.seg_delta == 0, G, PL);
-    }
+        MMLF_CONV_KIND_SWITCH(launch_conv_x6s_epi, G == 18, G != 18 || a.seg_delta == 0, true, G, PL);
+    }
+    if (a.bn_bwd_partial) return mmlf_fail("mmlf_conv2x2_h2: no kernel takes the BatchNorm-backward sums at this width or precision");
     return launch_conv_x6s_epi<G, PL, EPI_GENERIC>(a, ntiles, st);
 }
 
@@ -1331,11 +1422,18 @@
     }
 }
 
+struct BnBwdSums {
+    const float *z, *scale, *shift;
+    int cs_z;
+    double *partial;
+};
+
 static int conv_split_impl(const char *who, int planes, const float *in, int cs_in, int K, const void *packed,
                            const float *bias, int N, float *out, int cs_out, int N_store, int out_shift, int vh,
                            int vw, int B, int H, int W, int relu, const float *relu_ref, int cs_ref,
                            const float *in_amax, float *out_amax, double *bn_partial, void *stream,
-                           unsigned *relu_mask_out = nullptr, const unsigned *relu_mask_in = nullptr)
+                           unsigned *relu_mask_out = nullptr, const unsigned *relu_mask_in = nullptr,
+                           const BnBwdSums *bn_bwd = nullptr)
 {
     const int np = x6_np(N);
     ConvArgs a;
@@ -1349,6 +1447,16 @@
     MMLF_CHECK_ARG(!bn_partial || (planes == 2 && N_store >= N), "%s: BatchNorm statistics need the f16 split path", who);
     a.in_amax = in_amax; a.out_amax = out_amax; a.bn_partial = bn_partial;
     a.relu_mask_out = relu_mask_out; a.relu_mask_in = relu_mask_in;
+    if (bn_bwd) {
+        MMLF_CHECK_ARG(bn_bwd->z && bn_bwd->scale && bn_bwd->shift && bn_bwd->partial, "%s: null pointer", who);
+        MMLF_CHECK_ARG(bn_bwd->cs_z % 4 == 0 && bn_bwd->cs_z >= N_store && N_store >= N &&
+                           (reinterpret_cast<uintptr_t>(bn_bwd->z) & 15) == 0,
+                       "%s: cs_z=%d N_store=%d N=%d (z rows take 16-byte loads of the stored channels)", who, bn_bwd->cs_z,
+                       N_store, N);
+        a.bn_z = bn_bwd->z; a.bn_scale = bn_bwd->scale; a.bn_shift = bn_bwd->shift; a.cs_z = bn_bwd->cs_z;
+        a.bn_bwd_partial = bn_bwd->partial;
+        a.z_bytes = grid_alloc_positions(g) * a.cs_z * 4;
+    }
     a.w_unscale = planes == 2 ? reinterpret_cast<const float *>(reinterpret_cast<const char *>(packed) +
                                                                   (size_t)(cs_in / 8) * 8 * np * 16)
                               : nullptr;
@@ -1410,6 +1518,14 @@
                                float *out_amax, double *bn_partial, uint32_t *relu_mask_out,
                                const uint32_t *relu_mask_in, void *stream)
 {
+    if (relu == MMLF_RELU_BN_BWD_SUMS) {
+        MMLF_CHECK_ARG(!relu_mask_out && !relu_mask_in, "mmlf_conv2x2_h2 (BatchNorm-backward sums): no ReLU masks in this launch");
+        MMLF_CHECK_ARG(bias && relu_ref && bn_partial, "mmlf_conv2x2_h2 (BatchNorm-backward sums): null pointer");
+        const BnBwdSums sums = {relu_ref, bias, bias + N, cs_ref, bn_partial};
+        return conv_split_impl("mmlf_conv2x2_h2 (BatchNorm-backward sums)", 2, in, cs_in, K, packed, nullptr, N, out, cs_out,
+                               N_store, out_shift, vh, vw, B, H, W, 0, nullptr, 0, in_amax, out_amax, nullptr, stream, nullptr,
+                               nullptr, &sums);
+    }
     return conv_split_impl("mmlf_conv2x2_h2", 2, in, cs_in, K, packed, bias, N, out, cs_out, N_store, out_shift, vh,
                            vw, B, H, W, relu, relu_ref, cs_ref, in_amax, out_amax, bn_partial, stream, relu_mask_out,
                            relu_mask_in);
diff --git a/mmlf_amd/csrc/elementwise.hip b/mmlf_amd/csrc/elementwise.hip
--- a/mmlf_amd/csrc/elementwise.hip
+++ b/mmlf_amd/csrc/elementwise.hip
@@ -239,12 +239,14 @@
 __global__ __launch_bounds__(64) void bn_bwd_finalize_kernel(const double *__restrict__ partial, int nblocks, int C,
                                                              double n, const float *__restrict__ gamma,
                                                              const float *__restrict__ invstd, float *dgamma,
-                                                             float *dbeta, int accumulate, float *coef)
+                                                             float *dbeta, int accumulate, float *coef,
+                                                             const float *__restrict__ mean)
 {
     const int c = blockIdx.x;
     double sg, sgx;
     reduce_partials(partial, nblocks, C, c, sg, sgx);
     if (threadIdx.x != 0) return;
+    if (mean) sgx = (double)invstd[c] * (sgx - (double)mean[c] * sg);
     if (dgamma) dgamma[c] = accumulate ? dgamma[c] + (float)sgx : (float)sgx;
     if (dbeta) dbeta[c] = accumulate ? dbeta[c] + (float)sg : (float)sg;
     const double k1 = (double)(gamma ? gamma[c] : 1.f) * invstd[c];
@@ -1344,6 +1346,14 @@
                                   int accumulate, float *coef, double *partial, int nblocks, int B, int H, int W,
                                   void *stream)
 {
+    if (!gy && !z) {
+        MMLF_CHECK_ARG(save_mean && save_invstd && coef && partial && C > 0 && nblocks > 0,
+                       "mmlf_bn_bwd_reduce (sums given): bad argument");
+        MMLF_CHECK_ARG(B > 0 && H > 0 && W > 0, "mmlf_bn_bwd_reduce: bad shape B=%d H=%d W=%d", B, H, W);
+        hipLaunchKernelGGL(bn_bwd_finalize_kernel, dim3(C), dim3(64), 0, (hipStream_t)stream, partial, nblocks, C,
+                           (double)B * H * W, gamma, save_invstd, dgamma, dbeta, accumulate, coef, save_mean);
+        return mmlf_launch_status("mmlf_bn_bwd_reduce");
+    }
     MMLF_CHECK_ARG(gy && z && scale && shift && save_mean && save_invstd && coef && partial,
                    "mmlf_bn_bwd_reduce: null pointer");
     MMLF_CHECK_ARG(cs_gy % 2 == 0 && c_off % 2 == 0 && c_off >= 0 && cs_z % 4 == 0 && C > 0 && C <= cs_z &&
@@ -1355,7 +1365,7 @@
     hipLaunchKernelGGL(bn_reduce_bwd_kernel, dim3(nblocks), dim3(256), 0, st, z, cs_z, gy, cs_gy, c_off,
                        scale, shift, save_mean, save_invstd, C, partial, B, H, W);
     hipLaunchKernelGGL(bn_bwd_finalize_kernel, dim3(C), dim3(64), 0, st, partial, nblocks, C,
-                       (double)B * H * W, gamma, save_invstd, dgamma, dbeta, accumulate, coef);
+                       (double)B * H * W, gamma, save_invstd, dgamma, dbeta, accumulate, coef, (const float *)nullptr);
     return mmlf_launch_status("mmlf_bn_bwd_reduce");
 }
 
diff --git a/mmlf_amd/engine.py b/mmlf_amd/engine.py
--- a/mmlf_amd/engine.py
+++ b/mmlf_amd/engine.py
@@ -134,6 +134,13 @@
             cur.wait_event(last.record_event())
         self._last_stream = cur
 
+    def bn_bwd_sums(self, n):
+        self.enter_stream()
+        t = self.__dict__.get('_bn_bwd_sums')
+        if t is None or t.numel() < n:
+            t = self._bn_bwd_sums = torch.empty(n, dtype=torch.float64, device=self.device)
+        return t
+
     def scratch(self, name, n):
         if not name.endswith('_side'):
             self.enter_stream()
@@ -210,6 +217,7 @@
 
 CHECK_ABSMAX = bool(os.environ.get('MMLF_CHECK_ABSMAX'))
 OVERLAP_WGRAD = os.environ.get('MMLF_OVERLAP_WGRAD', '1') not in ('', '0')
+WIDE_MIN_K = 128
 
 
 CHECK_EXTENTS = bool(os.environ.get('MMLF_CHECK_EXTENTS'))
@@ -271,7 +279,7 @@
 
 
 def conv(geo, x, cs_in, K, packed, bias, N, out, cs_out, out_shift, vh, vw, relu, ref=None, cs_ref=0,
-         n_store=None, out_off=0, bn_partial=None, mask_out=None, mask_in=None, w_master=None, variant=0):
+         n_store=None, out_off=0, bn_partial=None, mask_out=None, mask_in=None, w_master=None, variant=0, bn_bwd=None):
     aout = getattr(out, 'absmax', None)
     if (w_master is not None and N <= THIN_MAX_N and K >= THIN_MIN_K and cs_in <= 512 and ref is None and mask_in is None
             and mask_out is None and bn_partial is None and out_off == 0 and n_store in (None, cs_out)):
@@ -293,12 +301,34 @@
                    {'in': (0, x, 0), 'packed': (1, packed, 0), 'bias': (2, bias, 0), 'out': (3, out, out_off),
                     'ref': (4, ref, 0), 'in_amax': (5, ax, 0), 'out_amax': (6, aout, 0), 'bn_partial': (7, bn_partial, 0),
                     'mask_out': (8, mask_out, 0), 'mask_in': (8, mask_in, 0)})
-        call('mmlf_conv2x2_h2', *args, ptr(ax), ptr(aout), ptr(bn_partial), ptr(mask_out), ptr(mask_in), _lib.stream_ptr())
+        if bn_bwd is not None:
+            assert bias is None and not relu and ref is None and bn_partial is None and mask_out is None and mask_in is None
+            z, cs_z, scale, shift, partial = bn_bwd
+            assert shift.data_ptr() == scale.data_ptr() + 4 * N and scale.numel() == N, 'scale and shift must be adjacent'
+            call('mmlf_conv2x2_h2', ptr(x), cs_in, K, ptr(packed), ptr(scale), N, ptr(out) + 4 * out_off, cs_out, n_store,
+                 out_shift, vh, vw, geo.B, geo.H, geo.W, RELU_BN_BWD_SUMS, ptr(z), cs_z, ptr(ax), ptr(aout), ptr(partial), None,
+                 None, _lib.stream_ptr())
+        else:
+            call('mmlf_conv2x2_h2', *args, ptr(ax), ptr(aout), ptr(bn_partial), ptr(mask_out), ptr(mask_in), _lib.stream_ptr())
     else:
+        assert bn_bwd is None
         call('mmlf_conv2x2_split' if CONV_MODE == 'bf16x6' else 'mmlf_conv2x2', *args, _lib.stream_ptr())
     if prof:
         nbytes = 4.0 * geo.B * (K * (geo.H * geo.W if out_shift == 0 else (geo.H + 1) * (geo.W + 1)) + N * vh * vw)
         _toc(events, 'conv' if K >= 256 else 'conv70', 2.0 * geo.B * vh * vw * N * 4 * K, nbytes)
+
+
+RELU_BN_BWD_SUMS = 2
+
+
+def bn_bwd_fusable(geo, K, N, cs_out):
+    if CONV_MODE != 'f16x3' or geo.ksize != 2 or cs_out % 4 or cs_out < N:
+        return False
+    if any(os.environ.get(k) is not None for k in ('MMLF_CONV_TR', 'MMLF_CONV_RS', 'MMLF_CONV_NW16')):
+        return False
+    if 32 < N <= 80:
+        return geo.P + 513 <= 640
+    return 128 < N <= 288 and geo.P + 257 <= 640
 
 
 
@@ -565,7 +595,8 @@
         call('mmlf_unpack_nchw', ptr(x), cs_x, ptr(out), self.oc, B, H, W, _lib.stream_ptr())
         return out, (tape if save else None)
 
-    def _block_bwd(self, geo, rec, p, grads, gy, cs_gy, c_off, need_dx, after_bn=None, overlap=False, packs=None):
+    def _block_bwd(self, geo, rec, p, grads, gy, cs_gy, c_off, need_dx, after_bn=None, overlap=False, packs=None, sums=None,
+                   below=None):
         spec, var = rec.spec, rec.var
         dev = gy.device
         ws = _Workspace.get(dev)
@@ -588,11 +619,18 @@
         dx = got[-1] if need_dx else None
         if spec.bn:
             coef = torch.empty(3 * C, dtype=torch.float32, device=dev)
+        if spec.bn and sums is not None:
+            assert c_off == 0 and not rec.eval
+            call('mmlf_bn_bwd_reduce', None, 0, 0, None, 0, C, None, None, ptr(p[f'{pre}.3.weight']), ptr(rec.smean),
+                 ptr(rec.sinv), ptr(grads[f'{pre}.3.weight']), ptr(grads[f'{pre}.3.bias']), 1, ptr(coef), ptr(sums[0]), sums[1],
+                 B, H, W, sp())
+        elif spec.bn:
             call('mmlf_bn_bwd_reduce', ptr(gy), cs_gy, c_off, ptr(z), cs_mid, C, ptr(rec.scale), ptr(rec.shift),
                  ptr(p[f'{pre}.3.weight']), ptr(rec.smean), ptr(rec.sinv), ptr(grads[f'{pre}.3.weight']),
                  ptr(grads[f'{pre}.3.bias']), 1, ptr(coef), ptr(ws.partial), BN_BLOCKS, B, H, W, sp())
             if rec.eval:
                 coef[C:].zero_()
+        if spec.bn:
             dz = got[0]
             call('mmlf_bn_bwd_apply', ptr(gy), cs_gy, c_off, ptr(z), cs_mid, C, ptr(rec.scale), ptr(rec.shift),
                  ptr(rec.smean), ptr(coef), ptr(dz), cs_mid, B, H, W, ptr(dz.absmax), sp())
@@ -604,6 +642,12 @@
         self._wgrad(geo, True, y, cs_mid, C, dz, cs_mid, C, gw2, gb2, var)
         self._dgrad(geo, True, dz, cs_mid, C, self._packed(packs, p, f'{pre}.2.weight', var, True), C, dy, cs_mid, **y_relu)
         del dz, got
+        fused = None
+        if (need_dx and spec.cin < WIDE_MIN_K and spec.bn is True and below is not None and below.spec.bn is True and not below.eval and not x_relu
+                and below.spec.cout == spec.cin and bn_bwd_fusable(geo, C, spec.cin, cs_x)):
+            nblk = int(_lib.load().mmlf_conv2x2_blocks(C, spec.cin, B, H, W))
+            fused = (ws.bn_bwd_sums(2 * nblk * spec.cin), nblk)
+            x_relu = {'bn_bwd': (below.z, cs_of(below.spec.cout), below.scale, below.shift, fused[0])}
         if overlap and need_dx:
             self._dgrad(geo, False, dy, cs_mid, C, self._packed(packs, p, f'{pre}.0.weight', var, True), spec.cin, dx, cs_x,
                         **x_relu)
@@ -613,12 +657,12 @@
                 ws.side.wait_event(ready)
                 self._wgrad(geo, False, x, cs_x, spec.cin, dy, cs_mid, C, gw1, gb1, var, side=True)
                 done = ws.side.record_event()
-            return dx, done, (x, dy)
+            return dx, done, (x, dy), fused
         self._wgrad(geo, False, x, cs_x, spec.cin, dy, cs_mid, C, gw1, gb1, var)
         if need_dx:
             self._dgrad(geo, False, dy, cs_mid, C, self._packed(packs, p, f'{pre}.0.weight', var, True), spec.cin, dx, cs_x,
                         **x_relu)
-        return dx, None, None
+        return dx, None, None, fused
 
     def backward(self, p, tape, grad_output, grads, on_done=None):
         geo = tape['geo']
@@ -642,11 +686,12 @@
                     on_done(pending[1])
                 pending = None
 
+        sums = None
         while recs:
             rec = recs.pop()
-            wide = OVERLAP_WGRAD and rec.spec.cin >= 128 and self.ksize == 2
-            g, event, keep = self._block_bwd(geo, rec, p, grads, g, cs_g, 0, True, after_bn=settle, overlap=wide,
-                                             packs=tape['packs'])
+            wide = OVERLAP_WGRAD and rec.spec.cin >= WIDE_MIN_K and self.ksize == 2
+            g, event, keep, sums = self._block_bwd(geo, rec, p, grads, g, cs_g, 0, True, after_bn=settle, overlap=wide,
+                                                   packs=tape['packs'], sums=sums, below=recs[-1] if recs else None)
             settle()
             if event is not None:
                 pending = (event, rec.spec.prefix, keep)
@@ -662,9 +707,11 @@
                 cs_s, off = cs_of(self.chs), 0
                 gs = geo.buf(cs_s, dev)
                 relu_bwd_slice(geo, g, cs_g, s * self.chs, tape['concat'], cs_g, s * self.chs, self.chs, gs, cs_s)
+            sums = None
             while recs:
                 rec = recs.pop()
-                gs, _, _ = self._block_bwd(geo, rec, p, grads, gs, cs_s, off, need_dx=bool(recs), packs=tape['packs'])
+                gs, _, _, sums = self._block_bwd(geo, rec, p, grads, gs, cs_s, off, need_dx=bool(recs), packs=tape['packs'],
+                                                 sums=sums, below=recs[-1] if recs else None)
                 cs_s, off = rec.cs_x, 0
             if on_done and s in (2, 0):
                 on_done('in_net_id' if s == 2 else 'in_net_hv')
```

After: 1137 (median of 6 runs). About the same (+0.3%).
